# stochasticHydroTools/PSE

Hardware: AMD Instinct MI355X
Metric: BD particle-steps/s (full PSE Brownian step: M.F + k-space noise + Lanczos M^1/2.psi + Euler), N=1e6, phi=0.1 (higher is better)
Workload: dtype f64; 1 GPU; random-sphere suspension N=1000000, phi=0.1, cubic L=347.29, grid 256^3, xi=0.4405, rcut=5.966, P=6, error=0.001, kT=1.0, dt=0.001; parallelism=1 GPU

## Files before the change

include/pse_amd.h:

```cpp
#ifndef PSE_AMD_H
#define PSE_AMD_H

#ifdef __cplusplus
extern "C" {
#endif

typedef struct { double x, y, z, w; } pse_double4;
typedef struct { double x, y, z; } pse_double3;
typedef struct { int x, y, z; } pse_int3;

typedef struct pse_handle pse_handle;

enum pse_status {
    PSE_OK = 0,
    PSE_ERR_INVALID = -1,
    PSE_ERR_HIP = -2,
    PSE_ERR_FFT = -3,
    PSE_ERR_COMM = -4,
    PSE_ERR_NUMERIC = -5
};

typedef struct pse_params {
    unsigned int n_max;
    double Lx, Ly, Lz, xy;
    double xi;
    double error;
    double max_strain;
    unsigned int seed;
    int Nx, Ny, Nz;
    int P;
    double rcut;
    int device;
    int n_slabs;
    int slab_rank;
    int local_rows;
} pse_params;

typedef struct pse_info {
    int Nx, Ny, Nz, P;
    double rcut, xi, eta, gaussm, lambda, self_mobility, hx, hy, hz;
    int ncell_x, ncell_y, ncell_z;
    int lanczos_m;
    int lanczos_matvecs;
    double lanczos_stepnorm;
    double t_sort, t_spread, t_fft_fwd, t_scale, t_fft_inv, t_gather, t_real, t_lanczos, t_integrate, t_comm, t_total;
    unsigned long long device_bytes;
    double t_matvec;
    double t_records;
    int lanczos_exchanges;
    int lanczos_status;
    unsigned long long lanczos_open_calls;
} pse_info;

int pse_create(const pse_params *params, pse_handle **out);
int pse_destroy(pse_handle *h);
int pse_set_box(pse_handle *h, double Lx, double Ly, double Lz, double xy);
int pse_set_stream(pse_handle *h, void *hip_stream);
int pse_set_async(pse_handle *h, int enabled);
int pse_set_timestep_offset(pse_handle *h, const unsigned int *device_word);
int pse_debug_last_gate(pse_handle *h, int *gate);
int pse_set_neighbor_skin(pse_handle *h, double r_buff);
int pse_neighbor_stats(pse_handle *h, double *r_buff, unsigned long long *builds, unsigned long long *reuses);
int pse_set_timing(pse_handle *h, int enabled);
int pse_get_info(pse_handle *h, pse_info *info);
const char *pse_last_error(void);

int pse_mobility(pse_handle *h, const pse_double4 *pos, const pse_double4 *force, pse_double4 *vel,
                 const unsigned int *group_members, unsigned int N, int parts);

int pse_brownian_velocity(pse_handle *h, const pse_double4 *pos, const pse_double4 *force, pse_double4 *vel,
                          const unsigned int *group_members, unsigned int N,
                          double kT, double dt, unsigned int timestep, int *lanczos_m);

int pse_brownian_velocity_part(pse_handle *h, const pse_double4 *pos, const pse_double4 *force, pse_double4 *vel,
                               const unsigned int *group_members, unsigned int N, double kT, double dt, unsigned int timestep,
                               int parts, int *lanczos_m);
int pse_integrate(pse_handle *h, pse_double4 *pos, const pse_double4 *vel, pse_double3 *accel, pse_int3 *image,
                  const pse_double4 *net_force, const unsigned int *group_members, unsigned int N, double dt, double shear_rate);

int pse_step(pse_handle *h, pse_double4 *pos, pse_double4 *vel, pse_double3 *accel, pse_int3 *image,
             const pse_double4 *net_force, const unsigned int *group_members, unsigned int N,
             double kT, double dt, unsigned int timestep, double shear_rate, int *lanczos_m);

int pse_sqrt_mreal(pse_handle *h, const pse_double4 *pos, const pse_double4 *psi, pse_double4 *out,
                   const unsigned int *group_members, unsigned int N, double tol, int *lanczos_m);

int pse_random_psi(pse_handle *h, pse_double4 *psi, const unsigned int *group_members, unsigned int N,
                   unsigned int timestep);

int pse_eval_realspace(pse_handle *h, const double *r_host, int n, double *f_host, double *g_host);
int pse_pair_repulsion(pse_handle *h, const pse_double4 *pos, pse_double4 *force, const unsigned *group, unsigned N,
                       double k, double sigma, int accumulate);
int pse_debug_copy_grid(pse_handle *h, int stage, double *host_out);
int pse_debug_spread(pse_handle *h, const pse_double4 *pos, const pse_double4 *force, const unsigned int *group_members,
                     unsigned int N);
int pse_debug_kvector(pse_handle *h, int n, const int *ijk_host, double *out_host);
int pse_debug_grid_placement(pse_handle *h, int *tried, float *ms_first, float *ms_kept);
int pse_debug_vq_roundtrip(int n, const double *rows_host, double *out_host);
int pse_debug_matvec_ms(pse_handle *h, int reps, float *ms_per_launch);

typedef struct pse_team pse_team;
int pse_team_unique_id(void *id128_host);
int pse_team_create(pse_handle **members, int n_members, const void *id128_host, pse_team **out);
typedef struct pse_host_xfer {
    const double *send; size_t send_count; int send_to;
    double *recv; size_t recv_count; int recv_from;
} pse_host_xfer;
typedef struct pse_transport {
    void *user;
    int (*exchange)(void *user, int n_xfers, const pse_host_xfer *xfers);
    int (*allreduce_sum)(void *user, double *host_buf, size_t count);
} pse_transport;
int pse_team_create_transport(pse_handle *member, const pse_transport *transport, pse_team **out);
int pse_team_destroy(pse_team *team);
int pse_team_mobility(pse_team *team, const pse_double4 *const *pos, const pse_double4 *const *force,
                      pse_double4 *const *vel, const unsigned int *group_members, unsigned int N, int parts);
int pse_team_brownian_velocity(pse_team *team, const pse_double4 *const *pos, const pse_double4 *const *force,
                               pse_double4 *const *vel, const unsigned int *group_members, unsigned int N,
                               double kT, double dt, unsigned int timestep, int *lanczos_m);
int pse_team_step(pse_team *team, pse_double4 *const *pos, pse_double4 *const *vel, pse_double3 *const *accel,
                  pse_int3 *const *image, const pse_double4 *const *net_force, const unsigned int *group_members,
                  unsigned int N, double kT, double dt, unsigned int timestep, double shear_rate, int *lanczos_m);

int pse_team_step_local(pse_team *team, pse_double4 *const *pos, pse_double4 *const *vel, pse_double3 *const *accel,
                        pse_int3 *const *image, const pse_double4 *const *net_force, unsigned int *const *tag,
                        unsigned int *const *n_local, double kT, double dt, unsigned int timestep, double shear_rate,
                        int integrate, int *lanczos_m);
int pse_team_redistribute_local(pse_team *team, pse_double4 *const *pos, pse_double4 *const *vel, pse_double3 *const *accel,
                                pse_int3 *const *image, pse_double4 *const *net_force, unsigned int *const *tag,
                                unsigned int *const *n_local);
int pse_team_set_lanczos_extra(pse_team *team, int extra);
int pse_set_lanczos_extra(pse_handle *h, int extra);
enum pse_lanczos_operator { PSE_LANCZOS_RECORDS16 = 0, PSE_LANCZOS_FP64 = 1 };
int pse_set_lanczos_operator(pse_handle *h, int op);
int pse_get_lanczos_operator(pse_handle *h, int *op);
int pse_local_layout(pse_handle *h, int *rows_own, int *rows_ghost, int *records, int *layers, int *layers_per_rank);
int pse_team_local_status(pse_team *team, int *flags);

#define PSE_DIAG_MAX 48
typedef struct pse_team_diag {
    int n_exchanges;
    int kind[PSE_DIAG_MAX];
    int lane[PSE_DIAG_MAX];
    double device_us[PSE_DIAG_MAX];
    double host_us[PSE_DIAG_MAX];
    unsigned long long bytes[PSE_DIAG_MAX];
    double main_lane_ms, side_lane_ms;
    double critical_path_ms;
} pse_team_diag;
int pse_team_set_diag(pse_team *team, int enabled);
int pse_team_get_diag(pse_team *team, pse_team_diag *out);

int pse_team_debug_solo(pse_team *team, int slab_rank);

int pse_host_lanczos_sqrt_e1(int m, const double *alpha, const double *beta, double *t);
int pse_host_select_params(const pse_params *params, pse_info *info);

#ifdef __cplusplus
}
#endif
#endif
```

pse_amd/_lib.py:

```python
import ctypes
import os

_HERE = os.path.dirname(os.path.abspath(__file__))


def asan_dir():
    d = os.environ.get("PSE_ASAN_DIR")
    if not d:
        return None
    if not os.path.exists(os.path.join(d, ".pse_asan_build")):
        import sys
        print(f"pse_amd: PSE_ASAN_DIR={d} ignored: no sanitizer build there (python -m pse_amd.build --asan writes one)", file=sys.stderr)
        return None
    if not getattr(asan_dir, "_said", False):
        import sys
        print(f"pse_amd: using the CPU SANITIZER build in {d} (PSE_ASAN_DIR): device entry points are stubs", file=sys.stderr)
        asan_dir._said = True
    return d


_ASAN_DIR = asan_dir()
LIB_PATH = os.path.join(_ASAN_DIR or _HERE, "libpse_amd.so")

PSE_OK = 0
# ... 13 lines not shown
        ("local_rows", ctypes.c_int),
    ]


class pse_info(ctypes.Structure):
    _fields_ = [
        ("Nx", ctypes.c_int), ("Ny", ctypes.c_int), ("Nz", ctypes.c_int), ("P", ctypes.c_int),
        ("rcut", ctypes.c_double), ("xi", ctypes.c_double), ("eta", ctypes.c_double), ("gaussm", ctypes.c_double),
        ("lam", ctypes.c_double), ("self_mobility", ctypes.c_double),
        ("hx", ctypes.c_double), ("hy", ctypes.c_double), ("hz", ctypes.c_double),
        ("ncell_x", ctypes.c_int), ("ncell_y", ctypes.c_int), ("ncell_z", ctypes.c_int),
        ("lanczos_m", ctypes.c_int), ("lanczos_matvecs", ctypes.c_int),
        ("lanczos_stepnorm", ctypes.c_double),
        ("t_sort", ctypes.c_double), ("t_spread", ctypes.c_double), ("t_fft_fwd", ctypes.c_double),
        ("t_scale", ctypes.c_double), ("t_fft_inv", ctypes.c_double), ("t_gather", ctypes.c_double),
        ("t_real", ctypes.c_double), ("t_lanczos", ctypes.c_double), ("t_integrate", ctypes.c_double),
        ("t_comm", ctypes.c_double), ("t_total", ctypes.c_double),
        ("device_bytes", ctypes.c_ulonglong),
        ("t_matvec", ctypes.c_double),
        ("t_records", ctypes.c_double),
        ("lanczos_exchanges", ctypes.c_int),
        ("lanczos_status", ctypes.c_int),
        ("lanczos_open_calls", ctypes.c_ulonglong),
    ]

    def as_dict(self):
        return {name: getattr(self, name) for name, _ in self._fields_}


class pse_host_xfer(ctypes.Structure):
    _fields_ = [("send", ctypes.POINTER(ctypes.c_double)), ("send_count", ctypes.c_size_t), ("send_to", ctypes.c_int),
                ("recv", ctypes.POINTER(ctypes.c_double)), ("recv_count", ctypes.c_size_t), ("recv_from", ctypes.c_int)]


PSE_DIAG_MAX = 48


class pse_team_diag(ctypes.Structure):
    _fields_ = [("n_exchanges", ctypes.c_int), ("kind", ctypes.c_int * PSE_DIAG_MAX), ("lane", ctypes.c_int * PSE_DIAG_MAX),
                ("device_us", ctypes.c_double * PSE_DIAG_MAX), ("host_us", ctypes.c_double * PSE_DIAG_MAX),
                ("bytes", ctypes.c_ulonglong * PSE_DIAG_MAX), ("main_lane_ms", ctypes.c_double), ("side_lane_ms", ctypes.c_double),
                ("critical_path_ms", ctypes.c_double)]


EXCHANGE_FN = ctypes.CFUNCTYPE(ctypes.c_int, ctypes.c_void_p, ctypes.c_int, ctypes.POINTER(pse_host_xfer))
ALLREDUCE_FN = ctypes.CFUNCTYPE(ctypes.c_int, ctypes.c_void_p, ctypes.POINTER(ctypes.c_double), ctypes.c_size_t)


class pse_transport(ctypes.Structure):
    _fields_ = [("user", ctypes.c_void_p), ("exchange", EXCHANGE_FN), ("allreduce_sum", ALLREDUCE_FN)]


_vp, _i, _u, _d = ctypes.c_void_p, ctypes.c_int, ctypes.c_uint, ctypes.c_double
_ip = ctypes.POINTER(ctypes.c_int)
_dp = ctypes.POINTER(ctypes.c_double)
SYMBOLS = {
    "pse_create": (_i, [ctypes.POINTER(pse_params), ctypes.POINTER(_vp)]),
    "pse_destroy": (_i, [_vp]),
    "pse_set_box": (_i, [_vp, _d, _d, _d, _d]),
    "pse_set_stream": (_i, [_vp, _vp]),
    "pse_set_timing": (_i, [_vp, _i]),
    "pse_set_async": (_i, [_vp, _i]),
    "pse_set_timestep_offset": (_i, [_vp, _vp]),
    "pse_debug_last_gate": (_i, [_vp, _ip]),
    "pse_set_neighbor_skin": (_i, [_vp, _d]),
    "pse_neighbor_stats": (_i, [_vp, ctypes.POINTER(ctypes.c_double), ctypes.POINTER(ctypes.c_ulonglong), ctypes.POINTER(ctypes.c_ulonglong)]),
    "pse_get_info": (_i, [_vp, ctypes.POINTER(pse_info)]),
    "pse_last_error": (ctypes.c_char_p, []),
    "pse_mobility": (_i, [_vp, _vp, _vp, _vp, _vp, _u, _i]),
    "pse_brownian_velocity": (_i, [_vp, _vp, _vp, _vp, _vp, _u, _d, _d, _u, _ip]),
    "pse_brownian_velocity_part": (_i, [_vp, _vp, _vp, _vp, _vp, _u, _d, _d, _u, _i, _ip]),
    "pse_integrate": (_i, [_vp, _vp, _vp, _vp, _vp, _vp, _vp, _u, _d, _d]),
    "pse_step": (_i, [_vp, _vp, _vp, _vp, _vp, _vp, _vp, _u, _d, _d, _u, _d, _ip]),
    "pse_sqrt_mreal": (_i, [_vp, _vp, _vp, _vp, _vp, _u, _d, _ip]),
    "pse_random_psi": (_i, [_vp, _vp, _vp, _u, _u]),
    "pse_pair_repulsion": (_i, [_vp, _vp, _vp, _vp, _u, _d, _d, _i]),
    "pse_eval_realspace": (_i, [_vp, _dp, _i, _dp, _dp]),
    "pse_debug_copy_grid": (_i, [_vp, _i, _dp]),
    "pse_debug_spread": (_i, [_vp, _vp, _vp, _vp, _u]),
    "pse_debug_kvector": (_i, [_vp, _i, _ip, _dp]),
    "pse_debug_grid_placement": (_i, [_vp, _ip, ctypes.POINTER(ctypes.c_float), ctypes.POINTER(ctypes.c_float)]),
    "pse_debug_vq_roundtrip": (_i, [_i, _dp, _dp]),
    "pse_debug_matvec_ms": (_i, [_vp, _i, ctypes.POINTER(ctypes.c_float)]),
    "pse_team_unique_id": (_i, [_vp]),
    "pse_team_create": (_i, [ctypes.POINTER(_vp), _i, _vp, ctypes.POINTER(_vp)]),
    "pse_team_create_transport": (_i, [_vp, ctypes.POINTER(pse_transport), ctypes.POINTER(_vp)]),
    "pse_team_destroy": (_i, [_vp]),
    "pse_team_debug_solo": (_i, [_vp, _i]),
    "pse_team_mobility": (_i, [_vp, ctypes.POINTER(_vp), ctypes.POINTER(_vp), ctypes.POINTER(_vp), _vp, _u, _i]),
    "pse_team_brownian_velocity": (_i, [_vp, ctypes.POINTER(_vp), ctypes.POINTER(_vp), ctypes.POINTER(_vp), _vp, _u, _d, _d, _u, _ip]),
    "pse_team_step": (_i, [_vp, ctypes.POINTER(_vp), ctypes.POINTER(_vp), ctypes.POINTER(_vp), ctypes.POINTER(_vp),
                           ctypes.POINTER(_vp), _vp, _u, _d, _d, _u, _d, _ip]),
    "pse_team_step_local": (_i, [_vp, ctypes.POINTER(_vp), ctypes.POINTER(_vp), ctypes.POINTER(_vp), ctypes.POINTER(_vp),
                                 ctypes.POINTER(_vp), ctypes.POINTER(_vp), ctypes.POINTER(_vp), _d, _d, _u, _d, _i, _ip]),
    "pse_local_layout": (_i, [_vp, _ip, _ip, _ip, _ip, _ip]),
    "pse_team_local_status": (_i, [_vp, _ip]),
    "pse_team_set_lanczos_extra": (_i, [_vp, _i]),
    "pse_set_lanczos_extra": (_i, [_vp, _i]),
    "pse_set_lanczos_operator": (_i, [_vp, _i]),
    "pse_get_lanczos_operator": (_i, [_vp, _ip]),
    "pse_team_redistribute_local": (_i, [_vp] + [ctypes.POINTER(_vp)] * 7),
    "pse_team_set_diag": (_i, [_vp, _i]),
    "pse_team_get_diag": (_i, [_vp, ctypes.POINTER(pse_team_diag)]),
    "pse_host_lanczos_sqrt_e1": (_i, [_i, _dp, _dp, _dp]),
    "pse_host_select_params": (_i, [ctypes.POINTER(pse_params), ctypes.POINTER(pse_info)]),
}

_lib = None


class PSEError(RuntimeError):
    pass


def load():
    global _lib
    if _lib is not None:
        return _lib
    if not os.path.exists(LIB_PATH):
        raise PSEError(f"{LIB_PATH} not found: build it with `python -m pse_amd.build` "
                       "(there is no CPU fallback for the PSE hot path)")
    if not _ASAN_DIR:
        try:
            import torch
        except ImportError:
            pass
    lib = ctypes.CDLL(LIB_PATH, mode=ctypes.RTLD_GLOBAL)
    for name, (res, args) in SYMBOLS.items():
        fn = getattr(lib, name)
        fn.restype = res
        fn.argtypes = args
    _lib = lib
    return lib


def check(status):
    if status != PSE_OK:
        raise PSEError(f"pse_amd error {status}: {load().pse_last_error().decode()}")
```

pse_amd/csrc/asan_stub.cpp:

```cpp
#include <cmath>
#include <vector>

#include "pse_err.h"

using namespace pse;

struct pse_handle {
    pse_params par;
    Derived d;
    pse_info info;
    std::vector<double> coef;
    int n_intervals = 0;
    unsigned long long steps = 0;
    int lz_op = PSE_LANCZOS_RECORDS16;
};
struct pse_team { int unused; };

static int no_device(const char *what) { return fail(PSE_ERR_HIP, "%s: sanitizer build, there is no device behind this library", what); }

extern "C" {

int pse_create(const pse_params *p, pse_handle **out) {
    if (!p || !out) return fail(PSE_ERR_INVALID, "null argument");
    *out = nullptr;
    if (p->n_max == 0) return fail(PSE_ERR_INVALID, "n_max must be positive");
    if (!(std::fabs(p->xy) <= 0.5 * (1.0 + 1e-9))) return fail(PSE_ERR_INVALID, "tilt xy = %g outside [-0.5, 0.5]", p->xy);
    pse_handle *h = new pse_handle();
    h->par = *p;
    std::string e = select_params(Box{p->Lx, p->Ly, p->Lz, p->xy}, p->xi, p->error, p->max_strain, p->Nx, p->Ny, p->Nz, p->P, p->rcut, h->d);
    if (!e.empty()) { delete h; return fail(PSE_ERR_INVALID, "%s", e.c_str()); }
    if (int rc = gaussian_fits(h->d, h->d.hx, h->d.hy, h->d.hz)) { delete h; return rc; }
    build_realspace_table(h->d.xi, h->d.rcut, h->coef, h->n_intervals);
    fill_info(h->d, &h->info);
    *out = h;
    return 0;
}
int pse_destroy(pse_handle *h) { delete h; return 0; }
int pse_set_box(pse_handle *h, double Lx, double Ly, double Lz, double xy) {
    if (!h) return fail(PSE_ERR_INVALID, "null handle");
    if (!(Lx > 0 && Ly > 0 && Lz > 0)) return fail(PSE_ERR_INVALID, "box lengths must be positive");
    if (!(std::fabs(xy) <= 0.5 * (1.0 + 1e-9))) return fail(PSE_ERR_INVALID, "tilt xy = %g outside [-0.5, 0.5]", xy);
    if (int rc = gaussian_fits(h->d, Lx / h->d.Nx, Ly / h->d.Ny, Lz / h->d.Nz)) return rc;
    h->par.Lx = Lx; h->par.Ly = Ly; h->par.Lz = Lz; h->par.xy = xy;
    h->info.hx = Lx / h->d.Nx; h->info.hy = Ly / h->d.Ny; h->info.hz = Lz / h->d.Nz;
    return 0;
}
int pse_get_info(pse_handle *h, pse_info *info) {
    if (!h || !info) return fail(PSE_ERR_INVALID, "null argument");
    *info = h->info;
    return 0;
}
int pse_step(pse_handle *h, pse_double4 *, pse_double4 *, pse_double3 *, pse_int3 *, const pse_double4 *, const unsigned int *,
             unsigned int N, double kT, double dt, unsigned int, double, int *lanczos_m) {
    if (!h) return fail(PSE_ERR_INVALID, "null handle");
    if (N == 0 || N > h->par.n_max) return fail(PSE_ERR_INVALID, "N = %u outside (0, n_max = %u]", N, h->par.n_max);
    if (kT < 0 || !(dt > 0)) return fail(PSE_ERR_INVALID, "need kT >= 0 and dt > 0");
    ++h->steps;
    if (lanczos_m && *lanczos_m < 2) *lanczos_m = 2;
    return 0;
}
int pse_pair_repulsion(pse_handle *h, const pse_double4 *, pse_double4 *, const unsigned *, unsigned N, double, double sigma, int) {
    if (!h) return fail(PSE_ERR_INVALID, "null handle");
    if (N == 0 || N > h->par.n_max) return fail(PSE_ERR_INVALID, "N = %u outside (0, n_max = %u]", N, h->par.n_max);
    if (!(sigma > 0.0) || sigma > h->d.rcut) return fail(PSE_ERR_INVALID, "repulsion range %.4f outside (0, rcut = %.4f]", sigma, h->d.rcut);
    return 0;
}

int pse_set_stream(pse_handle *, void *) { return no_device("pse_set_stream"); }
int pse_set_timing(pse_handle *, int) { return no_device("pse_set_timing"); }
int pse_set_async(pse_handle *, int) { return no_device("pse_set_async"); }
int pse_set_timestep_offset(pse_handle *, const unsigned int *) { return no_device("pse_set_timestep_offset"); }
int pse_debug_last_gate(pse_handle *, int *) { return no_device("pse_debug_last_gate"); }
int pse_set_neighbor_skin(pse_handle *, double) { return no_device("pse_set_neighbor_skin"); }
int pse_neighbor_stats(pse_handle *, double *, unsigned long long *, unsigned long long *) { return no_device("pse_neighbor_stats"); }
int pse_mobility(pse_handle *, const pse_double4 *, const pse_double4 *, pse_double4 *, const unsigned int *, unsigned int, int) { return no_device("pse_mobility"); }
int pse_brownian_velocity(pse_handle *, const pse_double4 *, const pse_double4 *, pse_double4 *, const unsigned int *, unsigned int, double,
                          double, unsigned int, int *) { return no_device("pse_brownian_velocity"); }
int pse_sqrt_mreal(pse_handle *, const pse_double4 *, const pse_double4 *, pse_double4 *, const unsigned int *, unsigned int, double, int *) { return no_device("pse_sqrt_mreal"); }
int pse_random_psi(pse_handle *, pse_double4 *, const unsigned int *, unsigned int, unsigned int) { return no_device("pse_random_psi"); }
int pse_eval_realspace(pse_handle *, const double *, int, double *, double *) { return no_device("pse_eval_realspace"); }
int pse_debug_copy_grid(pse_handle *, int, double *) { return no_device("pse_debug_copy_grid"); }
int pse_debug_spread(pse_handle *, const pse_double4 *, const pse_double4 *, const unsigned int *, unsigned int) { return no_device("pse_debug_spread"); }
int pse_debug_kvector(pse_handle *, int, const int *, double *) { return no_device("pse_debug_kvector"); }
int pse_debug_grid_placement(pse_handle *, int *, float *, float *) { return no_device("pse_debug_grid_placement"); }
int pse_debug_vq_roundtrip(int, const double *, double *) { return no_device("pse_debug_vq_roundtrip"); }
int pse_debug_matvec_ms(pse_handle *, int, float *) { return no_device("pse_debug_matvec_ms"); }
int pse_set_lanczos_extra(pse_handle *, int) { return no_device("pse_set_lanczos_extra"); }
int pse_set_lanczos_operator(pse_handle *h, int op) {
    if (!h) return fail(PSE_ERR_INVALID, "pse_set_lanczos_operator: null handle");
    if (op != PSE_LANCZOS_RECORDS16 && op != PSE_LANCZOS_FP64) return fail(PSE_ERR_INVALID, "pse_set_lanczos_operator: %d is not an operator", op);
    h->lz_op = op;
    return 0;
}
int pse_get_lanczos_operator(pse_handle *h, int *op) {
    if (!h || !op) return fail(PSE_ERR_INVALID, "pse_get_lanczos_operator: null argument");
    *op = h->lz_op;
    return 0;
}
int pse_brownian_velocity_part(pse_handle *, const pse_double4 *, const pse_double4 *, pse_double4 *, const unsigned int *, unsigned int, double,
                               double, unsigned int, int, int *) { return no_device("pse_brownian_velocity_part"); }
int pse_integrate(pse_handle *, pse_double4 *, const pse_double4 *, pse_double3 *, pse_int3 *, const pse_double4 *, const unsigned int *, unsigned int,
                  double, double) { return no_device("pse_integrate"); }
int pse_team_redistribute_local(pse_team *, pse_double4 *const *, pse_double4 *const *, pse_double3 *const *, pse_int3 *const *, pse_double4 *const *,
                                unsigned int *const *, unsigned int *const *) { return no_device("pse_team_redistribute_local"); }
int pse_team_set_lanczos_extra(pse_team *, int) { return no_device("pse_team_set_lanczos_extra"); }
int pse_team_unique_id(void *) { return no_device("pse_team_unique_id"); }
int pse_team_create(pse_handle **, int, const void *, pse_team **) { return no_device("pse_team_create"); }
int pse_team_create_transport(pse_handle *, const pse_transport *, pse_team **) { return no_device("pse_team_create_transport"); }
int pse_team_destroy(pse_team *) { return 0; }
int pse_team_debug_solo(pse_team *, int) { return no_device("pse_team_debug_solo"); }
int pse_team_step_local(pse_team *, pse_double4 *const *, pse_double4 *const *, pse_double3 *const *, pse_int3 *const *, const pse_double4 *const *,
                        unsigned int *const *, unsigned int *const *, double, double, unsigned int, double, int, int *) { return no_device("pse_team_step_local"); }
int pse_local_layout(pse_handle *, int *, int *, int *, int *, int *) { return no_device("pse_local_layout"); }
int pse_team_local_status(pse_team *, int *) { return no_device("pse_team_local_status"); }
int pse_team_set_diag(pse_team *, int) { return no_device("pse_team_set_diag"); }
int pse_team_get_diag(pse_team *, pse_team_diag *) { return no_device("pse_team_get_diag"); }
int pse_team_mobility(pse_team *, const pse_double4 *const *, const pse_double4 *const *, pse_double4 *const *, const unsigned int *, unsigned int, int) { return no_device("pse_team_mobility"); }
int pse_team_brownian_velocity(pse_team *, const pse_double4 *const *, const pse_double4 *const *, pse_double4 *const *, const unsigned int *,
                               unsigned int, double, double, unsigned int, int *) { return no_device("pse_team_brownian_velocity"); }
int pse_team_step(pse_team *, pse_double4 *const *, pse_double4 *const *, pse_double3 *const *, pse_int3 *const *, const pse_double4 *const *,
                  const unsigned int *, unsigned int, double, double, unsigned int, double, int *) { return no_device("pse_team_step"); }

}
```

pse_amd/csrc/pse_capi.hip:

```cpp
#include <hip/hip_runtime.h>
#include <rccl/rccl.h>
#include <rocfft/rocfft.h>

#include <algorithm>
#include <chrono>
#include <cmath>
#include <cstdarg>
#include <cstdio>
#include <cstring>
#include <dlfcn.h>
#include <functional>
#include <future>
#include <memory>
#include <mutex>
#include <thread>
#include <string>
#include <vector>

#include "../../include/pse_amd.h"
#include "pse_err.h"
#include "pse_host.h"
#include "pse_kernels.h"
#include "pse_local.h"

using namespace pse;

#define HIPCHK(x)                                                                                      \
    do {                                                                                               \
        hipError_t e_ = (x);                                                                           \
        if (e_ != hipSuccess) return fail(PSE_ERR_HIP, "%s failed: %s (%s:%d)", #x, hipGetErrorString(e_), __FILE__, __LINE__); \
    } while (0)
#define FFTCHK(x)                                                                                      \
    do {                                                                                               \
        rocfft_status s_ = (x);                                                                        \
        if (s_ != rocfft_status_success) return fail(PSE_ERR_FFT, "%s failed: rocfft status %d (%s:%d)", #x, (int)s_, __FILE__, __LINE__); \
    } while (0)

#define TRY(x)              \
    do {                    \
        int r_ = (x);       \
        if (r_) return r_;  \
    } while (0)

constexpr int M_MAX = 100;
constexpr int PH_COUNT_ = 13;

struct Phase {
    hipEvent_t a = nullptr, b = nullptr;
};

struct pse_handle {
    pse_params par;
    Derived d;
    Box box;
    DBox dbox;
    DGrid G;
    DCells nc;
    double cell_gamma;
    int device = 0;
    hipStream_t stream = nullptr;
    hipStream_t wstream = nullptr;
    hipStream_t side = nullptr;
    hipStream_t side_owned = nullptr;
    int *bounds_host = nullptr;
    hipEvent_t ev_bounds = nullptr;
    bool bounds_pending = false;
    struct Tuning {
        int cell_bz = 6;
        double skin = 0.4;
        int overlap = 1;
        bool no_xfuse = false;
        int own_y_pow2 = 1;
        int own_y = 1;
        int own_z = 1;
        int yslab_regs = 1;
        int yfft_kb = 4;
        int wave_mode = 0;
        int spread_tz = 0, spread_nw = 0;
        int gather_bz = 0;
        int xmix_runtime = 0;
        int xfft_small_wide = 0;
        bool verbose = false;
        bool team_sstep = true;
        int team_sched[3] = {1, 2, 3};
        int vq = 1;
        int place_trials = 10;
        int lz_extra = 2;
        int lz_op = PSE_LANCZOS_RECORDS16;
    } tun;
    DCells bidx_nc = {0, 0, 0};
    hipEvent_t ev_fork = nullptr, ev_join = nullptr;
    bool overlap_all = false;
    bool side_on = false;
    hipEvent_t ev_scal = nullptr;
    int n_max = 0, n_pad = 0;
    unsigned *keys = nullptr, *keys_s = nullptr, *vals = nullptr, *perm = nullptr, *tag_s = nullptr;
    void *sort_tmp = nullptr;
    int *cell_cnt = nullptr;
    size_t sort_tmp_bytes = 0;
    int *cell_off = nullptr;
    int *cnt_block = nullptr;
    size_t cnt_bins = 0;
    SpreadWork sw = {};
    NbList nb = {};
    double4 *nb64 = nullptr;
    int lz_op = PSE_LANCZOS_RECORDS16;
    bool nb_valid = false;
    bool lz_last_queued = false;
    double skin = 0.0;
    double skin_max = 0.0;
    VerletList vl = {};
    double4 *pos_build = nullptr;
    int *flags_host = nullptr;
    bool vl_valid = false;
    bool vl_use = false;
    bool vl_pending = false;
    int vl_N = 0; const unsigned *vl_group = nullptr; Box vl_box = {};
    bool nc_wide = false;
    unsigned long long nlist_builds = 0, nlist_reuses = 0;
    int vl_reused_since_build = 0, vl_misses[2] = {0, 0}, vl_suspend_left[2] = {0, 0}, vl_suspend_len[2] = {32, 32};
    int vl_kind = 0;
    bool pv_is_f = false;
    bool w_is_mpsi = false;
    bool sums0_done = false;
    CombineSink sink = {};
    bool tail_done = false;
    bool async_mode = false;
    bool gated = false;
    int *gate_word = nullptr;
    size_t n_cells_alloc = 0;
    float4 *posf_s = nullptr;
    double2 *pv = nullptr;
    double4 *pos_s = nullptr, *f_s = nullptr, *uw_s = nullptr, *ur_s = nullptr, *ub_s = nullptr, *psi_s = nullptr, *w_s = nullptr;
    double *coef = nullptr;
    int n_intervals = 0;
    double *rgrid = nullptr;
    double2 *cgrid = nullptr;
    rocfft_plan plan_fwd = nullptr, plan_inv = nullptr;
    rocfft_plan plan_x_fwd = nullptr, plan_x_inv = nullptr;
    rocfft_execution_info info_fwd = nullptr, info_inv = nullptr;
    int n_slabs = 1, slab_rank = 0, nyl = 0, y0 = 0;
    double2 *sendbuf = nullptr, *recvbuf = nullptr;
    int *d_bidx = nullptr, *d_bounds = nullptr;
    std::vector<int> row_lo, first_end, last_begin;
    std::vector<int> first2_end, last2_begin;
    double4 *w2_s = nullptr, *u_s = nullptr;
    double *sums_all = nullptr;
    double4 *utot_s = nullptr;
    bool xfuse = false;
    bool own_y = false;
    bool own_y_slab = false;
    int lz_extra = -1;
    void *vq = nullptr;
    int place_tried = 0; float place_ms_first = 0, place_ms_kept = 0;
    bool own_z = false;
    double2 *twiddle_z = nullptr, *twiddle_z_owned = nullptr;
    double2 *twiddle_y = nullptr;
    double2 *twiddle_y_owned = nullptr;
    int grid_slabs = 1;
    double2 *twiddle = nullptr;
    void *fft_work = nullptr;
    size_t fft_work_bytes = 0;
    double4 *V = nullptr;
    double *scal = nullptr, *partials = nullptr;
    double *sc_host = nullptr;
    double *sc_host_dev = nullptr;
    int *bounds_host_dev = nullptr;
    int npart_cap = 0;
    struct LocalPlan {
        bool on = false;
        LocalGeom g{};
        int rows_cap = 0;
        double *send[2] = {nullptr, nullptr}, *recv[2] = {nullptr, nullptr};
        size_t msg = 0;
        double4 *stage_w1 = nullptr, *stage_w2 = nullptr;
        double4 *porig_s = nullptr; double *mass_s = nullptr; int3 *image_s = nullptr;
        LocalRows *rows = nullptr;
        int *counters = nullptr;
        int *layer_cnt = nullptr;
        size_t zero_ints = 0;
        bool zeroed = false;
        int *err = nullptr, *err_host = nullptr;
        double *rd_send = nullptr, *rd_recv = nullptr;
        int *rd_rows = nullptr, *rd_off = nullptr, *rd_host = nullptr;
    } loc;
// ... 94 lines not shown

static int cells_for(const Box &box, double rc, double gamma, int n_slabs, int bz_want, DCells &out, int xpad = 0) {
    const double wx = box.Lx / std::sqrt(1.0 + gamma * gamma), wy = box.Ly, wz = box.Lz;
    if (rc > 0.5 * wx * (1 + 1e-12) || rc > 0.5 * wy * (1 + 1e-12) || rc > 0.5 * wz * (1 + 1e-12))
        return fail(PSE_ERR_INVALID, "real-space cutoff %.4f exceeds half the box width (%.4f, %.4f, %.4f at tilt %.3f): "
                    "the minimum-image near field needs rcut <= L/2; increase xi", rc, wx, wy, wz, gamma);
    auto n = [&](double w) { int c = (int)std::floor(w / rc); if (c < 3) c = 1; if (c > 1024) c = 1024; return c; };
    out = DCells{n(wx), n(wy), n(wz), 0, 1, xpad};
    out.bz = (bz_want > 0 && out.nz >= 2 * bz_want) ? bz_want : out.nz;
    out.nzb = (out.nz + out.bz - 1) / out.bz;
    if (n_slabs > 1) {
        const int c = (int)std::floor(wx / rc) / n_slabs * n_slabs;
        if (c < 3 || c < n_slabs)
            return fail(PSE_ERR_INVALID, "box too small to split the near field over %d ranks: only %d cells of width >= rcut "
                        "fit along x", n_slabs, (int)std::floor(wx / rc));
        out.nx = std::min(c, 1024 / n_slabs * n_slabs);
    }
    return 0;
}
static double near_radius(const pse_handle *h) { return h->d.rcut + h->skin_max; }
static int set_cells(pse_handle *h, double gamma) {
    DCells nc;
    TRY(cells_for(h->box, near_radius(h), gamma, h->n_slabs, h->tun.cell_bz, nc, h->loc.on ? 1 : 0));
    h->nc = nc;
    h->cell_gamma = gamma;
    h->nc_wide = h->skin_max > 0.0;
    return 0;
}

enum { PH_SORT, PH_SPREAD, PH_FFTF, PH_SCALE, PH_FFTI, PH_GATHER, PH_REAL, PH_LANCZOS, PH_INTEG, PH_COMM, PH_TOTAL, PH_MATVEC, PH_RECORDS, PH_COUNT };
struct Roctx {
    int (*push)(const char *) = nullptr;
    int (*pop)() = nullptr;
    Roctx() {
        const char *e = getenv("PSE_ROCTX");
        if (!e || !atoi(e)) return;
        void *lib = dlopen("libroctx64.so.4", RTLD_NOW | RTLD_GLOBAL);
        if (!lib) lib = dlopen("libroctx64.so", RTLD_NOW | RTLD_GLOBAL);
        if (!lib) return;
        push = (int (*)(const char *))dlsym(lib, "roctxRangePushA");
        pop = (int (*)())dlsym(lib, "roctxRangePop");
        if (!push || !pop) push = nullptr, pop = nullptr;
    }
};
static const Roctx &roctx() { static Roctx r; return r; }
static_assert(PH_COUNT == PH_COUNT_, "phase table");
static const char *const PH_NAME[PH_COUNT] = {"pse:sort", "pse:spread", "pse:fft_forward", "pse:kspace_scale", "pse:fft_inverse", "pse:gather",
                                              "pse:near_field", "pse:lanczos", "pse:integrate", "pse:exchange", "pse:total", "pse:matvec",
                                              "pse:far_records"};
static void range_push(int p) { if (roctx().push) roctx().push(PH_NAME[p]); }
static void range_pop() { if (roctx().pop) roctx().pop(); }
static int ts(pse_handle *h, int p) { range_push(p); if (h->timing) HIPCHK(hipEventRecord(h->ph[p].a, h->stream)); return 0; }
static int te(pse_handle *h, int p) { if (h->timing) HIPCHK(hipEventRecord(h->ph[p].b, h->stream)); range_pop(); return 0; }
static int tsw(pse_handle *h, int p) { range_push(p); if (h->timing) HIPCHK(hipEventRecord(h->ph[p].a, h->wstream)); return 0; }
static int tew(pse_handle *h, int p) { if (h->timing) HIPCHK(hipEventRecord(h->ph[p].b, h->wstream)); range_pop(); return 0; }

static int collect_times(pse_handle *h, unsigned mask) {
    if (!h->timing) return 0;
    HIPCHK(hipStreamSynchronize(h->stream));
    if (h->side) HIPCHK(hipStreamSynchronize(h->side));
    double *dst[PH_COUNT] = {&h->info.t_sort, &h->info.t_spread, &h->info.t_fft_fwd, &h->info.t_scale, &h->info.t_fft_inv,
                             &h->info.t_gather, &h->info.t_real, &h->info.t_lanczos, &h->info.t_integrate, &h->info.t_comm,
                             &h->info.t_total, &h->info.t_matvec, &h->info.t_records};
    for (int p = 0; p < PH_COUNT; ++p) {
        *dst[p] = 0.0;
        if (mask & (1u << p)) {
            float ms = 0;
            if (hipEventElapsedTime(&ms, h->ph[p].a, h->ph[p].b) == hipSuccess) *dst[p] = ms;
        }
    }
    return 0;
}

extern "C" int pse_destroy(pse_handle *h) {
    if (!h) return 0;
    (void)hipSetDevice(h->device);
    (void)hipDeviceSynchronize();
    if (h->plan_fwd) rocfft_plan_destroy(h->plan_fwd);
    if (h->plan_inv) rocfft_plan_destroy(h->plan_inv);
    if (h->plan_x_fwd) rocfft_plan_destroy(h->plan_x_fwd);
    if (h->plan_x_inv) rocfft_plan_destroy(h->plan_x_inv);
    if (h->info_fwd) rocfft_execution_info_destroy(h->info_fwd);
    if (h->info_inv) rocfft_execution_info_destroy(h->info_inv);
    void *ptrs[] = {h->keys, h->keys_s, h->vals, h->perm, h->tag_s, h->sort_tmp, h->cell_off, h->cnt_block, h->sw.rec_t, h->sw.fb.off, h->sw.fb.rank_s, h->sw.fb.tmp, h->nb.data, h->nb.cnt, h->vl.idx, h->vl.cnt, h->pos_build, h->pos_s, h->posf_s, h->pv,
                    h->f_s, h->uw_s, h->ur_s, h->ub_s, h->psi_s, h->w_s, h->coef, h->rgrid, h->cgrid, h->sendbuf, h->recvbuf, h->d_bidx, h->d_bounds, h->utot_s, h->w2_s, h->u_s, h->sums_all, h->twiddle, h->twiddle_y_owned, h->twiddle_z_owned, h->fft_work, h->V,
                    h->scal, h->partials, h->lz_state, h->vq, h->nb64};
    for (void *p : ptrs) if (p) (void)hipFree(p);
    for (auto &p : h->ph) { if (p.a) (void)hipEventDestroy(p.a); if (p.b) (void)hipEventDestroy(p.b); }
    if (h->ev_fork) (void)hipEventDestroy(h->ev_fork);
    if (h->ev_scal) (void)hipEventDestroy(h->ev_scal);
    if (h->ev_join) (void)hipEventDestroy(h->ev_join);
    if (h->side_owned) (void)hipStreamDestroy(h->side_owned);
    if (h->bounds_host) (void)hipHostFree(h->bounds_host);
    if (h->ev_bounds) (void)hipEventDestroy(h->ev_bounds);
    if (h->sc_host) (void)hipHostFree(h->sc_host);
    if (h->flags_host) (void)hipHostFree(h->flags_host);
    {
        void *lp[] = {h->loc.send[0], h->loc.send[1], h->loc.recv[0], h->loc.recv[1], h->loc.stage_w1, h->loc.stage_w2, h->loc.porig_s, h->loc.mass_s,
                      h->loc.image_s, h->loc.rows, h->loc.err, h->loc.rd_send, h->loc.rd_recv, h->loc.rd_rows, h->loc.rd_off};
        for (void *q : lp) if (q) (void)hipFree(q);
        if (h->loc.err_host) (void)hipHostFree(h->loc.err_host);
        if (h->loc.rd_host) (void)hipHostFree(h->loc.rd_host);
    }
    delete h;
    return 0;
}

static int make_plans(pse_handle *h) {
    std::call_once(g_fft_once, [] { rocfft_setup(); });
    const DGrid &G = h->G;
    size_t work = 0, w = 0;
    h->xfuse = xfuse_supported(G.Nx) && !h->tun.no_xfuse;
    if (h->xfuse) {
        std::vector<double2> tw(G.Nx);
        for (int m = 0; m < G.Nx; ++m) {
            const long double ang = -2.0L * 3.14159265358979323846264338327950288L * m / G.Nx;
            tw[m] = make_double2((double)cosl(ang), (double)sinl(ang));
        }
        TRY(dmalloc(h, &h->twiddle, (size_t)G.Nx));
        HIPCHK(hipMemcpy(h->twiddle, tw.data(), G.Nx * sizeof(double2), hipMemcpyHostToDevice));
    }
    const bool z_ok = h->tun.own_z > 0 && zfft_supported(G.Nz);
    h->own_y = h->xfuse && h->grid_slabs == 1 && h->tun.own_y > 0 &&
               (yfft_supported(G.Ny) || (h->tun.own_y_pow2 && yfft_regs_supported(G.Ny, G.Nz, z_ok)));
    h->own_y_slab = h->xfuse && h->grid_slabs > 1 && h->tun.own_y > 0 && yfft_possible(G.Ny);
    h->own_z = z_ok && (h->own_y || h->own_y_slab);
    if (h->own_z) {
        if (G.Nz == G.Nx) h->twiddle_z = h->twiddle;
        else {
            std::vector<double2> tw(G.Nz);
            for (int m = 0; m < G.Nz; ++m) {
                const long double ang = -2.0L * 3.14159265358979323846264338327950288L * m / G.Nz;
                tw[m] = make_double2((double)cosl(ang), (double)sinl(ang));
            }
            TRY(dmalloc(h, &h->twiddle_z_owned, (size_t)G.Nz));
            HIPCHK(hipMemcpy(h->twiddle_z_owned, tw.data(), G.Nz * sizeof(double2), hipMemcpyHostToDevice));
            h->twiddle_z = h->twiddle_z_owned;
        }
    }
    if (h->own_y || h->own_y_slab) {
        if (G.Ny == G.Nx) h->twiddle_y = h->twiddle;
        else {
            std::vector<double2> tw(G.Ny);
            for (int m = 0; m < G.Ny; ++m) {
                const long double ang = -2.0L * 3.14159265358979323846264338327950288L * m / G.Ny;
                tw[m] = make_double2((double)cosl(ang), (double)sinl(ang));
            }
            TRY(dmalloc(h, &h->twiddle_y_owned, (size_t)G.Ny));
            HIPCHK(hipMemcpy(h->twiddle_y_owned, tw.data(), G.Ny * sizeof(double2), hipMemcpyHostToDevice));
            h->twiddle_y = h->twiddle_y_owned;
        }
    }
    auto real_plans = [&](size_t dims, const size_t *len, size_t batch) -> int {
        size_t rs[3] = {1, (size_t)G.Nz, (size_t)G.Ny * G.Nz}, cs[3] = {1, (size_t)G.Nzp, (size_t)G.Ny * G.Nzp};
        const size_t rdist = dims == 1 ? (size_t)G.Nz : (dims == 2 ? (size_t)G.Ny * G.Nz : (size_t)G.Nx * G.Ny * G.Nz);
        const size_t cdist = dims == 1 ? (size_t)G.Nzp : (dims == 2 ? (size_t)G.Ny * G.Nzp : (size_t)G.Nx * G.Ny * G.Nzp);
        rocfft_plan_description df = nullptr, di = nullptr;
        FFTCHK(rocfft_plan_description_create(&df));
        FFTCHK(rocfft_plan_description_create(&di));
        FFTCHK(rocfft_plan_description_set_data_layout(df, rocfft_array_type_real, rocfft_array_type_hermitian_interleaved, nullptr, nullptr,
                                                       dims, rs, rdist, dims, cs, cdist));
        FFTCHK(rocfft_plan_description_set_data_layout(di, rocfft_array_type_hermitian_interleaved, rocfft_array_type_real, nullptr, nullptr,
                                                       dims, cs, cdist, dims, rs, rdist));
        FFTCHK(rocfft_plan_create(&h->plan_fwd, rocfft_placement_notinplace, rocfft_transform_type_real_forward,
                                  rocfft_precision_double, dims, len, batch, df));
        FFTCHK(rocfft_plan_create(&h->plan_inv, rocfft_placement_notinplace, rocfft_transform_type_real_inverse,
                                  rocfft_precision_double, dims, len, batch, di));
// ... 1 lines not shown
        rocfft_plan_description_destroy(di);
        return 0;
    };
    if (h->own_y) {
        const size_t len1[1] = {(size_t)G.Nz};
        TRY(real_plans(1, len1, (size_t)3 * G.Nx * G.Ny));
    } else if (h->xfuse && h->grid_slabs == 1) {
        const size_t len2[2] = {(size_t)G.Nz, (size_t)G.Ny};
        TRY(real_plans(2, len2, (size_t)3 * G.Nx));
    } else if (h->grid_slabs == 1) {
        const size_t len[3] = {(size_t)G.Nz, (size_t)G.Ny, (size_t)G.Nx};
        TRY(real_plans(3, len, 3));
    } else {
        const size_t len2[2] = {(size_t)G.Nz, (size_t)G.Ny};
        const size_t len1[1] = {(size_t)G.Nz};
        if (h->own_y_slab) TRY(real_plans(1, len1, (size_t)G.nxl * G.Ny));
        else TRY(real_plans(2, len2, (size_t)G.nxl));
        const size_t lenx[1] = {(size_t)G.Nx};
        size_t stride[1] = {(size_t)h->nyl * G.Nzp};
        rocfft_plan_description desc = nullptr;
        FFTCHK(rocfft_plan_description_create(&desc));
        FFTCHK(rocfft_plan_description_set_data_layout(desc, rocfft_array_type_complex_interleaved,
                                                       rocfft_array_type_complex_interleaved, nullptr, nullptr, 1, stride, 1,
                                                       1, stride, 1));
        FFTCHK(rocfft_plan_create(&h->plan_x_fwd, rocfft_placement_inplace, rocfft_transform_type_complex_forward,
                                  rocfft_precision_double, 1, lenx, stride[0], desc));
        FFTCHK(rocfft_plan_create(&h->plan_x_inv, rocfft_placement_inplace, rocfft_transform_type_complex_inverse,
                                  rocfft_precision_double, 1, lenx, stride[0], desc));
        rocfft_plan_description_destroy(desc);
        FFTCHK(rocfft_plan_get_work_buffer_size(h->plan_x_fwd, &w)); work = std::max(work, w);
        FFTCHK(rocfft_plan_get_work_buffer_size(h->plan_x_inv, &w)); work = std::max(work, w);
    }
    FFTCHK(rocfft_plan_get_work_buffer_size(h->plan_fwd, &w)); work = std::max(work, w);
    FFTCHK(rocfft_plan_get_work_buffer_size(h->plan_inv, &w)); work = std::max(work, w);
    h->fft_work_bytes = work;
    if (work) TRY(dmalloc(h, (char **)&h->fft_work, work));
    FFTCHK(rocfft_execution_info_create(&h->info_fwd));
    FFTCHK(rocfft_execution_info_create(&h->info_inv));
    if (work) {
        FFTCHK(rocfft_execution_info_set_work_buffer(h->info_fwd, h->fft_work, work));
        FFTCHK(rocfft_execution_info_set_work_buffer(h->info_inv, h->fft_work, work));
    }
    FFTCHK(rocfft_execution_info_set_stream(h->info_fwd, h->wstream));
    FFTCHK(rocfft_execution_info_set_stream(h->info_inv, h->wstream));
    return 0;
}

static bool team_sstep(const pse_handle *h);
static int create_impl(const pse_params *p, pse_handle *h) {
    h->par = *p;
    h->box = Box{p->Lx, p->Ly, p->Lz, p->xy};
    std::string e = select_params(h->box, p->xi, p->error, p->max_strain, p->Nx, p->Ny, p->Nz, p->P, p->rcut, h->d);
    if (!e.empty()) return fail(PSE_ERR_INVALID, "%s", e.c_str());
    if (p->n_max == 0) return fail(PSE_ERR_INVALID, "n_max must be positive");
    TRY(gaussian_fits(h->d, h->d.hx, h->d.hy, h->d.hz));
    if (!(std::fabs(p->xy) <= 0.5 * (1.0 + 1e-9)))
        return fail(PSE_ERR_INVALID, "tilt xy = %g outside [-0.5, 0.5]: HOOMD flips the box there, and the sequential minimum image "
                    "(PSEv1/Mobility.cu:648) is exact only up to that tilt", p->xy);
    const Derived &d = h->d;
    if (p->device >= 0) { HIPCHK(hipSetDevice(p->device)); h->device = p->device; }
    else HIPCHK(hipGetDevice(&h->device));
    h->n_max = (int)p->n_max;
    set_dbox(h);
    h->n_slabs = std::max(1, p->n_slabs);
    h->loc.on = p->local_rows != 0;
    if (h->loc.on && h->n_slabs < 2) return fail(PSE_ERR_INVALID, "local_rows needs n_slabs >= 2 (an owned-particle rank is a member of a team)");
    (void)roctx();
    {
        auto ienv = [](const char *name, int dflt) { const char *v = getenv(name); return v ? atoi(v) : dflt; };
        auto &t = h->tun;
        t.cell_bz = std::min(16, std::max(0, ienv("PSE_CELL_BZ", 6)));
        if (const char *v = getenv("PSE_SKIN")) t.skin = atof(v);
        t.overlap = ienv("PSE_OVERLAP", 1);
        t.no_xfuse = getenv("PSE_NO_XFUSE") != nullptr;
        t.own_y = ienv("PSE_OWN_Y", 1); t.own_y_pow2 = ienv("PSE_OWN_Y_POW2", 1); t.yfft_kb = ienv("PSE_YFFT_KB", 4); t.own_z = ienv("PSE_OWN_Z", 1); t.yslab_regs = ienv("PSE_YSLAB_REGS", 1);
        if (const char *v = getenv("PSE_WAVE_MODE")) t.wave_mode = !strcmp(v, "slab") ? 1 : (!strcmp(v, "replicated") ? 2 : 0);
        t.spread_tz = ienv("PSE_SPREAD_TZ", 0); t.spread_nw = ienv("PSE_SPREAD_NW", 0);
        t.gather_bz = ienv("PSE_GATHER_BZ", 0); t.xmix_runtime = ienv("PSE_XMIX", 0) == 1; t.xfft_small_wide = ienv("PSE_XFFT_SMALL_KB", 2) == 8;
        t.verbose = ienv("PSE_VERBOSE", 0) > 0;
        t.team_sstep = ienv("PSE_TEAM_SSTEP", 1) > 0;
        t.lz_extra = std::max(0, std::min(32, ienv("PSE_LANCZOS_EXTRA", 2)));
        t.place_trials = std::max(0, std::min(12, ienv("PSE_PLACE_TRIALS", 10)));
        t.vq = ienv("PSE_VQ", 1);
        if (const char *v = getenv("PSE_LANCZOS_OP")) t.lz_op = !strcmp(v, "fp64") ? PSE_LANCZOS_FP64 : PSE_LANCZOS_RECORDS16;
        if (const char *v = getenv("PSE_TEAM_SCHED")) {
            int a = 1, b = 2, c = 3;
            if (sscanf(v, "%d,%d,%d", &a, &b, &c) == 3) { t.team_sched[0] = a; t.team_sched[1] = b; t.team_sched[2] = c; }
        }
        h->sw.force_tz = t.spread_tz; h->sw.force_nw = t.spread_nw; h->sw.force_bz = t.gather_bz;
    }
    {
        double skin = h->tun.skin;
        const int nint = (int)std::ceil(d.rcut * RS_PER_UNIT) + 1;
        const double gam = std::max(std::fabs(p->xy), p->max_strain);
        const double wmin = std::min(std::min(h->box.Lx / std::sqrt(1.0 + gam * gam), h->box.Ly), h->box.Lz);
        if (!(skin > 0.0) || h->n_slabs > 1 || !mreal_table_in_lds(nint * 2 * RS_NCOEF) || d.rcut + skin > 0.5 * wmin)
            skin = 0.0;
        h->skin = h->skin_max = skin;
    }
    TRY(set_cells(h, std::max(std::fabs(p->xy), p->max_strain)));
    fill_info(d, &h->info);
    h->info.ncell_x = h->nc.nx; h->info.ncell_y = h->nc.ny; h->info.ncell_z = h->nc.nz;

    DGrid &G = h->G;
    G.Nx = d.Nx; G.Ny = d.Ny; G.Nz = d.Nz; G.Nzh = d.Nz / 2 + 1; G.P = d.P;
    G.Nzp = (G.Nzh + 7) & ~7;
    h->n_slabs = std::max(1, p->n_slabs);
    h->slab_rank = h->n_slabs > 1 ? p->slab_rank : 0;
    if (h->slab_rank < 0 || h->slab_rank >= h->n_slabs) return fail(PSE_ERR_INVALID, "slab_rank outside [0, n_slabs)");
    h->grid_slabs = h->n_slabs;
    if (h->n_slabs > 1) {
        const bool replicate = h->tun.wave_mode ? h->tun.wave_mode == 2 : h->n_slabs == 2;
        if (replicate && !h->loc.on) h->grid_slabs = 1;
    }
    if (h->grid_slabs > 1) {
        if (d.Nx % h->grid_slabs || d.Ny % h->grid_slabs)
            return fail(PSE_ERR_INVALID, "slab decomposition needs Nx and Ny divisible by the number of ranks (%d x %d over %d)",
                        d.Nx, d.Ny, h->grid_slabs);
        if (d.Nx / h->grid_slabs < d.P)
            return fail(PSE_ERR_INVALID, "slabs of %d planes are thinner than the support P = %d", d.Nx / h->grid_slabs, d.P);
    }
    const int grid_rank = h->grid_slabs > 1 ? h->slab_rank : 0;
    G.nxl = d.Nx / h->grid_slabs; G.x0 = grid_rank * G.nxl;
    G.hl = h->grid_slabs > 1 ? (d.P - 1) / 2 : 0;
    G.nhalo = h->grid_slabs > 1 ? (d.P + 1) / 2 : 0;
    h->nyl = d.Ny / h->grid_slabs; h->y0 = grid_rank * h->nyl;
    G.hx = d.hx; G.hy = d.hy; G.hz = d.hz;
    const double c = 2.0 * d.xi * d.xi / d.eta;
    G.expfac = c;
    G.prefac = (c / M_PI) * std::sqrt(c / M_PI);

    const size_t n = ((size_t)h->n_max + h->n_slabs - 1) / h->n_slabs * h->n_slabs;
    h->n_pad = (int)n;
    TRY(dmalloc(h, &h->keys, n)); TRY(dmalloc(h, &h->keys_s, n)); TRY(dmalloc(h, &h->vals, n));
    TRY(dmalloc(h, &h->perm, n)); TRY(dmalloc(h, &h->tag_s, n));

    {
        const double rc = d.rcut;
        auto cnt = [&](double w) { int c2 = (int)std::floor(w / rc); if (c2 < 3) c2 = 1; if (c2 > 1024) c2 = 1024; return (size_t)c2; };
        h->n_cells_alloc = cnt(h->box.Lx) * cnt(h->box.Ly) * (cnt(h->box.Lz) + 16) + cnt(h->box.Lx);
    }
    TRY(dmalloc(h, &h->cell_off, h->n_cells_alloc + 1));
    h->sort_tmp_bytes = cell_sort_temp_bytes(h->n_cells_alloc);
    TRY(dmalloc(h, (char **)&h->sort_tmp, h->sort_tmp_bytes));
    const size_t nbins = (size_t)((d.Nx + 7) / 8) * ((d.Ny + 7) / 8) * ((d.Nz + 7) / 8);
    const bool fast_far = d.P >= 4 && d.P <= FAR_PMAX;
    h->cnt_bins = ((fast_far ? nbins + 1 : 0) + 1 + 3) & ~(size_t)3;
    constexpr size_t LAYER_INTS = (size_t)LOCAL_MAX_LAYERS * LOCAL_LAYER_SLOTS;
    TRY(dmalloc(h, &h->cnt_block, h->cnt_bins + 4 + h->n_cells_alloc + 1 + 8 + LOCAL_NCOUNTER + 2 + LAYER_INTS + 4));
    h->loc.counters = h->cnt_block + ((h->cnt_bins + 4 + h->n_cells_alloc + 1 + 8 + 1) & ~(size_t)1);
    h->loc.layer_cnt = h->loc.counters + LOCAL_NCOUNTER;
    h->loc.zero_ints = ((size_t)(h->loc.layer_cnt - h->cnt_block) + LAYER_INTS + 3) & ~(size_t)3;
    if (h->nc.nx > LOCAL_MAX_LAYERS && p->local_rows) return fail(PSE_ERR_INVALID, "more than %d cell layers along x", LOCAL_MAX_LAYERS);
    h->vl.flags = h->cnt_block + h->cnt_bins - 1;
    h->gate_word = h->cnt_block + h->cnt_bins + 1;
    h->cell_cnt = h->cnt_block + h->cnt_bins + 4;
    if (fast_far) {
        h->sw.fb.cnt = h->cnt_block;
        TRY(dmalloc(h, (char **)&h->sw.rec_t, (n + 64) * 64));
        TRY(dmalloc(h, &h->sw.fb.rank_s, n));
        TRY(dmalloc(h, &h->sw.fb.off, nbins + 1));
        h->sw.fb.tmp_bytes = bin_scan_temp_bytes(nbins);
        TRY(dmalloc(h, (char **)&h->sw.fb.tmp, h->sw.fb.tmp_bytes));
    }
    std::vector<double> coef;
    build_realspace_table(d.xi, d.rcut, coef, h->n_intervals);
    TRY(dmalloc(h, &h->coef, coef.size()));
    HIPCHK(hipMemcpy(h->coef, coef.data(), coef.size() * sizeof(double), hipMemcpyHostToDevice));
    TRY(dmalloc(h, &h->nb.cnt, n));
    {
        const double vol = h->box.Lx * h->box.Ly * h->box.Lz;
        const double n_box = h->loc.on ? (double)n * h->n_slabs * (h->nc.nx / h->n_slabs) / (h->nc.nx / h->n_slabs + 4.0) : (double)n;
        const double nbar = n_box / vol * 4.18879020478639 * d.rcut * d.rcut * d.rcut;
        int cap = (int)std::ceil(1.5 * nbar + 16.0);
        cap = (std::max(16, std::min(cap, 256)) + 3) & ~3;
        const double bytes = (double)cap * (double)n * 20.0;
        if (bytes > 32e9 || n >= ((size_t)1 << 27)) cap = 0;
        h->nb.cap = cap;
        if (cap > 0) {
            TRY(dmalloc(h, &h->nb.data, nb_list_bytes(n + 1024, cap)));
        }
        if (cap == 0) h->skin = h->skin_max = 0.0;
        if (h->skin_max > 0.0) {
            const double rs = d.rcut + h->skin_max, nbar_v = n_box / vol * 4.18879020478639 * rs * rs * rs;
            h->vl.cap = (std::max(16, std::min((int)std::ceil(2.0 * nbar_v + 32.0), 512)) + 3) & ~3;
            h->vl.rskin = rs;
            TRY(dmalloc(h, (char **)&h->vl.idx, verlet_list_bytes(n + 1024, h->vl.cap)));
            TRY(dmalloc(h, &h->vl.cnt, n));
            TRY(dmalloc(h, &h->pos_build, n));
            HIPCHK(hipHostMalloc((void **)&h->flags_host, 2 * sizeof(int)));
        }
    }
    TRY(dmalloc(h, &h->pos_s, n)); TRY(dmalloc(h, &h->posf_s, n));
    TRY(dmalloc(h, &h->pv, 3 * n));
    TRY(dmalloc(h, &h->f_s, n)); TRY(dmalloc(h, &h->uw_s, n)); TRY(dmalloc(h, &h->ur_s, n));
    TRY(dmalloc(h, &h->ub_s, n)); TRY(dmalloc(h, &h->psi_s, n)); TRY(dmalloc(h, &h->w_s, n));

    const size_t nr = (size_t)(G.nxl + G.hl + G.nhalo) * G.Ny * G.Nz, ncx = (size_t)G.nxl * G.Ny * G.Nzp;
    TRY(dmalloc(h, &h->rgrid, 3 * nr));
    TRY(dmalloc(h, &h->cgrid, 3 * ncx));
    if (h->grid_slabs > 1) { TRY(dmalloc(h, &h->sendbuf, 3 * ncx)); TRY(dmalloc(h, &h->recvbuf, 3 * ncx)); }
    if (h->n_slabs > 1) {
        HIPCHK(hipHostMalloc((void **)&h->bounds_host, ((size_t)5 * h->n_slabs + 1) * sizeof(int), hipHostMallocMapped));
        HIPCHK(hipHostGetDevicePointer((void **)&h->bounds_host_dev, h->bounds_host, 0));
        HIPCHK(hipEventCreateWithFlags(&h->ev_bounds, hipEventDisableTiming));
        TRY(dmalloc(h, &h->d_bidx, (size_t)5 * h->n_slabs + 1)); TRY(dmalloc(h, &h->d_bounds, (size_t)5 * h->n_slabs + 1));
        TRY(dmalloc(h, &h->utot_s, n));
        TRY(dmalloc(h, &h->sums_all, (size_t)h->n_slabs * LZ_NGRAM));
        if (h->tun.team_sstep && h->nb.cap > 0) {
            TRY(dmalloc(h, &h->w2_s, n)); TRY(dmalloc(h, &h->u_s, n));
        }
    }
    if (h->loc.on) {
        auto &L = h->loc;
        const int G_ = h->n_slabs, per = h->nc.nx / G_, depth = 2;
        if (per < depth + 1 || (G_ - 1) * per < 2 * depth)
            return fail(PSE_ERR_INVALID, "an owned-particle rank needs >= %d cell layers of width rcut per rank along x (%d ranks: %d layers each)",
                        G_ == 2 ? 2 * depth : depth + 1, G_, per);
        if (!team_sstep(h))
            return fail(PSE_ERR_INVALID, "an owned-particle rank needs the per-step pair list and the real-space table in LDS (rcut = %.3f, n_max = %d)",
                        d.rcut, h->n_max);
        if ((d.P / 2 + 1.0) / d.Nx > (double)depth / h->nc.nx)
            return fail(PSE_ERR_INVALID, "the spreading support (P = %d on %d planes) reaches beyond the %d ghost cell layers of an owned-particle rank", d.P, d.Nx, depth);
        const int c_g = (int)((double)h->n_max * depth / (per + 2 * depth)) / 256 * 256, c_own = (h->n_max - 2 * c_g) / 256 * 256;
        if (c_g < 256 || c_own < c_g)
            return fail(PSE_ERR_INVALID, "n_max = %d is too small a row capacity for an owned-particle rank (%d layers + 2 x %d ghost layers)", h->n_max, per, depth);
        L.g = LocalGeom{h->slab_rank, G_, per, depth, h->nc.nx, c_own, c_g, c_g};
        L.rows_cap = c_own + 2 * c_g;
        L.msg = (size_t)LOCAL_HDR + (size_t)LOCAL_REC * c_g;
        for (int q = 0; q < 2; ++q) { TRY(dmalloc(h, &L.send[q], L.msg)); TRY(dmalloc(h, &L.recv[q], L.msg)); HIPCHK(hipMemset(L.recv[q], 0, L.msg * sizeof(double))); }
        TRY(dmalloc(h, &L.stage_w1, (size_t)c_g)); TRY(dmalloc(h, &L.stage_w2, (size_t)c_g));
        TRY(dmalloc(h, &L.porig_s, (size_t)c_own)); TRY(dmalloc(h, &L.mass_s, (size_t)c_own)); TRY(dmalloc(h, &L.image_s, (size_t)c_own));
        TRY(dmalloc(h, &L.rows, 1));
        TRY(dmalloc(h, &L.err, 4));
        HIPCHK(hipMemset(L.err, 0, 4 * sizeof(int)));
        HIPCHK(hipMemset(L.rows, 0, sizeof(LocalRows)));
        HIPCHK(hipHostMalloc((void **)&L.err_host, 4 * sizeof(int)));
        L.err_host[0] = 0;
    }
    h->wstream = h->stream;
    if (h->tun.overlap >= 0) {
        {
            int lo = 0, hi = 0;
            (void)hipDeviceGetStreamPriorityRange(&lo, &hi);
// ... 409 lines not shown
    CopyBatch cb(act(T)[0]->stream);
    for (pse_handle *src : T.m)
        for (pse_handle *dst : act(T))
            if (src != dst) {
                const int r = src->slab_rank;
                cb.add(buf(dst) + (size_t)lo[r] * 4, buf(src) + (size_t)lo[r] * 4, (size_t)(lo[r + 1] - lo[r]) * 4);
            }
    return 0;
}

static int check_n(pse_handle *h, unsigned N) {
    if (!h) return fail(PSE_ERR_INVALID, "null handle");
    if (N == 0 || (int)N > h->n_max) return fail(PSE_ERR_INVALID, "N = %u outside (0, n_max = %d]", N, h->n_max);
    HIPCHK(hipSetDevice(h->device));
    return 0;
}

static void row_range(const pse_handle *h, int N, int &lo, int &hi) {
    if (h->n_slabs == 1) { lo = 0; hi = N; return; }
    lo = h->row_lo[h->slab_rank]; hi = h->row_lo[h->slab_rank + 1];
}

static int slab_bounds_issue(pse_handle *h) {
    const int G = h->n_slabs;
    if (G == 1) return 0;
    const int layer = h->nc.nzb * h->nc.ny * h->nc.bz, per = h->nc.nx / G;
    std::vector<int> idx(5 * G + 1);
    for (int r = 0; r <= G; ++r) idx[r] = r * per * layer;
    for (int r = 0; r < G; ++r) {
        idx[G + 1 + r] = (r * per + 1) * layer;
        idx[2 * G + 1 + r] = ((r + 1) * per - 1) * layer;
        idx[3 * G + 1 + r] = (r * per + std::min(2, per)) * layer;
        idx[4 * G + 1 + r] = ((r + 1) * per - std::min(2, per)) * layer;
    }
    if (h->bidx_nc.nx != h->nc.nx || h->bidx_nc.ny != h->nc.ny || h->bidx_nc.nz != h->nc.nz) {
        HIPCHK(hipStreamSynchronize(h->stream));
        HIPCHK(hipMemcpy(h->d_bidx, idx.data(), idx.size() * sizeof(int), hipMemcpyHostToDevice));
        h->bidx_nc = h->nc;
    }
    launch_pick(h->cell_off, h->d_bidx, (int)idx.size(), h->bounds_host_dev, h->stream);
    HIPCHK(hipEventRecord(h->ev_bounds, h->stream));
    h->bounds_pending = true;
    return 0;
}
static int slab_bounds_wait(pse_handle *h, int N) {
    if (!h->bounds_pending) return 0;
    h->bounds_pending = false;
    const int G = h->n_slabs;
    HIPCHK(hipEventSynchronize(h->ev_bounds));
    const int *out = h->bounds_host;
    h->row_lo.assign(out, out + G + 1);
    h->first_end.assign(out + G + 1, out + 2 * G + 1);
    h->last_begin.assign(out + 2 * G + 1, out + 3 * G + 1);
    h->first2_end.assign(out + 3 * G + 1, out + 4 * G + 1);
    h->last2_begin.assign(out + 4 * G + 1, out + 5 * G + 1);
    if (h->row_lo[0] != 0 || h->row_lo[G] != N) return fail(PSE_ERR_NUMERIC, "inconsistent cell offsets after the sort");
    return 0;
}

static bool team_sstep(const pse_handle *h) {
    const int G = h->n_slabs, per = h->nc.nx / std::max(1, G);
    return G > 1 && h->tun.team_sstep && h->w2_s && h->nb.cap > 0 && mreal_table_in_lds(h->n_intervals * 2 * RS_NCOEF) && per >= 2 &&
           h->nc.nx >= per + 4;
}

static CellRanges slab_need(const pse_handle *h) {
    CellRanges r{};
    const int G = h->n_slabs, nx = h->nc.nx;
    if (G == 1 || h->grid_slabs == 1) return r;
    const int per = nx / G, layer = h->nc.nzb * h->nc.ny * h->nc.bz;
    const int depth = team_sstep(h) ? 2 : 1;
    if (per + 2 * depth >= nx) return r;
    if ((h->G.P / 2 + 1.0) / h->G.Nx > 1.0 / nx) return r;
    const int start = ((h->slab_rank * per - depth) % nx + nx) % nx, len = per + 2 * depth;
    if (start + len <= nx) { r.n = 1; r.c0[0] = start * layer; r.c1[0] = (start + len) * layer; }
    else { r.n = 2; r.c0[0] = start * layer; r.c1[0] = nx * layer; r.c0[1] = 0; r.c1[1] = (start + len - nx) * layer; }
    return r;
}

struct PrepExtra { bool psi; unsigned timestep; };
static int prepare(pse_handle *h, const double4 *pos, const double4 *vec, const unsigned *group, int N, bool defer_bounds = false,
                   bool need_cells = false, PrepExtra px = PrepExtra{false, 0}, bool with_real = true) {
    TRY(ts(h, PH_SORT));
    const FarBinArgs far = far_bin_args(h->G, h->sw);
    double4 *psi_out = px.psi ? h->psi_s : nullptr;
    h->nb_valid = false;
    h->w_is_mpsi = false; h->sums0_done = false;
    h->vl_use = false;
    h->vl_pending = false;
    h->pv_is_f = vec != nullptr && h->pv != nullptr;
    const bool same_box = h->vl_box.Lx == h->box.Lx && h->vl_box.Ly == h->box.Ly && h->vl_box.Lz == h->box.Lz && h->vl_box.xy == h->box.xy;
    h->gated = false;
    if (h->async_mode && with_real && !px.psi && h->skin > 0.0 && h->vl_valid && !need_cells && h->vl_N == N && h->vl_group == group && same_box &&
        h->sorted_N == N && h->nc_wide && h->n_slabs == 1) {
        const int ncell = cells_total(h->nc);
        HIPCHK(hipMemsetAsync(h->cnt_block, 0, h->cnt_bins * sizeof(int), h->stream));
        launch_permute(pos, vec, group, h->perm, N, h->dbox, h->pos_s, h->posf_s, h->pv, h->f_s, h->tag_s, h->stream,
                       h->pos_build, 0.25 * h->skin * h->skin, h->vl.flags, CellRanges{}, nullptr, &far, nullptr, 0, 0);
        launch_gate_decide(h->vl.flags, h->gate_word, h->stream);
        const Gate rb{h->gate_word, 1};
        launch_gate_zero(rb, h->cnt_block, h->cnt_bins - 1, h->cell_cnt, (size_t)ncell + 1, h->stream);
        HIPCHK(cell_sort(pos, group, N, h->dbox, h->nc, h->keys, h->vals, h->keys_s, h->cell_cnt, ncell, h->sort_tmp, h->sort_tmp_bytes,
                         h->cell_off, h->perm, h->stream, CellRanges{}, SlabBook{}, true, rb));
        launch_permute(pos, vec, group, h->perm, N, h->dbox, h->pos_s, h->posf_s, h->pv, h->f_s, h->tag_s, h->stream, nullptr, 0.0, nullptr,
                       CellRanges{}, h->cell_off, &far, nullptr, 0, 0, rb);
        h->gated = true;
        h->vl.rskin = h->d.rcut + h->skin;
        h->sw.need = CellRanges{}; h->sw.cell_off = h->cell_off;
        ++h->nlist_builds;
        TRY(te(h, PH_SORT));
        HIPCHK(hipGetLastError());
        return 0;
    }
    if (h->skin > 0.0 && !h->async_mode && h->vl_valid && !need_cells && h->vl_N == N && h->vl_group == group && same_box && h->sorted_N == N) {
        HIPCHK(hipMemsetAsync(h->cnt_block, 0, h->cnt_bins * sizeof(int), h->stream));
        launch_permute(pos, vec, group, h->perm, N, h->dbox, h->pos_s, h->posf_s, h->pv, h->f_s, h->tag_s, h->stream,
                       h->pos_build, 0.25 * h->skin * h->skin, h->vl.flags, CellRanges{}, nullptr, &far, psi_out, h->par.seed, px.timestep, Gate{}, h->ts_off);
        HIPCHK(hipMemcpyAsync(h->flags_host, h->vl.flags, 2 * sizeof(int), hipMemcpyDeviceToHost, h->stream));
        HIPCHK(hipStreamSynchronize(h->stream));
        if (h->flags_host[0] == 0 && h->flags_host[1] == 0) {
            h->vl_use = true;
            ++h->nlist_reuses;
            ++h->vl_reused_since_build;
            h->vl_misses[h->vl_kind] = 0; h->vl_suspend_len[h->vl_kind] = 32;
            TRY(te(h, PH_SORT));
            return 0;
        }
        const int q = h->vl_kind;
        if (h->vl_reused_since_build == 0 && ++h->vl_misses[q] >= 2) {
            h->vl_suspend_left[q] = h->vl_suspend_len[q];
            h->vl_suspend_len[q] = std::min(2 * h->vl_suspend_len[q], 4096);
            h->vl_misses[q] = 1;
        }
    }
    h->vl_valid = false;
    ++h->nlist_builds;
    const bool with_list = h->skin > 0.0 && (h->async_mode ? !px.psi : h->vl_suspend_left[h->vl_kind] == 0);
    if (h->skin > 0.0 && !h->async_mode && !with_list) --h->vl_suspend_left[h->vl_kind];
    if (h->skin_max > 0.0) {
        const bool wide = h->nc_wide;
        if (wide != with_list) {
            DCells nc;
            TRY(cells_for(h->box, h->d.rcut + (with_list ? h->skin_max : 0.0), h->cell_gamma, h->n_slabs, h->tun.cell_bz, nc));
            h->nc = nc; h->nc_wide = with_list;
            h->info.ncell_x = nc.nx; h->info.ncell_y = nc.ny; h->info.ncell_z = nc.nz;
        }
    }
    const int ncell = cells_total(h->nc);
    if ((size_t)ncell > h->n_cells_alloc)
        return fail(PSE_ERR_INVALID, "cell grid %d x %d x %d exceeds the capacity sized at creation", h->nc.nx, h->nc.ny, h->nc.nz);
    const CellRanges need = slab_need(h);
    h->sw.need = need; h->sw.cell_off = h->cell_off;
    SlabBook sb{};
    if (need.n > 0 && h->n_slabs <= 64) {
        auto kept = [&](int c) { for (int q = 0; q < need.n; ++q) if (c >= need.c0[q] && c < need.c1[q]) return true; return false; };
        const int layer = h->nc.nzb * h->nc.ny * h->nc.bz, per = h->nc.nx / h->n_slabs;
        sb.n = h->n_slabs; sb.cells_per_slab = per * layer; sb.spread = std::max(1, std::min(1024, layer));
        for (int q = 0; q < h->n_slabs; ++q) {
            sb.book[q] = q * per * layer;
            for (int l = 0; l < per; ++l)
                if (!kept((q * per + l) * layer)) { sb.book[q] = (q * per + l) * layer; break; }
        }
    }
    HIPCHK(hipMemsetAsync(h->cnt_block, 0, ((h->cnt_bins + 4 + (size_t)ncell + 1 + 3) & ~(size_t)3) * sizeof(int), h->stream));
    HIPCHK(cell_sort(pos, group, N, h->dbox, h->nc, h->keys, h->vals, h->keys_s, h->cell_cnt, ncell, h->sort_tmp, h->sort_tmp_bytes,
                     h->cell_off, h->perm, h->stream, need, sb, true));
    launch_permute(pos, vec, group, h->perm, N, h->dbox, h->pos_s, h->posf_s, h->pv, h->f_s, h->tag_s, h->stream, nullptr, 0.0, nullptr,
                   need, h->cell_off, &far, psi_out, h->par.seed, px.timestep, Gate{}, h->ts_off);
    h->sorted_N = N;
    if (with_list) {
        h->vl_pending = true; h->vl_N = N; h->vl_group = group;
        h->vl.rskin = h->d.rcut + h->skin;
        h->vl_reused_since_build = 0;
    }
    TRY(slab_bounds_issue(h));
    if (!defer_bounds) TRY(slab_bounds_wait(h, N));
    TRY(te(h, PH_SORT));
    HIPCHK(hipGetLastError());
    return 0;
}

static ScaleArgs scale_args(pse_handle *h, bool noise, double kT, double dt, unsigned timestep) {
    ScaleArgs a;
    const DGrid &G = h->G;
    a.xi = h->d.xi; a.eta = h->d.eta; a.noise = noise ? 1 : 0;
    a.noise_fac = noise ? std::sqrt(2.0 * kT / dt / (G.hx * G.hy * G.hz)) : 0.0;
    a.seed = h->par.seed; a.timestep = timestep; a.ts_off = h->ts_off;
    a.transposed = h->grid_slabs > 1 ? 1 : 0; a.y0 = h->y0; a.nyl = h->grid_slabs > 1 ? h->nyl : G.Ny;
    a.runtime_plan = h->tun.xmix_runtime; a.wide_small = h->tun.xfft_small_wide;
    return a;
}

struct WaveArgs { int N; bool noise; double kT, dt; unsigned timestep; };
static int wave_compute(pse_team &T, const WaveArgs &a, int part) {
    const int GS = T.m[0]->grid_slabs;
    for (pse_handle *h : act(T)) {
        const DGrid &G = h->G;
        const size_t nr = (size_t)(G.nxl + G.hl + G.nhalo) * G.Ny * G.Nz, ncx = (size_t)G.nxl * G.Ny * G.Nzp;
        if (part == 0) {
            double *gx = h->rgrid, *gy = h->rgrid + nr, *gz = h->rgrid + 2 * nr;
            TRY(tsw(h, PH_RECORDS));
            HIPCHK(launch_far_records(h->pos_s, h->f_s, a.N, G, h->dbox, h->sw, h->wstream));
            TRY(tew(h, PH_RECORDS));
            TRY(tsw(h, PH_SPREAD));
            if (spread_needs_zero(G)) HIPCHK(hipMemsetAsync(h->rgrid, 0, 3 * nr * sizeof(double), h->wstream));
            HIPCHK(launch_spread(h->pos_s, h->f_s, a.N, gx, gy, gz, G, h->dbox, h->sw, h->wstream));
            TRY(tew(h, PH_SPREAD));
            TRY(tsw(h, PH_FFTF));
            double *zr[3]; double2 *zs[3];
            for (int c = 0; c < 3; ++c) { zr[c] = h->rgrid + c * nr + (size_t)G.hl * G.Ny * G.Nz; zs[c] = h->cgrid + c * ncx; }
            if (GS == 1) {
                if (h->own_z) launch_zfft(zr, zs, G.Nx * G.Ny, G.Nz, G.Nzp, false, h->twiddle_z, h->wstream);
                else {
                    void *in[1] = {h->rgrid}, *out[1] = {h->cgrid};
                    FFTCHK(rocfft_execute(h->plan_fwd, in, out, h->info_fwd));
                }
                if (h->own_y) launch_yfft(h->cgrid, G, false, h->twiddle_y, h->wstream, h->tun.yfft_kb);
            } else {
                if (h->own_z) launch_zfft(zr, zs, G.nxl * G.Ny, G.Nz, G.Nzp, false, h->twiddle_z, h->wstream);
                else for (int c = 0; c < 3; ++c) {
                    void *in[1] = {h->rgrid + c * nr + (size_t)G.hl * G.Ny * G.Nz}, *out[1] = {h->cgrid + c * ncx};
                    FFTCHK(rocfft_execute(h->plan_fwd, in, out, h->info_fwd));
                }
                if (h->own_y_slab) launch_yfft_slab(h->cgrid, h->sendbuf, G, h->nyl, false, h->twiddle_y, h->wstream, h->tun.yslab_regs > 0);
                else launch_slab_pack(h->cgrid, h->sendbuf, G.nxl, G.Ny, G.Nzp, h->nyl, 0, h->wstream);
            }
            TRY(tew(h, PH_FFTF));
        } else if (part == 1) {
            double2 *sp = GS == 1 ? h->cgrid : h->recvbuf;
            TRY(tsw(h, PH_SCALE));
            const ScaleArgs sa = scale_args(h, a.noise, a.kT, a.dt, a.timestep);
            if (h->xfuse) {
                launch_xfft_scale(sp, sp + ncx, sp + 2 * ncx, G, h->dbox, sa, h->twiddle, h->wstream);
            } else {
                if (GS > 1)
                    for (int c = 0; c < 3; ++c) { void *io[1] = {sp + c * ncx}; FFTCHK(rocfft_execute(h->plan_x_fwd, io, nullptr, h->info_fwd)); }
                launch_scale(sp, sp + ncx, sp + 2 * ncx, G, h->dbox, sa, h->wstream);
                if (GS > 1)
                    for (int c = 0; c < 3; ++c) { void *io[1] = {sp + c * ncx}; FFTCHK(rocfft_execute(h->plan_x_inv, io, nullptr, h->info_inv)); }
            }
            TRY(tew(h, PH_SCALE));
        } else if (part == 2) {
            TRY(tsw(h, PH_FFTI));
            double *zr[3]; double2 *zs[3];
            for (int c = 0; c < 3; ++c) { zr[c] = h->rgrid + c * nr + (size_t)G.hl * G.Ny * G.Nz; zs[c] = h->cgrid + c * ncx; }
            if (GS == 1) {
                if (h->own_y) launch_yfft(h->cgrid, G, true, h->twiddle_y, h->wstream, h->tun.yfft_kb);
                if (h->own_z) launch_zfft(zr, zs, G.Nx * G.Ny, G.Nz, G.Nzp, true, h->twiddle_z, h->wstream);
                else {
                    void *in[1] = {h->cgrid}, *out[1] = {h->rgrid};
                    FFTCHK(rocfft_execute(h->plan_inv, in, out, h->info_inv));
                }
            } else {
                if (h->own_y_slab) launch_yfft_slab(h->cgrid, h->sendbuf, G, h->nyl, true, h->twiddle_y, h->wstream, h->tun.yslab_regs > 0);
                else launch_slab_pack(h->cgrid, h->sendbuf, G.nxl, G.Ny, G.Nzp, h->nyl, 1, h->wstream);
                if (h->own_z) launch_zfft(zr, zs, G.nxl * G.Ny, G.Nz, G.Nzp, true, h->twiddle_z, h->wstream);
                else for (int c = 0; c < 3; ++c) {
                    void *in[1] = {h->cgrid + c * ncx}, *out[1] = {h->rgrid + c * nr + (size_t)G.hl * G.Ny * G.Nz};
                    FFTCHK(rocfft_execute(h->plan_inv, in, out, h->info_inv));
                }
            }
            TRY(tew(h, PH_FFTI));
        } else {
            TRY(tsw(h, PH_GATHER));
            HIPCHK(launch_gather(h->pos_s, h->sw, a.N, h->rgrid, h->rgrid + nr, h->rgrid + 2 * nr, G, h->dbox, h->uw_s, h->wstream));
            TRY(tew(h, PH_GATHER));
        }
    }
    return 0;
}
static int wave_exchange(pse_team &T, int k) {
    pse_handle *h0 = T.m[0];
    if (h0->grid_slabs == 1) return 0;
    const size_t blk = (size_t)h0->G.nxl * h0->nyl * h0->G.Nzp * 2, comp = blk * h0->grid_slabs;
    if (k == 0) {
        for (pse_handle *h : act(T)) TRY(tsw(h, PH_COMM));
        TRY(team_all_to_all(T, [&](pse_handle *h) { return (double *)h->sendbuf; }, [&](pse_handle *h) { return (double *)h->recvbuf; }, blk, 3, comp));
        for (pse_handle *h : act(T)) TRY(tew(h, PH_COMM));
        return 0;
    }
    if (k == 1)
        return team_all_to_all(T, [&](pse_handle *h) { return (double *)h->recvbuf; }, [&](pse_handle *h) { return (double *)h->sendbuf; }, blk, 3, comp);
    return team_halo_exchange(T);
}
struct WavePump {
// ... 912 lines not shown
    HIPCHK(hipMalloc((void **)&buf, (size_t)3 * n * sizeof(double)));
    hipError_t e = hipMemcpy(buf, r_host, n * sizeof(double), hipMemcpyHostToDevice);
    if (e == hipSuccess) {
        launch_eval_fg(buf, n, h->coef, buf + n, buf + 2 * n, h->stream);
        e = hipStreamSynchronize(h->stream);
    }
    if (e == hipSuccess) e = hipMemcpy(f_host, buf + n, n * sizeof(double), hipMemcpyDeviceToHost);
    if (e == hipSuccess) e = hipMemcpy(g_host, buf + 2 * n, n * sizeof(double), hipMemcpyDeviceToHost);
    (void)hipFree(buf);
    if (e != hipSuccess) return fail(PSE_ERR_HIP, "pse_eval_realspace: %s", hipGetErrorString(e));
    return 0;
}

extern "C" int pse_debug_matvec_ms(pse_handle *h, int reps, float *ms_per_launch) {
    if (!h || !ms_per_launch || reps < 1) return fail(PSE_ERR_INVALID, "pse_debug_matvec_ms: bad argument");
    HIPCHK(hipSetDevice(h->device));
    if (h->n_slabs != 1 || !h->nb_valid || h->nb.cap <= 0 || h->sorted_N <= 0)
        return fail(PSE_ERR_INVALID, "pse_debug_matvec_ms: needs the pair list of a Brownian call on a single-GPU engine (call it right after one)");
    const size_t stride = h->n_pad;
    const int N = h->sorted_N;
    RowMap rm{};
    rm.n = 1; rm.lo[0] = 0; rm.hi[0] = N;
    hipEvent_t e0 = nullptr, e1 = nullptr;
    HIPCHK(hipEventCreate(&e0)); HIPCHK(hipEventCreate(&e1));
    auto run = [&](int n) {
        for (int r = 0; r < n; ++r)
            launch_mreal_lanczos(h->pos_s, h->V + stride, h->w_s, rm, h->cell_off, h->dbox, h->nc, h->d.rcut, h->d.self, h->coef, h->nb,
                                 LzFuse{h->psi_s, h->partials, h->npart_cap, nullptr, nullptr, nullptr}, h->scal, nullptr, nullptr, h->stream,
                                 VerletList{}, 1, nullptr, DevRowArgs{}, vq_of(h), true);
    };
    run(2);
    HIPCHK(hipEventRecord(e0, h->stream));
    run(reps);
    HIPCHK(hipEventRecord(e1, h->stream));
    HIPCHK(hipEventSynchronize(e1));
    float ms = 0;
    HIPCHK(hipEventElapsedTime(&ms, e0, e1));
    (void)hipEventDestroy(e0); (void)hipEventDestroy(e1);
    HIPCHK(hipGetLastError());
    *ms_per_launch = ms / (float)reps;
    return 0;
}
extern "C" int pse_debug_vq_roundtrip(int n, const double *rows_host, double *out_host) {
    if (n < 0 || (n > 0 && (!rows_host || !out_host))) return fail(PSE_ERR_INVALID, "pse_debug_vq_roundtrip: null argument");
    if (n == 0) return 0;
    double *d_in = nullptr, *d_out = nullptr;
    hipError_t e = hipMalloc((void **)&d_in, (size_t)3 * n * sizeof(double));
    if (e == hipSuccess) e = hipMalloc((void **)&d_out, (size_t)3 * n * sizeof(double));
    if (e == hipSuccess) e = hipMemcpy(d_in, rows_host, (size_t)3 * n * sizeof(double), hipMemcpyHostToDevice);
    if (e == hipSuccess) { launch_vq_roundtrip(d_in, d_out, n, nullptr); e = hipGetLastError(); }
    if (e == hipSuccess) e = hipMemcpy(out_host, d_out, (size_t)3 * n * sizeof(double), hipMemcpyDeviceToHost);
    (void)hipFree(d_in); (void)hipFree(d_out);
    if (e != hipSuccess) return fail(PSE_ERR_HIP, "pse_debug_vq_roundtrip: %s", hipGetErrorString(e));
    return 0;
}
extern "C" int pse_debug_grid_placement(pse_handle *h, int *tried, float *ms_first, float *ms_kept) {
    if (!h || !tried || !ms_first || !ms_kept) return fail(PSE_ERR_INVALID, "pse_debug_grid_placement: null argument");
    *tried = h->place_tried; *ms_first = h->place_ms_first; *ms_kept = h->place_ms_kept;
    return 0;
}
extern "C" int pse_debug_kvector(pse_handle *h, int n, const int *ijk_host, double *out_host) {
    if (!h || !ijk_host || !out_host || n <= 0) return fail(PSE_ERR_INVALID, "bad argument");
    HIPCHK(hipSetDevice(h->device));
    for (int t = 0; t < n; ++t)
        if (ijk_host[3 * t] < 0 || ijk_host[3 * t] >= h->G.Nx || ijk_host[3 * t + 1] < 0 || ijk_host[3 * t + 1] >= h->G.Ny ||
            ijk_host[3 * t + 2] < 0 || ijk_host[3 * t + 2] >= h->G.Nz)
            return fail(PSE_ERR_INVALID, "node %d outside the %d x %d x %d grid", t, h->G.Nx, h->G.Ny, h->G.Nz);
    int *d_ijk = nullptr;
    double *d_out = nullptr;
    HIPCHK(hipMalloc((void **)&d_ijk, (size_t)3 * n * sizeof(int)));
    hipError_t e = hipMalloc((void **)&d_out, (size_t)5 * n * sizeof(double));
    if (e == hipSuccess) e = hipMemcpy(d_ijk, ijk_host, (size_t)3 * n * sizeof(int), hipMemcpyHostToDevice);
    if (e == hipSuccess) {
        launch_debug_kop(d_ijk, n, h->G, h->dbox, h->d.xi, h->d.eta, d_out, h->stream);
        e = hipStreamSynchronize(h->stream);
    }
    if (e == hipSuccess) e = hipMemcpy(out_host, d_out, (size_t)5 * n * sizeof(double), hipMemcpyDeviceToHost);
    (void)hipFree(d_ijk);
    if (d_out) (void)hipFree(d_out);
    if (e != hipSuccess) return fail(PSE_ERR_HIP, "pse_debug_kvector: %s", hipGetErrorString(e));
    return 0;
}

extern "C" int pse_debug_spread(pse_handle *h, const pse_double4 *pos, const pse_double4 *force, const unsigned *group, unsigned N) {
    TRY(check_n(h, N));
    if (!pos || !force) return fail(PSE_ERR_INVALID, "null array");
    if (h->n_slabs > 1) return fail(PSE_ERR_INVALID, "this handle is a slab rank: drive it through a pse_team");
    TRY(prepare(h, (const double4 *)pos, (const double4 *)force, group, (int)N));
    const DGrid &G = h->G;
    const size_t nr = (size_t)(G.nxl + G.hl + G.nhalo) * G.Ny * G.Nz;
    if (spread_needs_zero(G)) HIPCHK(hipMemsetAsync(h->rgrid, 0, 3 * nr * sizeof(double), h->stream));
    HIPCHK(launch_far_records(h->pos_s, h->f_s, (int)N, G, h->dbox, h->sw, h->stream));
    HIPCHK(launch_spread(h->pos_s, h->f_s, (int)N, h->rgrid, h->rgrid + nr, h->rgrid + 2 * nr, G, h->dbox, h->sw, h->stream));
    HIPCHK(hipStreamSynchronize(h->stream));
    return 0;
}

extern "C" int pse_debug_copy_grid(pse_handle *h, int stage, double *host_out) {
    if (!h || !host_out) return fail(PSE_ERR_INVALID, "bad argument");
    (void)stage;
    HIPCHK(hipSetDevice(h->device));
    HIPCHK(hipStreamSynchronize(h->stream));
    if (h->side) HIPCHK(hipStreamSynchronize(h->side));
    const size_t plane = (size_t)h->G.Ny * h->G.Nz, full = plane * (h->G.nxl + h->G.hl + h->G.nhalo);
    for (int c = 0; c < 3; ++c)
        HIPCHK(hipMemcpy(host_out + (size_t)c * plane * h->G.nxl, h->rgrid + c * full + plane * h->G.hl, plane * h->G.nxl * sizeof(double),
                         hipMemcpyDeviceToHost));
    return 0;
}

extern "C" int pse_team_unique_id(void *id128_host) {
    if (!id128_host) return fail(PSE_ERR_INVALID, "null argument");
    static_assert(sizeof(ncclUniqueId) == 128, "RCCL unique id is 128 bytes");
    ncclUniqueId id;
    NCCLCHK(ncclGetUniqueId(&id));
    memcpy(id128_host, &id, sizeof id);
    return 0;
}

extern "C" int pse_team_destroy(pse_team *T);
static int team_ring_test(pse_team &T) {
    if (T.G < 2 || !remote(T)) return 0;
    pse_handle *h = T.m[0];
    HIPCHK(hipSetDevice(h->device));
    double *buf = nullptr;
    HIPCHK(hipMalloc((void **)&buf, 2 * sizeof(double)));
    const double mine = 1000.0 + h->slab_rank;
    double got = -1.0;
    int rc = 0;
    hipError_t e = hipMemcpy(buf, &mine, sizeof(double), hipMemcpyHostToDevice);
    if (e == hipSuccess) {
        const int L = (h->slab_rank + T.G - 1) % T.G, R = (h->slab_rank + 1) % T.G;
        rc = team_exchange(T, {Xfer{buf, 1, R, buf + 1, 1, L}}, false);
        if (!rc) e = hipStreamSynchronize(h->stream);
        if (!rc && e == hipSuccess && T.comm) e = hipStreamSynchronize(T.comm);
        if (!rc && e == hipSuccess) e = hipMemcpy(&got, buf + 1, sizeof(double), hipMemcpyDeviceToHost);
        if (!rc && e == hipSuccess && got != 1000.0 + L)
            rc = fail(PSE_ERR_COMM, "team ring test: rank %d expected %g from its left neighbour %d and received %g -- the transport does not "
                      "connect the ranks as a ring of %d", h->slab_rank, 1000.0 + L, L, got, T.G);
    }
    (void)hipFree(buf);
    if (e != hipSuccess && !rc) rc = fail(PSE_ERR_COMM, "team ring test failed: %s", hipGetErrorString(e));
    return rc;
}
static int team_connect(pse_team *T, const void *id128_host) {
    if (T->m.size() != 1 || !id128_host) return 0;
    ncclUniqueId id;
    memcpy(&id, id128_host, sizeof id);
    HIPCHK(hipSetDevice(T->m[0]->device));
    {
        const char *te_ = getenv("PSE_TEAM_CONNECT_TIMEOUT");
        const int limit = te_ ? std::max(1, atoi(te_)) : 300;
        struct Slot { std::promise<ncclResult_t> done; ncclComm_t comm = nullptr; std::atomic<bool> abandoned{false}; };
        auto slot = std::make_shared<Slot>();
        std::future<ncclResult_t> fut = slot->done.get_future();
        const int G_ = T->G, r_ = T->m[0]->slab_rank, dev_ = T->m[0]->device;
        std::thread([slot, G_, id, r_, dev_]() {
            (void)hipSetDevice(dev_);
            const ncclResult_t r = ncclCommInitRank(&slot->comm, G_, id, r_);
            if (slot->abandoned.load() && r == ncclSuccess && slot->comm) { (void)ncclCommAbort(slot->comm); slot->comm = nullptr; }
            slot->done.set_value(r);
        }).detach();
        if (fut.wait_for(std::chrono::seconds(limit)) != std::future_status::ready) {
            slot->abandoned.store(true);
            return fail(PSE_ERR_COMM, "RCCL communicator of %d ranks did not form within %d s: a peer is missing (rank %d waited; "
                        "PSE_TEAM_CONNECT_TIMEOUT sets the limit)", G_, limit, r_);
        }
        const ncclResult_t r0 = fut.get();
        if (r0 != ncclSuccess) return fail(PSE_ERR_COMM, "ncclCommInitRank failed: %s", ncclGetErrorString(r0));
        T->nccl = slot->comm;
    }
    {
        const char *e = getenv("PSE_TEAM_LANES");
        T->lanes = e && atoi(e) > 0;
    }
// ... 313 lines not shown
```

pse_amd/csrc/pse_farbin.h:

```cpp
#pragma once
#include "pse_kernels.h"

namespace pse {

constexpr int BIN = 8;
__host__ __device__ inline int bins_of(int n) { return (n + BIN - 1) / BIN; }
__device__ __forceinline__ int bin_index(int ox, int oy, int oz, const FarBins &fb) {
    return ((ox / BIN) * fb.nby + (oy / BIN)) * fb.nbz + (oz / BIN);
}

__device__ __forceinline__ void support_start(double f, int n, int P, int &start, double &delta0) {
    const double s = f * n;
    const int i0 = (int)s;
    start = i0 - P / 2 + 1 - ((P & 1) && (s - i0 < 0.5) ? 1 : 0);
    delta0 = start - s;
}

__device__ __forceinline__ void far_support(double fx, double fy, double fz, const DGrid &G, int4 &o, double4 &d) {
    support_start(fx, G.Nx, G.P, o.x, d.x);
    support_start(fy, G.Ny, G.P, o.y, d.y);
    support_start(fz, G.Nz, G.P, o.z, d.z);
    o.x = wrapi(o.x, G.Nx); o.y = wrapi(o.y, G.Ny); o.z = wrapi(o.z, G.Nz);
    o.w = min((int)(fx * G.Nx), G.Nx - 1);
    d.w = 0.0;
}

__device__ __forceinline__ int far_bin_rank(bool need, int bin, int *__restrict__ cnt) {
    const int lane = threadIdx.x & 63;
    const unsigned long long below = (1ull << lane) - 1ull;
    unsigned long long todo = __ballot(need);
    if (!need) bin = -1;
    int prefix = 0, count = 0, leader = lane;
    while (todo) {
        const int src = __ffsll((long long)todo) - 1;
        const int b0 = __shfl(bin, src, 64);
        const unsigned long long m = __ballot(bin == b0) & todo;
        if (bin == b0) { prefix = __popcll(m & below); count = __popcll(m); leader = src; }
        todo &= ~m;
    }
    int base = 0;
    if (need && leader == lane) base = atomicAdd(&cnt[bin], count);
    base = __shfl(base, leader, 64);
    return need ? base + prefix : -1;
}

}
```

pse_amd/csrc/pse_farfield.hip:

```cpp
#include "pse_kernels.h"
#include "pse_farbin.h"

#include <hipcub/hipcub.hpp>
#include <type_traits>

namespace pse {

static inline int nblocks(long n, int tpb) { return (int)((n + tpb - 1) / tpb); }


struct FarRec {
    int ox, oy, oz;
    unsigned idx;
    double d0x, d0y, d0z;
    double fx, fy, fz;
};
static_assert(sizeof(FarRec) == 64, "record is four 16-byte loads");

template <int P>
__device__ __forceinline__ void gauss_axis(double e0, double lq, const double *__restrict__ r, double (&a)[P]) {
    double e = exp_lean(e0);
    const double q = exp_lean(lq);
#pragma unroll
    for (int t = 0; t < P; ++t) { a[t] = e; if (t + 1 < P) e *= q * r[t]; }
}

template <int P>
__device__ __forceinline__ void gauss_tables(double d0x, double d0y, double d0z, const DGrid &G, double s, const GaussConsts &gc,
                                             double (&ax)[P], double (&ay)[P], double (&az)[P]) {
    const double c = G.expfac;
    const double Y0 = G.hy * d0y, Z0 = G.hz * d0z, u = G.hx * d0x + s * Y0;
    double e = exp_lean(-c * u * u), q = exp_lean(-2.0 * c * G.hx * u);
#pragma unroll
    for (int t = 0; t < P; ++t) { ax[t] = e; if (t + 1 < P) e *= q * gc.rx[t]; }
    e = exp_lean(-c * Y0 * Y0); q = exp_lean(-2.0 * c * G.hy * (Y0 + s * u));
#pragma unroll
    for (int t = 0; t < P; ++t) { ay[t] = e; if (t + 1 < P) e *= q * gc.ry[t]; }
    e = exp_lean(-c * Z0 * Z0); q = exp_lean(-2.0 * c * G.hz * Z0);
#pragma unroll
    for (int t = 0; t < P; ++t) { az[t] = e; if (t + 1 < P) e *= q * gc.rz[t]; }
}

GaussConsts gauss_consts(const DGrid &G, double xy) {
    GaussConsts gc;
    const double c = G.expfac;
    for (int t = 0; t < FAR_PMAX - 1; ++t) {
        gc.rx[t] = std::exp(-c * G.hx * G.hx * (2 * t + 1));
        gc.ry[t] = std::exp(-c * G.hy * G.hy * (1.0 + xy * xy) * (2 * t + 1));
        gc.rz[t] = std::exp(-c * G.hz * G.hz * (2 * t + 1));
    }
    gc.lnk = -2.0 * c * xy * G.hx * G.hy;
    gc.s = xy;
    return gc;
}

struct FastDiv { unsigned m, d; };
static FastDiv fast_div(int d) { return FastDiv{(unsigned)((0x100000000ull + (unsigned)d - 1) / (unsigned)d), (unsigned)d}; }
__device__ __forceinline__ int fdiv(int n, FastDiv q, int &rem) {
    const int k = (int)__umulhi((unsigned)n, q.m);
    rem = n - k * (int)q.d;
    return k;
}

size_t bin_scan_temp_bytes(size_t nbins) {
    size_t bytes = 0;
    (void)hipcub::DeviceScan::ExclusiveSum(nullptr, bytes, (const int *)nullptr, (int *)nullptr, (int)(nbins + 1));
    return bytes;
}

bool farfield_fast_path(const DGrid &G);
__global__ void __launch_bounds__(256)
k_far_records(const double4 *__restrict__ pos_s, const double4 *__restrict__ f_s, int N, DGrid G, DBox box,
              FarBins fb, FarRec *__restrict__ rec) {
    const int p = blockIdx.x * blockDim.x + threadIdx.x;
    if (p >= N) return;
    const int rank = fb.rank_s[p];
    if (rank < 0) return;
    const double4 q = pos_s[p];
    double fx, fy, fz;
    frac_coords(box, q.x, q.y, q.z, fx, fy, fz);
    int4 sp;
    double4 d0;
    far_support(fx, fy, fz, G, sp, d0);
    const double4 F = f_s[p];
    const int slot = fb.off[bin_index(sp.x, sp.y, sp.z, fb)] + rank;
    const bool owned = G.nxl == G.Nx || wrapi(sp.w - G.x0, G.Nx) < G.nxl;
    int4 h = make_int4(sp.x, sp.y, sp.z, (int)((unsigned)p | (owned ? 0u : 0x80000000u)));
    double2 *o = reinterpret_cast<double2 *>(rec + slot);
    o[0] = *reinterpret_cast<double2 *>(&h);
    o[1] = make_double2(d0.x, d0.y);
    o[2] = make_double2(d0.z, G.prefac * F.x);
    o[3] = make_double2(G.prefac * F.y, G.prefac * F.z);
}

hipError_t launch_far_records(const double4 *pos_s, const double4 *f_s, int N, DGrid G, DBox box, SpreadWork w, hipStream_t s) {
    if (!farfield_fast_path(G) || !w.rec_t) return hipSuccess;
    FarBins fb = w.fb;
    fb.nbx = bins_of(G.Nx); fb.nby = bins_of(G.Ny); fb.nbz = bins_of(G.Nz);
    const int nbins = fb.nbx * fb.nby * fb.nbz;
    size_t tb = fb.tmp_bytes;
    hipError_t e = hipcub::DeviceScan::ExclusiveSum(fb.tmp, tb, fb.cnt, fb.off, nbins + 1, s);
    if (e != hipSuccess) return e;
    hipLaunchKernelGGL(k_far_records, dim3(nblocks(N, 256)), dim3(256), 0, s, pos_s, f_s, N, G, box, fb, w.rec_t);
    return hipGetLastError();
}
FarBinArgs far_bin_args(const DGrid &G, const SpreadWork &w) {
    FarBinArgs a{};
    a.on = farfield_fast_path(G) && w.rec_t != nullptr;
    a.G = G;
    a.fb = w.fb;
    a.fb.nbx = bins_of(G.Nx); a.fb.nby = bins_of(G.Ny); a.fb.nbz = bins_of(G.Nz);
    return a;
}
size_t far_bin_count(const DGrid &G) { return (size_t)bins_of(G.Nx) * bins_of(G.Ny) * bins_of(G.Nz) + 1; }

template <class F, int... I>
__device__ __forceinline__ void static_for_impl(F &&f, std::integer_sequence<int, I...>) { (f(std::integral_constant<int, I>{}), ...); }
template <int N, class F>
__device__ __forceinline__ void static_for(F &&f) { static_for_impl(f, std::make_integer_sequence<int, N>{}); }

template <int LO, int HI, class F>
__device__ __forceinline__ void uniform_dispatch(int k, F &&f) {
    if constexpr (HI - LO == 1) {
        f(std::integral_constant<int, LO>{});
    } else {
        constexpr int MID = (LO + HI) / 2;
        if (k < MID) uniform_dispatch<LO, MID>(k, f);
        else uniform_dispatch<MID, HI>(k, f);
    }
}

template <int P, int TZ, bool SHEAR, int NW>
__global__ void __launch_bounds__(64 * NW)
k_spread_tiles(const FarRec *__restrict__ rec, FarBins fb, double *__restrict__ gx, double *__restrict__ gy,
               double *__restrict__ gz, DGrid G, GaussConsts gc, FastDiv dz, FastDiv dy) {
    constexpr int TX = 8, TY = 8, PT = P + 1, LS = 65, RMAX = P <= 8 ? 20 : 32;
    constexpr int UB = (P + 4) & ~1;
    constexpr int WB = 2 * PT * LS + UB * 64 + ((2 * PT * LS) & 1);
    constexpr int RED = (NW - 1) * TZ * 3 * 64;
    __shared__ __attribute__((aligned(16))) double s_tab[NW * WB > RED ? NW * WB : RED];
    constexpr int KS = PT <= 8 ? 8 : 16;
    __shared__ double s_k[SHEAR ? PT * KS : 1];
    __shared__ int s_rb[RMAX], s_ro[RMAX + 1];
    const int lane = threadIdx.x & 63, wv = threadIdx.x >> 6, lx = lane & 7, ly = lane >> 3;
    double *const s_ax = s_tab + wv * WB, *const s_ay = s_ax + PT * LS, *const s_u = s_tab + wv * WB + (WB - UB * 64);
    auto wave_sync = [] () __attribute__((always_inline)) {
        if (NW == 1) __syncthreads(); else __builtin_amdgcn_wave_barrier();
    };
    int tz_, ty_;
    const int tx_ = fdiv(fdiv(xcd_block(blockIdx.x, gridDim.x), dz, tz_), dy, ty_);
    const int t0[3] = {G.x0 + tx_ * TX, ty_ * TY, tz_ * TZ};
    const int ext[3] = {min(TX, G.x0 + G.nxl - t0[0]), min(TY, G.Ny - t0[1]), min(TZ, G.Nz - t0[2])};
    const int Nn[3] = {G.Nx, G.Ny, G.Nz};
    const int nb[3] = {fb.nbx, fb.nby, fb.nbz};

    if (SHEAR)
        for (int e = threadIdx.x; e < PT * KS; e += 64 * NW) s_k[e] = exp_lean(gc.lnk * (double)((e / KS) * (e % KS)));
    int blo[3], bcnt[3];
#pragma unroll
    for (int a = 0; a < 3; ++a) {
        blo[a] = wrapi(t0[a] - (P - 1), Nn[a]) / BIN;
        bcnt[a] = min(nb[a], wrapi((t0[a] + ext[a] - 1) / BIN - blo[a], nb[a]) + 1);
    }
    const int zparts = blo[2] + bcnt[2] > nb[2] ? 2 : 1;
    const int nr = bcnt[0] * bcnt[1] * zparts;
    if ((int)threadIdx.x < nr) {
        const int zp = lane % zparts, r = lane / zparts, iy = r % bcnt[1], ix = r / bcnt[1];
        const int row = (((blo[0] + ix) % nb[0]) * nb[1] + (blo[1] + iy) % nb[1]) * nb[2];
        int z0 = blo[2], z1 = blo[2] + bcnt[2];
        if (zparts == 2) { if (zp == 0) z1 = nb[2]; else { z0 = 0; z1 = blo[2] + bcnt[2] - nb[2]; } }
        const int o = fb.off[row + z0];
        s_rb[lane] = o;
        s_ro[lane + 1] = fb.off[row + z1] - o;
    }
    __syncthreads();
    if (threadIdx.x == 0) {
        int run = 0;
        s_ro[0] = 0;
        for (int r = 0; r < nr; ++r) { run += s_ro[r + 1]; s_ro[r + 1] = run; }
    }
    __syncthreads();
    const int total = s_ro[nr];

    double acc[TZ][3];
    static_for<TZ>([&](auto zc) __attribute__((always_inline)) { constexpr int z = decltype(zc)::value; acc[z][0] = acc[z][1] = acc[z][2] = 0.0; });

    const unsigned lxb = (unsigned)(lx * LS * 8), lyb = (unsigned)(ly * LS * 8);
    double2 n0, n1, n2, n3;
    auto fetch = [&](int c0) __attribute__((always_inline)) {
        const int k = c0 + lane;
        int r = 0;
        for (int q = 1; q < nr; ++q) r = s_ro[q] <= k ? q : r;
        const size_t slot = k < total ? (size_t)(s_rb[r] + (k - s_ro[r])) : (size_t)s_rb[0];
        const double2 *rp = reinterpret_cast<const double2 *>(rec + slot);
        n0 = rp[0]; n1 = rp[1]; n2 = rp[2]; n3 = rp[3];
    };
    if (64 * wv < total) fetch(64 * wv);
    for (int c0 = 64 * wv; c0 < total; c0 += 64 * NW) {
        const bool valid = c0 + lane < total;
        const double2 q0 = n0, q1 = n1, q2 = n2, q3 = n3;
        if (c0 + 64 * NW < total) fetch(c0 + 64 * NW);
        const int4 hd = *reinterpret_cast<const int4 *>(&q0);
        const int o[3] = {hd.x, hd.y, hd.z};
        int rel[3];
        bool hit = valid;
#pragma unroll
        for (int a = 0; a < 3; ++a) {
            int d = o[a] - t0[a];
            if (d < -Nn[a] / 2) d += Nn[a]; else if (d >= Nn[a] - Nn[a] / 2) d -= Nn[a];
            rel[a] = d;
            hit = hit && d + P > 0 && d < ext[a];
        }
        unsigned long long mask = __ballot(hit);
        if (mask == 0ull) continue;
        wave_sync();
        {
            const double c = G.expfac;
            const double Y0 = G.hy * q1.y, Z0 = G.hz * q2.x, u = G.hx * q1.x + gc.s * Y0;
            double a[P];
            gauss_axis<P>(-c * u * u, -2.0 * c * G.hx * u, gc.rx, a);
            if (hit) {
                s_ax[P * LS + lane] = 0.0;
#pragma unroll
                for (int t = 0; t < P; ++t) s_ax[t * LS + lane] = a[t];
            }
            gauss_axis<P>(-c * Y0 * Y0, -2.0 * c * G.hy * (Y0 + gc.s * u), gc.ry, a);
            if (hit) {
                s_ay[P * LS + lane] = 0.0;
#pragma unroll
                for (int t = 0; t < P; ++t) s_ay[t * LS + lane] = a[t];
            }
            gauss_axis<P>(-c * Z0 * Z0, -2.0 * c * G.hz * Z0, gc.rz, a);
            if (hit) {
                double ub[UB];
#pragma unroll
                for (int t = 0; t < UB; ++t) ub[t] = t < P ? a[t] : 0.0;
                ub[P] = q2.y; ub[P + 1] = q3.x; ub[P + 2] = q3.y;
                double2 *up = reinterpret_cast<double2 *>(s_u + lane * UB);
#pragma unroll
                for (int t = 0; t < UB / 2; ++t) up[t] = make_double2(ub[2 * t], ub[2 * t + 1]);
            }
        }
        const int metax = rel[0] * (LS * 8) - lane * 8, metay = rel[1] * (LS * 8) - lane * 8;
        const int kzl = hit ? rel[2] + P - 1 : -1;
        wave_sync();
        static_for<TZ + P - 1>([&](auto kc) __attribute__((always_inline)) {
            constexpr int KZ = decltype(kc)::value, OZ = KZ - (P - 1);
            unsigned long long m = __ballot(kzl == KZ);
            while (m) {
                const int p = __ffsll((long long)m) - 1;
                m &= m - 1ull;
                const unsigned mx = (unsigned)__builtin_amdgcn_readlane(metax, p), my = (unsigned)__builtin_amdgcn_readlane(metay, p);
                const unsigned cap = (unsigned)(P * LS * 8 + p * 8);
                const unsigned bxo = min(lxb - mx, cap), byo = min(lyb - my, cap);
                double w = *reinterpret_cast<const double *>(reinterpret_cast<const char *>(s_ax) + bxo) *
// ... 95 lines not shown
    if (force == 8 || force == 16) return G.Nz >= 2 * force ? force : 8;
    const long blocks16 = (long)((G.nxl + 7) / 8) * ((G.Ny + 7) / 8) * ((G.Nz + 15) / 16);
    return G.Nz >= 64 && blocks16 >= 2048 ? 16 : 8;
}

bool farfield_fast_path(const DGrid &G) {
    const int need = 2 * std::max(8, G.P);
    return G.P >= 4 && G.P <= FAR_PMAX && G.Nx >= need && G.Ny >= need && G.Nz >= need;
}
bool spread_needs_zero(const DGrid &G) { return !farfield_fast_path(G); }
size_t farfield_bins(const DGrid &G) { return (size_t)bins_of(G.Nx) * bins_of(G.Ny) * bins_of(G.Nz); }

template <int P, int TZ, int NW>
static void launch_spread_pt(const FarRec *rec, FarBins fb, double *gx, double *gy, double *gz, const DGrid &G, const GaussConsts &gc,
                             hipStream_t s) {
    const int ntx = (G.nxl + 7) / 8, nty = (G.Ny + 7) / 8, ntz = (G.Nz + TZ - 1) / TZ;
    const dim3 g(ntx * nty * ntz), b(64 * NW);
    const FastDiv dz = fast_div(ntz), dy = fast_div(nty);
    if (gc.s != 0.0) hipLaunchKernelGGL((k_spread_tiles<P, TZ, true, NW>), g, b, 0, s, rec, fb, gx, gy, gz, G, gc, dz, dy);
    else hipLaunchKernelGGL((k_spread_tiles<P, TZ, false, NW>), g, b, 0, s, rec, fb, gx, gy, gz, G, gc, dz, dy);
}
constexpr int SPREAD_NW = 4;
template <int P>
static void launch_spread_p(const FarRec *rec, FarBins fb, double *gx, double *gy, double *gz, const DGrid &G, const GaussConsts &gc,
                            int force_tz, int nw_env, hipStream_t s) {
    const long blocks8 = (long)((G.nxl + 7) / 8) * ((G.Ny + 7) / 8) * ((G.Nz + 7) / 8);
    if (spread_tz(G, force_tz) == 16) launch_spread_pt<P, 16, 1>(rec, fb, gx, gy, gz, G, gc, s);
    else if (P <= 8 && (nw_env ? nw_env > 1 : blocks8 < 1024)) launch_spread_pt<P, 8, SPREAD_NW>(rec, fb, gx, gy, gz, G, gc, s);
    else launch_spread_pt<P, 8, 1>(rec, fb, gx, gy, gz, G, gc, s);
}

hipError_t launch_spread(const double4 *pos_s, const double4 *f_s, int N, double *gx, double *gy, double *gz, DGrid G,
                         DBox box, SpreadWork w, hipStream_t s) {
    if (!farfield_fast_path(G) || !w.rec_t) {
        hipLaunchKernelGGL(k_spread_atomic, dim3(nblocks(N, 4)), dim3(256), 0, s, pos_s, f_s, N, gx, gy, gz, G, box, w.need, w.cell_off);
        return hipGetLastError();
    }
    FarBins fb = w.fb;
    fb.nbx = bins_of(G.Nx); fb.nby = bins_of(G.Ny); fb.nbz = bins_of(G.Nz);
    const GaussConsts gc = gauss_consts(G, box.xy);
    switch (G.P) {
#define PSE_SPREAD_CASE(PV) case PV: launch_spread_p<PV>(w.rec_t, fb, gx, gy, gz, G, gc, w.force_tz, w.force_nw, s); break;
        PSE_SPREAD_CASE(4) PSE_SPREAD_CASE(5) PSE_SPREAD_CASE(6) PSE_SPREAD_CASE(7) PSE_SPREAD_CASE(8) PSE_SPREAD_CASE(9)
        PSE_SPREAD_CASE(10) PSE_SPREAD_CASE(11) PSE_SPREAD_CASE(12) PSE_SPREAD_CASE(13)
        default: launch_spread_p<14>(w.rec_t, fb, gx, gy, gz, G, gc, w.force_tz, w.force_nw, s); break;
#undef PSE_SPREAD_CASE
    }
    return hipGetLastError();
}

template <int CTRL>
__device__ __forceinline__ double dpp_quad(double v) {
    const int lo = __builtin_amdgcn_mov_dpp(__double2loint(v), CTRL, 0xF, 0xF, true);
    const int hi = __builtin_amdgcn_mov_dpp(__double2hiint(v), CTRL, 0xF, 0xF, true);
    return __hiloint2double(hi, lo);
}

typedef __attribute__((address_space(3))) void lds_void_t;
typedef __attribute__((address_space(1))) const void glb_void_t;

template <int P, bool SHEAR, int BZ = 1>
__global__ void __launch_bounds__(256)
k_gather_bins(const FarRec *__restrict__ rec, FarBins fb, FastDiv dz, FastDiv dy, int bx0, const double *__restrict__ gx,
              const double *__restrict__ gy, const double *__restrict__ gz, DGrid G, GaussConsts gc, double4 *__restrict__ u_s) {
    constexpr int NT = 256, E = BIN + P - 1, BINZ = BIN * BZ;
    constexpr int ZPL = 2, LPP = P <= 7 ? 4 : 8, ZW = ZPL * LPP;
    constexpr int EZ = (BINZ + P - 1 > BINZ - 2 + ZW ? BINZ + P : BINZ - 2 + ZW) & ~1, HZ = EZ / 2, ROW = E * EZ, E3 = E * ROW, NW = 2 * P + ZW;
    constexpr int PPP = (NT / LPP) < 40 ? (NT / LPP) : 40;
    constexpr int NPC = E * E * HZ, ITER = (NPC + NT - 1) / NT;
    static_assert(EZ >= BINZ + P - 1 && BINZ - 2 + ZW <= EZ, "z window inside the padded row");
    __shared__ __attribute__((aligned(16))) double reg[E3];
    __shared__ double s_w[NW * PPP];
    __shared__ int s_o[PPP];
    __shared__ unsigned s_id[PPP];
    constexpr int KS = P <= 8 ? 8 : 16;
    __shared__ double s_k[SHEAR ? P * KS : 1];
    const int tid = threadIdx.x, wave = tid >> 6, lane = tid & 63;
    int b = xcd_block(blockIdx.x, gridDim.x), bz, by;
    const int cmp = b % 3; b /= 3;
    b = fdiv(b, dz, bz);
    b = fdiv(b, dy, by);
    int bx = bx0 + b; if (bx >= fb.nbx) bx -= fb.nbx;
    const int bin = (bx * fb.nby + by) * fb.nbz + bz * BZ;
    const int base = fb.off[bin], n = fb.off[bin + min(BZ, fb.nbz - bz * BZ)] - base;
    if (n == 0) return;
    const double *g = cmp == 0 ? gx : (cmp == 1 ? gy : gz);
    const int t0[3] = {bx * BIN, by * BIN, bz * BINZ};
    static_assert(P <= 16 && P * KS <= NT, "one table entry per thread");
    if (SHEAR && tid < P * KS) s_k[tid] = exp_lean(gc.lnk * (double)((tid / KS) * (tid % KS)));
    const bool windowed = G.nxl < G.Nx;
    const int px0 = windowed ? wrapi(t0[0] - (G.x0 - G.hl), G.Nx) : t0[0];
    if (px0 + E <= (windowed ? G.nxl + G.hl + G.nhalo : G.Nx) && t0[1] + E <= G.Ny && t0[2] + EZ <= G.Nz) {
        const char *src = reinterpret_cast<const char *>(g + ((size_t)px0 * G.Ny + t0[1]) * G.Nz + t0[2]);
#pragma unroll
        for (int it = 0; it < ITER; ++it) {
            const int e0 = it * NT + wave * 64, e = e0 + lane, hz = e % HZ, r = e / HZ, qy = r % E, qx = r / E;
            const unsigned rel = (unsigned)((((size_t)qx * G.Ny + qy) * G.Nz + 2 * hz) * sizeof(double));
            if (e < NPC) __builtin_amdgcn_global_load_lds((glb_void_t *)(src + rel), (lds_void_t *)(reg + 2 * e0), 16, 0, 0);
        }
    } else {
        const int xs = G.x0 - G.hl, nstored = G.nxl + G.hl + G.nhalo;
        const size_t plane = (size_t)G.Ny * G.Nz;
        double2 v[ITER];
#pragma unroll
        for (int it = 0; it < ITER; ++it) {
            const int e = tid + it * NT, hz = e % HZ, r = e / HZ, qy = r % E, qx = r / E;
            int ix = t0[0] + qx; if (ix >= G.Nx) ix -= G.Nx;
            int iy = t0[1] + qy; if (iy >= G.Ny) iy -= G.Ny;
            int iz = t0[2] + 2 * hz; if (iz >= G.Nz) iz -= G.Nz;
            bool ok = e < NPC;
            if (windowed) { ix = wrapi(ix - xs, G.Nx); ok = ok && ix < nstored; }
            v[it] = make_double2(0.0, 0.0);
            if (ok) v[it] = *reinterpret_cast<const double2 *>(g + (size_t)ix * plane + (size_t)iy * G.Nz + iz);
        }
#pragma unroll
        for (int it = 0; it < ITER; ++it) {
            const int e = tid + it * NT;
            if (e < NPC) *reinterpret_cast<double2 *>(reg + 2 * e) = v[it];
        }
    }
    const int grp = tid / LPP, tl = tid % LPP;
    const double cw = G.prefac * G.hx * G.hy * G.hz;
    for (int h0 = 0; h0 < n; h0 += PPP) {
        const int np = min(PPP, n - h0);
        if (h0) __syncthreads();
        if (wave < 3 && lane < np) {
            const double2 *rp = reinterpret_cast<const double2 *>(rec + base + h0 + lane);
            const double2 q0 = rp[0], q1 = rp[1], q2 = rp[2];
            const int4 hd = *reinterpret_cast<const int4 *>(&q0);
            const double c = G.expfac;
            const double Y0 = G.hy * q1.y, Z0 = G.hz * q2.x, u = G.hx * q1.x + gc.s * Y0;
            double a[P];
            if (wave == 0) {
                gauss_axis<P>(-c * u * u, -2.0 * c * G.hx * u, gc.rx, a);
#pragma unroll
                for (int t = 0; t < P; ++t) s_w[t * PPP + lane] = a[t];
            } else if (wave == 1) {
                gauss_axis<P>(-c * Y0 * Y0, -2.0 * c * G.hy * (Y0 + gc.s * u), gc.ry, a);
#pragma unroll
                for (int t = 0; t < P; ++t) s_w[(P + t) * PPP + lane] = a[t];
            } else {
                gauss_axis<P>(-c * Z0 * Z0, -2.0 * c * G.hz * Z0, gc.rz, a);
                const int oz = hd.z - t0[2], odd = ZPL == 2 ? (oz & 1) : 0;
#pragma unroll
                for (int jw = 0; jw < ZW; ++jw) {
                    double wj = 0.0;
#pragma unroll
                    for (int t = 0; t < P; ++t) wj = (jw - odd == t) ? a[t] : wj;
                    s_w[(2 * P + jw) * PPP + lane] = wj;
                }
                s_o[lane] = (hd.x - t0[0]) * ROW + (hd.y - t0[1]) * EZ + (oz - odd);
                s_id[lane] = (unsigned)hd.w;
            }
        }
        __syncthreads();
        double u0 = 0.0;
        if (grp < np) {
            const double *r0 = reg + s_o[grp] + ZPL * tl;
            double ax[P], ay[P];
#pragma unroll
            for (int t = 0; t < P; ++t) { ax[t] = s_w[t * PPP + grp]; ay[t] = s_w[(P + t) * PPP + grp]; }
            double x0 = 0.0, x1 = 0.0;
#pragma unroll
            for (int tx = 0; tx < P; ++tx) {
                double y0 = 0.0, y1 = 0.0;
#pragma unroll
                for (int ty = 0; ty < P; ++ty) {
// ... 124 lines not shown
```

pse_amd/csrc/pse_kernels.h:

```cpp
#pragma once
#include <hip/hip_runtime.h>
#include <stdint.h>

#include "pse_device.h"

namespace pse {

size_t cell_sort_temp_bytes(size_t ncell);
struct CellRanges {
    int n, c0[3], c1[3];
    __device__ __forceinline__ bool cell(int c) const {
        if (n == 0) return true;
        for (int q = 0; q < n; ++q) if (c >= c0[q] && c < c1[q]) return true;
        return false;
    }
    __device__ __forceinline__ bool row(int s, const int *__restrict__ cell_off) const {
        if (n == 0) return true;
        for (int q = 0; q < n; ++q) if (s >= cell_off[c0[q]] && s < cell_off[c1[q]]) return true;
        return false;
    }
};
struct RowMap {
    int n, lo[3], hi[3], base[3];
    __host__ __device__ int list_rows() const { return n ? base[n - 1] + ((hi[n - 1] - lo[n - 1] + 255) & ~255) : 0; }
    __device__ __forceinline__ int first_row() const { return hi[0] > lo[0] ? lo[0] : (n > 1 && hi[1] > lo[1] ? lo[1] : lo[2]); }
    __device__ __forceinline__ int row(int lr) const {
        int l = lo[0], h = hi[0], b = base[0];
        if (n > 1 && lr >= base[1]) { l = lo[1]; h = hi[1]; b = base[1]; }
        if (n > 2 && lr >= base[2]) { l = lo[2]; h = hi[2]; b = base[2]; }
        const int i = l + (lr - b);
        return i < h ? i : -1;
    }
};
struct RowRanges { int n, lo[3], hi[3]; };
struct LocalRows {
    int n_own, n_gl, n_gr;
    int first_end;
    int last_begin;
    int ok;
    RowMap own, own1;
    RowRanges all;
};
struct DevRowArgs {
    const RowMap *rm;
    const LocalRows *lr;
    double4 *stage_hi;
    int rows_cap;
    int stage_cap;
};
struct RowMapRegs {
    int n, l0, l1, l2, h0, h1, h2, b1, b2;
    __device__ __forceinline__ RowMapRegs(const RowMap &m, const RowMap *dev) {
        n = m.n; l0 = m.lo[0]; l1 = m.lo[1]; l2 = m.lo[2]; h0 = m.hi[0]; h1 = m.hi[1]; h2 = m.hi[2]; b1 = m.base[1]; b2 = m.base[2];
        if (dev) { n = dev->n; l0 = dev->lo[0]; l1 = dev->lo[1]; l2 = dev->lo[2]; h0 = dev->hi[0]; h1 = dev->hi[1]; h2 = dev->hi[2]; b1 = dev->base[1]; b2 = dev->base[2]; }
    }
    __device__ __forceinline__ int list_rows() const { return n == 0 ? 0 : (n == 1 ? ((h0 - l0 + 255) & ~255) : (n == 2 ? b1 + ((h1 - l1 + 255) & ~255) : b2 + ((h2 - l2 + 255) & ~255))); }
    __device__ __forceinline__ int first_row() const { return h0 > l0 ? l0 : (n > 1 && h1 > l1 ? l1 : l2); }
    __device__ __forceinline__ int row(int lr) const {
        int l = l0, h = h0, b = 0;
        if (n > 1 && lr >= b1) { l = l1; h = h1; b = b1; }
        if (n > 2 && lr >= b2) { l = l2; h = h2; b = b2; }
        const int i = l + (lr - b);
        return i < h ? i : -1;
    }
};
inline RowMap row_map(int lo, int hi) { return RowMap{1, {lo, 0, 0}, {hi, 0, 0}, {0, 0, 0}}; }
inline RowMap row_map(const int (*rg)[2], int n) {
    RowMap m{};
    m.n = n;
    int base = 0;
    for (int k = 0; k < n; ++k) { m.lo[k] = rg[k][0]; m.hi[k] = rg[k][1]; m.base[k] = base; base += (rg[k][1] - rg[k][0] + 255) & ~255; }
    return m;
}

struct Gate {
    const int *word;
    int want;
    __device__ __forceinline__ bool closed() const { return word != nullptr && ((*word != 0) != (want != 0)); }
};
void launch_gate_decide(int *flags, int *word, hipStream_t s);
void launch_gate_zero(Gate g, int *a, size_t na, int *b, size_t nb, hipStream_t s);
void launch_gate_copy(Gate g, double4 *dst, const double4 *src, size_t n, hipStream_t s);
struct SlabBook { int n, cells_per_slab, spread, book[64]; };
hipError_t cell_sort(const double4 *pos, const unsigned *group, int N, DBox box, DCells nc, unsigned *keys, unsigned *rank,
                     unsigned *slots, int *cnt, int ncell, void *tmp, size_t tmp_bytes, int *cell_off, unsigned *perm, hipStream_t s,
                     CellRanges need = CellRanges{}, SlabBook sb = SlabBook{}, bool cnt_is_zero = false,
                     Gate gate = Gate{});
hipError_t launch_cell_scan(const int *cnt, int *out, int n, void *tmp, size_t tmp_bytes, hipStream_t s);
void launch_permute(const double4 *pos, const double4 *vec, const unsigned *group, const unsigned *perm, int N, DBox box,
                    double4 *pos_s, float4 *posf_s, double2 *pv, double4 *vec_s, unsigned *tag_s, hipStream_t s,
                    const double4 *pos_build = nullptr, double half_skin2 = 0.0, int *flags = nullptr,
                    CellRanges need = CellRanges{}, const int *cell_off = nullptr,
                    const struct FarBinArgs *far = nullptr,
                    double4 *psi_s = nullptr, uint32_t seed = 0, uint32_t timestep = 0,
                    Gate gate = Gate{}, const uint32_t *ts_off = nullptr);
void launch_permute_vec(const double4 *vec, const unsigned *tag_s, int N, double4 *vec_s, hipStream_t s);

struct NbList {
    char *data;
    int *cnt;
    int cap;
    double4 *c64;
};
__host__ __device__ inline size_t nb_list64_bytes(size_t rows, int cap) { return ((rows + 63) / 64) * (size_t)cap * 64 * 32; }
struct VerletList {
    unsigned *idx;
    int *cnt;
    int cap;
    int *flags;
    double rskin;
};
__host__ __device__ inline size_t verlet_list_bytes(size_t rows, int cap) { return ((rows + 63) / 64) * (size_t)(cap / 4) * 1024; }
enum { VL_NONE = 0, VL_WRITE = 1, VL_USE = 2 };
constexpr size_t NB_REC = 64 * 16;
__host__ __device__ inline size_t nb_list_bytes(size_t rows, int cap) { return ((rows + 63) / 64) * (size_t)cap * NB_REC; }
enum { MREAL_CELLS = 0, MREAL_BUILD_LIST = 1, MREAL_USE_LIST = 2 };
struct LzFuse {
    const double4 *vprev;
    double *partials;
    int npart_cap;
    const double4 *q, *p, *u;
};
enum { LZG_QW1 = 0, LZG_W1W1, LZG_W1W2, LZG_W2W2, LZG_PW1, LZG_PW2, LZG_UW2, LZG_QQ, LZ_NGRAM };
void launch_mreal(const double4 *pos_s, const float4 *posf_s, const double4 *vec_s, double4 *out_s, RowMap rows,
                  const int *cell_off, DBox box, DCells nc, double rcut, double self, const double *coef, int ncoef, NbList nb,
                  int mode, hipStream_t s, const double4 *vec2_s = nullptr, double4 *out2_s = nullptr,
                  VerletList vl = VerletList{}, int vl_mode = VL_NONE,
                  const double2 *pv = nullptr,
                  double *sums0 = nullptr, int sums0_cap = 0, double *scal = nullptr,
                  Gate gate = Gate{},
                  DevRowArgs dr = DevRowArgs{});
bool mreal_table_in_lds(int ncoef);
void launch_mreal_lanczos(const double4 *pos_s, const double4 *vec_s, double4 *w, RowMap rows, const int *cell_off,
                          DBox box, DCells nc, double rcut, double self, const double *coef, NbList nb, LzFuse lz,
                          double *scal, hipEvent_t ev_begin, hipEvent_t ev_end, hipStream_t s,
                          VerletList vl = VerletList{},
                          int sums = 1,
                          const int *stop = nullptr,
                          DevRowArgs dr = DevRowArgs{},
                          const void *vec_q = nullptr,
                          bool no_reduce = false);
int mreal_partials_needed(int rows);
void launch_lz_reduce3(const double *partials, int npart, int cap, double *scal, hipStream_t s);

struct FarBins {
    int nbx, nby, nbz;
    int *cnt, *off;
    int *rank_s;
    void *tmp; size_t tmp_bytes;
};
size_t bin_scan_temp_bytes(size_t nbins);
struct FarRec;
struct SpreadWork {
    FarBins fb;
    FarRec *rec_t;
    int force_tz, force_nw;
    int force_bz;
    CellRanges need;
    const int *cell_off;
    int rows_local;
};
constexpr int FAR_PMAX = 14;
struct GaussConsts { double rx[FAR_PMAX - 1], ry[FAR_PMAX - 1], rz[FAR_PMAX - 1], lnk, s; };
size_t farfield_bins(const DGrid &G);
bool spread_needs_zero(const DGrid &G);
struct FarBinArgs { bool on; DGrid G; FarBins fb; };
FarBinArgs far_bin_args(const DGrid &G, const SpreadWork &w);
size_t far_bin_count(const DGrid &G);
hipError_t launch_far_records(const double4 *pos_s, const double4 *f_s, int N, DGrid G, DBox box, SpreadWork w, hipStream_t s);
hipError_t launch_spread(const double4 *pos_s, const double4 *f_s, int N, double *gx, double *gy, double *gz, DGrid G,
                   DBox box, SpreadWork w, hipStream_t s);
struct ScaleArgs {
    double xi, eta;
    int noise;
    double noise_fac;
    uint32_t seed, timestep;
    const uint32_t *ts_off;
    int transposed;
    int y0, nyl;
    int runtime_plan;
    int wide_small;
};
void launch_scale(double2 *X, double2 *Y, double2 *Z, DGrid G, DBox box, ScaleArgs a, hipStream_t s);
void launch_debug_kop(const int *ijk, int n, DGrid G, DBox box, double xi, double eta, double *out, hipStream_t s);
bool xfuse_supported(int Nx);
bool yfft_supported(int Ny);
bool yfft_regs_supported(int Ny, int Nz, bool own_z = false);
bool yfft_possible(int Ny);
void launch_yfft_slab(double2 *cgrid, double2 *blocks, DGrid G, int nyl, bool inverse, const double2 *tw, hipStream_t s,
                      bool regs = true);
void launch_yfft(double2 *spectra, DGrid G, bool inverse, const double2 *tw, hipStream_t s, int kb = 4);
bool zfft_supported(int Nz);
void launch_zfft(double *const real[3], double2 *const spec[3], int rows, int Nz, int Nzp, bool inverse, const double2 *tw, hipStream_t s);
void launch_xfft_scale(double2 *X, double2 *Y, double2 *Z, DGrid G, DBox box, ScaleArgs a, const double2 *tw, hipStream_t s);
hipError_t launch_gather(const double4 *pos_s, SpreadWork w, int N, const double *gx, const double *gy, const double *gz, DGrid G,
                   DBox box, double4 *u_s, hipStream_t s);

void launch_slab_pack(double2 *cgrid, double2 *buf, int nxl, int Ny, int Nzh, int nyl, int unpack, hipStream_t s);
void launch_add_inplace(double *a, const double *b, size_t n, hipStream_t s);
struct CopyList { int n; const double *src[40]; double *dst[40]; unsigned cnt[40]; };
void launch_copy_list(const CopyList &l, hipStream_t s);

void launch_psi(double4 *psi_s, const unsigned *tag_s, int N, uint32_t seed, uint32_t timestep, hipStream_t s,
                CellRanges need = CellRanges{}, const int *cell_off = nullptr);
constexpr int LZ_ALPHA = 0, LZ_BETA = 128, LZ_NORM = 256, LZ_TMP = 257, LZ_UU = 272, LZ_NSCAL = 400;
constexpr int LZ_NPART = 1024;
struct BasisCoef { double t[104]; };
struct CombineSink { bool on; const double4 *add_a, *add_b; const unsigned *tag_s; double4 *vel; double4 *rows; };
void launch_basis_combine(const double4 *x0, const double4 *V, size_t stride, const BasisCoef &t, int m, const double *scal,
                          double scale, int use_norm, double4 *out_s, int lo, int hi, hipStream_t s, CombineSink sink = CombineSink{},
                          const struct LzState *st = nullptr);
void launch_lz_dots(const double4 *x, const double4 *y, const double4 *vprev, int lo, int hi, double *partials, int cap,
                    double *scal, hipStream_t s);
struct LzBlockArgs {
    const double4 *q, *p, *w1, *w2;
    double4 *u;
    double4 *v1, *v2;
    int j;
};
void launch_lz_block(const LzBlockArgs &a, bool full, double *scal, const int (*row_ranges)[2], int n_ranges, hipStream_t s,
                     const double *sums_all = nullptr, int nranks = 0, double *sch = nullptr,
                     const RowRanges *rg_dev = nullptr, int rows_cap = 0,
                     bool vectors_off = false, const int *stop = nullptr);
void launch_vq_roundtrip(const double *in, double *out, int n, hipStream_t s);
void launch_lz_update(const double4 *xin, const double4 *y, const double4 *xprev, double4 *xnext, int j,
                      double *scal, const int (*row_ranges)[2], int n_ranges, hipStream_t s,
                      const double *sums_all = nullptr, int nranks = 0, double *sch = nullptr, const int *stop = nullptr,
                      void *xq = nullptr);
struct LzState {
    int done;
    int m_final;
    int checked;
    int status;
    double stepnorm;
    double t_prev[104];
    double coef[104];
};
struct LzDecide {
    int m_lo, m_hi;
    int done_iters;
    int have_last_beta;
    int pending_beta;
    int first;
    int last;
    int normalised;
    int m_max;
    double tol;
};
constexpr int LZ_HOST_M = 380, LZ_HOST_STEPNORM = 381, LZ_HOST_STATUS = 382, LZ_HOST_SEQ = 383, LZ_HOST_OPEN = 384;
// ... 15 lines not shown
```

pse_amd/csrc/pse_kernels.hip:

```cpp
#include "pse_kernels.h"
#include "pse_dft.h"
#include "pse_farbin.h"

#include <hipcub/hipcub.hpp>
#include <atomic>

namespace pse {

constexpr int TPB = 256;
constexpr double TWO_PI = 6.283185307179586476925286766559;

static inline int nblocks(long n, int tpb) { return (int)((n + tpb - 1) / tpb); }

struct LdsAttr {
    std::atomic<size_t> have[32];
    bool need(size_t lds) {
        int dev = 0;
        (void)hipGetDevice(&dev);
        if (dev < 0 || dev >= 32) return true;
        if (have[dev].load(std::memory_order_relaxed) >= lds) return false;
        have[dev].store(lds, std::memory_order_relaxed);
        return true;
    }
};

__device__ __forceinline__ double wave_sum(double v) {
#pragma unroll
    for (int o = 32; o > 0; o >>= 1) v += __shfl_xor(v, o, 64);
    return v;
}
__device__ __forceinline__ double block_sum(double v, double *sh ) {
    v = wave_sum(v);
    const int w = threadIdx.x >> 6;
    __syncthreads();
    if ((threadIdx.x & 63) == 0) sh[w] = v;
    __syncthreads();
    return sh[0] + sh[1] + sh[2] + sh[3];
}
__device__ __forceinline__ double reduce_partials(const double *partials, int n, double *sh) {
    double v = 0.0;
    for (int i = threadIdx.x; i < n; i += TPB) v += partials[i];
    return block_sum(v, sh);
}

constexpr unsigned KEY_FOREIGN = 0xFFFFFFFFu;
__global__ void k_cell_keys(const double4 *__restrict__ pos, const unsigned *__restrict__ group, int N, DBox box,
                            DCells nc, unsigned *__restrict__ keys, unsigned *__restrict__ rank, int *__restrict__ cnt, CellRanges need,
                            SlabBook sb, Gate gate) {
    if (gate.closed()) return;
    const int g = blockIdx.x * blockDim.x + threadIdx.x;
    const bool live = g < N;
    unsigned key = 0;
    bool mine = false;
    if (live) {
        const unsigned idx = group ? group[g] : (unsigned)g;
        const double4 p = pos[idx];
        double fx, fy, fz;
        frac_coords(box, p.x, p.y, p.z, fx, fy, fz);
        const int cx = cell_coord(fx, nc.nx), cy = cell_coord(fy, nc.ny), cz = cell_coord(fz, nc.nz);
        const int zb = cz / nc.bz;
        key = (unsigned)cell_slot(nc, cx, cy, zb, cz - zb * nc.bz);
        mine = need.cell((int)key);
        if (mine) {
            keys[g] = key;
            rank[g] = (unsigned)atomicAdd(&cnt[key], 1);
        } else {
            keys[g] = KEY_FOREIGN;
            if (sb.n == 0) atomicAdd(&cnt[key], 1);
        }
    }
    if (sb.n > 0) {
        const int slab = live && !mine ? (int)(key / (unsigned)sb.cells_per_slab) : -1;
        unsigned long long todo = __ballot(slab >= 0);
        const int lane = threadIdx.x & 63;
        while (todo) {
            const int src = __ffsll((long long)todo) - 1;
            const int s0 = __shfl(slab, src, 64);
            const unsigned long long m = __ballot(slab == s0) & todo;
            if (lane == src) atomicAdd(&cnt[sb.book[s0] + (int)((blockIdx.x * 4u + (threadIdx.x >> 6)) % (unsigned)sb.spread)], __popcll(m));
            todo &= ~m;
        }
    }
}
__global__ void k_cell_scatter(const unsigned *__restrict__ keys, const unsigned *__restrict__ rank,
                               const int *__restrict__ cell_off, int N, unsigned *__restrict__ slots, Gate gate) {
    if (gate.closed()) return;
    const int g = blockIdx.x * blockDim.x + threadIdx.x;
    if (g < N && keys[g] != KEY_FOREIGN) slots[cell_off[keys[g]] + rank[g]] = (unsigned)g;
}
__global__ void __launch_bounds__(TPB)
k_cell_order(const int *__restrict__ cell_off, const unsigned *__restrict__ keys, int N, const unsigned *__restrict__ slots,
             unsigned *__restrict__ perm, CellRanges need, Gate gate) {
    if (gate.closed()) return;
    const int s = blockIdx.x * TPB + threadIdx.x;
    if (s >= N || !need.row(s, cell_off)) return;
    const unsigned v = slots[s];
    const int c = (int)keys[v], a = cell_off[c], n = cell_off[c + 1] - a;
    int smaller = 0;
    for (int t = 0; t < n; ++t) smaller += slots[a + t] < v ? 1 : 0;
    perm[a + smaller] = v;
}
size_t cell_sort_temp_bytes(size_t ncell) {
    size_t bytes = 0;
    (void)hipcub::DeviceScan::ExclusiveSum(nullptr, bytes, (const int *)nullptr, (int *)nullptr, (int)(ncell + 1));
    return bytes;
}
hipError_t launch_cell_scan(const int *cnt, int *out, int n, void *tmp, size_t tmp_bytes, hipStream_t s) {
    return hipcub::DeviceScan::ExclusiveSum(tmp, tmp_bytes, cnt, out, n, s);
}
hipError_t cell_sort(const double4 *pos, const unsigned *group, int N, DBox box, DCells nc, unsigned *keys, unsigned *rank,
                     unsigned *slots, int *cnt, int ncell, void *tmp, size_t tmp_bytes, int *cell_off, unsigned *perm, hipStream_t s,
                     CellRanges need, SlabBook sb, bool cnt_is_zero, Gate gate) {
    hipError_t e = cnt_is_zero ? hipSuccess : hipMemsetAsync(cnt, 0, (size_t)(ncell + 1) * sizeof(int), s);
    if (e != hipSuccess) return e;
    hipLaunchKernelGGL(k_cell_keys, dim3(nblocks(N, TPB)), dim3(TPB), 0, s, pos, group, N, box, nc, keys, rank, cnt, need, sb, gate);
    e = hipcub::DeviceScan::ExclusiveSum(tmp, tmp_bytes, cnt, cell_off, ncell + 1, s);
    if (e != hipSuccess) return e;
    hipLaunchKernelGGL(k_cell_scatter, dim3(nblocks(N, TPB)), dim3(TPB), 0, s, keys, rank, cell_off, N, slots, gate);
    hipLaunchKernelGGL(k_cell_order, dim3(nblocks(N, TPB)), dim3(TPB), 0, s, cell_off, keys, N, slots, perm, need, gate);
    return hipGetLastError();
}

__global__ void __launch_bounds__(TPB)
k_permute(const double4 *__restrict__ pos, const double4 *__restrict__ vec,
                          const unsigned *__restrict__ group, const unsigned *__restrict__ perm, int N, DBox box,
                          double4 *__restrict__ pos_s, float4 *__restrict__ posf_s, double2 *__restrict__ pv,
                          double4 *__restrict__ vec_s, unsigned *__restrict__ tag_s, const double4 *__restrict__ pos_build,
                          double half_skin2, int *__restrict__ flags, CellRanges need, const int *__restrict__ cell_off,
                          FarBinArgs far, double4 *__restrict__ psi_s, uint32_t seed, uint32_t timestep, Gate gate,
                          const uint32_t *__restrict__ ts_off) {
    if (gate.closed()) return;
    if (ts_off) timestep += *ts_off;
    const int s = blockIdx.x * blockDim.x + threadIdx.x;
    if (s - (int)(threadIdx.x & 63) >= N) return;
    const bool live = s < N && need.row(s, cell_off);
    bool bin_need = false;
    int bin = -1;
    if (live) {
        const unsigned g = perm[s];
        const unsigned idx = group ? group[g] : g;
        const double4 p = pos[idx];
        double fx, fy, fz;
        frac_coords(box, p.x, p.y, p.z, fx, fy, fz);
        const double y = (fy - 0.5) * box.Ly;
        double4 q;
        q.x = (fx - 0.5) * box.Lx + box.xy * y;
        q.y = y;
        q.z = (fz - 0.5) * box.Lz;
        q.w = 0.0;
        pos_s[s] = q;
        posf_s[s] = make_float4((float)q.x, (float)q.y, (float)q.z, 0.0f);
        if (pv) {
            pv[3 * (size_t)s] = make_double2(q.x, q.y);
            ((double *)&pv[3 * (size_t)s + 1])[0] = q.z;
        }
        tag_s[s] = idx;
        if (vec) {
            double4 v = vec[idx];
            v.w = 0.0;
            vec_s[s] = v;
            if (pv) {
                ((double *)&pv[3 * (size_t)s + 1])[1] = v.x;
                pv[3 * (size_t)s + 2] = make_double2(v.y, v.z);
            }
        }
        if (pos_build) {
            const double4 b = pos_build[s];
            double dx = q.x - b.x, dy = q.y - b.y, dz = q.z - b.z;
            min_image(box, dx, dy, dz);
            if (dx * dx + dy * dy + dz * dz > half_skin2) flags[0] = 1;
        }
        if (psi_s) {
            uint32_t r[4];
            philox4x32(idx, 0u, timestep, DOMAIN_PARTICLE, seed, PHILOX_KEY1, r);
            const double c = 1.7320508075688772;
            psi_s[s] = make_double4(uniform_pm(r[0], c), uniform_pm(r[1], c), uniform_pm(r[2], c), 0.0);
        }
        if (far.on) {
            double gx, gy, gz;
            frac_coords(box, q.x, q.y, q.z, gx, gy, gz);
            int4 o;
            double4 d;
            far_support(gx, gy, gz, far.G, o, d);
            bin_need = true;
            if (far.G.nxl < far.G.Nx) bin_need = wrapi(o.w - (far.G.x0 - far.G.P), far.G.Nx) < far.G.nxl + 2 * far.G.P;
            bin = bin_index(o.x, o.y, o.z, far.fb);
        }
    }
    if (far.on) {
        const int rk = far_bin_rank(bin_need, bin, far.fb.cnt);
        if (s < N) far.fb.rank_s[s] = rk;
    }
}

__global__ void k_permute_vec(const double4 *__restrict__ vec, const unsigned *__restrict__ tag_s, int N,
                              double4 *__restrict__ vec_s) {
    const int s = blockIdx.x * blockDim.x + threadIdx.x;
    if (s >= N) return;
    double4 v = vec[tag_s[s]];
    v.w = 0.0;
    vec_s[s] = v;
}

void launch_permute(const double4 *pos, const double4 *vec, const unsigned *group, const unsigned *perm, int N, DBox box,
                    double4 *pos_s, float4 *posf_s, double2 *pv, double4 *vec_s, unsigned *tag_s, hipStream_t s,
                    const double4 *pos_build, double half_skin2, int *flags, CellRanges need, const int *cell_off,
                    const FarBinArgs *far, double4 *psi_s, uint32_t seed, uint32_t timestep, Gate gate, const uint32_t *ts_off) {
    hipLaunchKernelGGL(k_permute, dim3(nblocks(N, TPB)), dim3(TPB), 0, s, pos, vec, group, perm, N, box, pos_s, posf_s, pv, vec_s, tag_s,
                       pos_build, half_skin2, flags, need, cell_off, far ? *far : FarBinArgs{}, psi_s, seed, timestep, gate, ts_off);
}
__global__ void k_gate_decide(int *__restrict__ flags, int *__restrict__ word) {
    const int f = flags[0] | flags[1];
    *word = f;
    if (f) flags[1] = 0;
}
void launch_gate_decide(int *flags, int *word, hipStream_t s) { hipLaunchKernelGGL(k_gate_decide, dim3(1), dim3(1), 0, s, flags, word); }
__global__ void k_gate_zero(Gate g, int *__restrict__ a, size_t na, int *__restrict__ b, size_t nb) {
    if (g.closed()) return;
    for (size_t i = (size_t)blockIdx.x * blockDim.x + threadIdx.x; i < na + nb; i += (size_t)gridDim.x * blockDim.x) {
        if (i < na) a[i] = 0; else b[i - na] = 0;
    }
}
void launch_gate_zero(Gate g, int *a, size_t na, int *b, size_t nb, hipStream_t s) {
    hipLaunchKernelGGL(k_gate_zero, dim3(std::max(1, std::min(1024, nblocks((long)(na + nb), TPB)))), dim3(TPB), 0, s, g, a, na, b, nb);
}
__global__ void k_gate_copy(Gate g, double4 *__restrict__ dst, const double4 *__restrict__ src, size_t n) {
    if (g.closed()) return;
    for (size_t i = (size_t)blockIdx.x * blockDim.x + threadIdx.x; i < n; i += (size_t)gridDim.x * blockDim.x) dst[i] = src[i];
}
void launch_gate_copy(Gate g, double4 *dst, const double4 *src, size_t n, hipStream_t s) {
    hipLaunchKernelGGL(k_gate_copy, dim3(std::max(1, std::min(4096, nblocks((long)n, TPB)))), dim3(TPB), 0, s, g, dst, src, n);
}
void launch_permute_vec(const double4 *vec, const unsigned *tag_s, int N, double4 *vec_s, hipStream_t s) {
    hipLaunchKernelGGL(k_permute_vec, dim3(nblocks(N, TPB)), dim3(TPB), 0, s, vec, tag_s, N, vec_s);
}

constexpr int QCAP = 44;
constexpr unsigned JMASK = (1u << 27) - 1;

struct PairCoef { int f, mx, my, mz, es; unsigned neg; };
__device__ __forceinline__ PairCoef pair_coef(double f, double h, double dx, double dy, double dz) {
    const double hs = (double)sqrtf((float)fabs(h));
    const double sx = dx * hs, sy = dy * hs, sz = dz * hs;
    const double m = fmax(fabs(sx), fmax(fabs(sy), fabs(sz)));
    int e = 0;
    (void)frexp(m, &e);
    e = e < -100 ? -100 : (e > 100 ? 100 : e);
    const double sc = __hiloint2double((21 - e + 1023) << 20, 0);
    const double lim = 2097151.0;
    PairCoef p;
    p.mx = (int)fmax(-lim, fmin(lim, rint(sx * sc))); p.my = (int)fmax(-lim, fmin(lim, rint(sy * sc))); p.mz = (int)fmax(-lim, fmin(lim, rint(sz * sc)));
    p.es = e;
    p.f = (int)fmax(-33554431.0, fmin(33554431.0, rint(f * 16777216.0)));
    p.neg = h < 0.0 ? 1u : 0u;
    return p;
}
__device__ __forceinline__ void pair_apply(const PairCoef &p, double vx, double vy, double vz, double &ux, double &uy, double &uz) {
    const double sc = __hiloint2double((p.es - 21 + 1023) << 20, 0);
    const double fr = (double)p.f * 5.9604644775390625e-08, sx = (double)p.mx * sc, sy = (double)p.my * sc, sz = (double)p.mz * sc;
    double sd = sx * vx + sy * vy + sz * vz;
    if (p.neg) sd = -sd;
    ux += fr * vx + sd * sx; uy += fr * vy + sd * sy; uz += fr * vz + sd * sz;
}
typedef unsigned nb4 __attribute__((ext_vector_type(4)));
__device__ __forceinline__ nb4 nb_pack(unsigned j, const PairCoef &p) {
    const unsigned f = (unsigned)p.f & 0x3FFFFFFu, mx = (unsigned)p.mx & 0x3FFFFFu, my = (unsigned)p.my & 0x3FFFFFu, mz = (unsigned)p.mz & 0x3FFFFFu;
    nb4 w;
    w.x = j | (p.neg ? (1u << 27) : 0u) | (f << 28);
    w.y = (f >> 4) | (mx << 22);
    w.z = (mx >> 10) | (my << 12);
    w.w = (my >> 20) | (mz << 2) | ((unsigned)(p.es + 128) << 24);
    return w;
}
__device__ __forceinline__ PairCoef nb_unpack(nb4 w, bool ok) {
    PairCoef p;
    p.neg = w.x & (1u << 27);
    p.f = ok ? (int)((((w.y & 0x3FFFFFu) << 4) | (w.x >> 28)) << 6) >> 6 : 0;
    p.mx = ok ? (int)((((w.z & 0xFFFu) << 10) | (w.y >> 22)) << 10) >> 10 : 0;
    p.my = ok ? (int)((((w.w & 0x3u) << 20) | (w.z >> 12)) << 10) >> 10 : 0;
    p.mz = ok ? (int)(((w.w >> 2) & 0x3FFFFFu) << 10) >> 10 : 0;
    p.es = ok ? (int)(w.w >> 24) - 128 : 0;
    return p;
}
template <bool STREAM = false>
__device__ __forceinline__ void nb_store(char *rec, int slot, int lane, unsigned j, const PairCoef &p) {
    char *r = rec + (size_t)(slot >> 2) * (4 * NB_REC);
    const nb4 w = nb_pack(j, p);
    if (STREAM) __builtin_nontemporal_store(w, (nb4 *)r + (slot & 3) * 64 + lane);
    else ((nb4 *)r)[(slot & 3) * 64 + lane] = w;
}
constexpr unsigned NB_NEG = 1u << 27;

// ... 2158 lines not shown
```

pse_amd/engine.py:

```python
import ctypes

from . import _lib
from ._lib import pse_info, pse_params


def _ptr(t):
    return ctypes.c_void_p(t.data_ptr()) if t is not None else None


def _chk4(t, name, n=None):
    import torch
    if not (isinstance(t, torch.Tensor) and t.is_cuda and t.dtype == torch.float64 and t.dim() == 2
            and t.shape[1] == 4 and t.is_contiguous()):
        raise ValueError(f"{name} must be a contiguous (N,4) float64 CUDA tensor")
    if n is not None and t.shape[0] < n:
        raise ValueError(f"{name} has fewer than {n} rows")


def _chk_group(g, name="group"):
    import torch
    if g is None:
        return
    if not (isinstance(g, torch.Tensor) and g.is_cuda and g.dtype in (torch.int32, torch.uint32) and g.dim() == 1
            and g.is_contiguous()):
# ... 138 lines not shown
        _chk4(pos, "pos"); _chk4(force, "force"); _chk_group(group)
        if vel is None:
            vel = torch.zeros_like(pos)
        _chk4(vel, "vel")
        m = ctypes.c_int(int(lanczos_m))
        _lib.check(self._lib.pse_brownian_velocity_part(self._h, _ptr(pos), _ptr(force), _ptr(vel), _ptr(group), n, float(kT), float(dt),
                                                        int(timestep), int(parts), ctypes.byref(m)))
        return vel, m.value

    def integrate(self, pos, vel, accel, image, force, dt, shear_rate=0.0, group=None):
        import torch
        n = pos.shape[0] if group is None else group.shape[0]
        _chk4(pos, "pos"); _chk4(vel, "vel"); _chk4(force, "force"); _chk_group(group)
        _chk_arr(accel, "accel", 3, torch.float64, pos.shape[0]); _chk_arr(image, "image", 3, torch.int32, pos.shape[0])
        _lib.check(self._lib.pse_integrate(self._h, _ptr(pos), _ptr(vel), _ptr(accel), _ptr(image), _ptr(force), _ptr(group), n, float(dt),
                                           float(shear_rate)))

    def step(self, pos, vel, accel, image, force, kT, dt, timestep, shear_rate=0.0, group=None, lanczos_m=2):
        n = pos.shape[0] if group is None else group.shape[0]
        import torch
        _chk4(pos, "pos"); _chk4(vel, "vel"); _chk4(force, "force"); _chk_group(group)
        _chk_arr(accel, "accel", 3, torch.float64, pos.shape[0]); _chk_arr(image, "image", 3, torch.int32, pos.shape[0])
        m = ctypes.c_int(int(lanczos_m))
        _lib.check(self._lib.pse_step(self._h, _ptr(pos), _ptr(vel), _ptr(accel), _ptr(image), _ptr(force),
                                      _ptr(group), n, float(kT), float(dt), int(timestep), float(shear_rate),
                                      ctypes.byref(m)))
        return m.value

    def sqrt_mreal(self, pos, psi, tol=1e-3, group=None, lanczos_m=2):
        import torch
        n = pos.shape[0] if group is None else group.shape[0]
        _chk4(pos, "pos"); _chk4(psi, "psi"); _chk_group(group)
        out = torch.zeros_like(psi)
        m = ctypes.c_int(int(lanczos_m))
        _lib.check(self._lib.pse_sqrt_mreal(self._h, _ptr(pos), _ptr(psi), _ptr(out), _ptr(group), n, float(tol),
                                            ctypes.byref(m)))
        return out, m.value

    def pair_repulsion(self, pos, force, k, sigma=2.0, group=None, accumulate=True):
        n = pos.shape[0] if group is None else group.shape[0]
        _chk4(pos, "pos"); _chk4(force, "force"); _chk_group(group)
        _lib.check(self._lib.pse_pair_repulsion(self._h, _ptr(pos), _ptr(force), _ptr(group), n, float(k), float(sigma),
                                                1 if accumulate else 0))
        return force

    def random_psi(self, n, timestep, group=None):
        import torch
        rows = n if group is None else int(group.max().item()) + 1
        psi = torch.zeros((rows, 4), dtype=torch.float64, device="cuda")
        _lib.check(self._lib.pse_random_psi(self._h, _ptr(psi), _ptr(group), n, int(timestep)))
        return psi

    def eval_realspace(self, r):
        import numpy as np
        r = np.ascontiguousarray(r, dtype=np.float64)
        f = np.zeros_like(r); g = np.zeros_like(r)
        dp = ctypes.POINTER(ctypes.c_double)
        _lib.check(self._lib.pse_eval_realspace(self._h, r.ctypes.data_as(dp), len(r), f.ctypes.data_as(dp),
                                                g.ctypes.data_as(dp)))
        return f, g

    def debug_spread(self, pos, force, group=None):
        n = pos.shape[0] if group is None else group.shape[0]
        _chk4(pos, "pos"); _chk4(force, "force"); _chk_group(group)
        _lib.check(self._lib.pse_debug_spread(self._h, _ptr(pos), _ptr(force), _ptr(group), n))
        return self.debug_grid()

    def debug_kvector(self, ijk):
        import numpy as np
        ijk = np.ascontiguousarray(ijk, dtype=np.int32)
        out = np.zeros((len(ijk), 5))
        _lib.check(self._lib.pse_debug_kvector(self._h, len(ijk), ijk.ctypes.data_as(ctypes.POINTER(ctypes.c_int)),
                                               out.ctypes.data_as(ctypes.POINTER(ctypes.c_double))))
        return out

    def set_lanczos_extra(self, extra):
        _lib.check(self._lib.pse_set_lanczos_extra(self._h, int(extra)))

    def matvec_ms(self, reps=20):
        ms = ctypes.c_float(0)
        _lib.check(self._lib.pse_debug_matvec_ms(self._h, int(reps), ctypes.byref(ms)))
        return ms.value

    def grid_placement(self):
        n, a, b = ctypes.c_int(0), ctypes.c_float(0), ctypes.c_float(0)
        _lib.check(self._lib.pse_debug_grid_placement(self._h, ctypes.byref(n), ctypes.byref(a), ctypes.byref(b)))
        return {"tried": n.value, "ms_first": a.value, "ms_kept": b.value}

    def debug_grid(self):
        import numpy as np
        i = self.info()
        out = np.zeros((3, i["Nx"] // max(1, self.params.n_slabs), i["Ny"], i["Nz"]))
        _lib.check(self._lib.pse_debug_copy_grid(self._h, 0, out.ctypes.data_as(ctypes.POINTER(ctypes.c_double))))
        return out


class Team:

    def __init__(self, engines, unique_id=None, transport=None):
        self._lib = _lib.load()
        self.engines = list(engines)
        self._t = ctypes.c_void_p()
        if transport is not None:
            self._transport = transport
            self._cb = _lib.pse_transport(None, _lib.EXCHANGE_FN(self._exchange), _lib.ALLREDUCE_FN(self._allreduce))
            _lib.check(self._lib.pse_team_create_transport(self.engines[0]._h, ctypes.byref(self._cb), ctypes.byref(self._t)))
            return
        arr = (ctypes.c_void_p * len(self.engines))(*[e._h for e in self.engines])
        idbuf = ctypes.create_string_buffer(bytes(unique_id), 128) if unique_id is not None else None
        _lib.check(self._lib.pse_team_create(arr, len(self.engines), idbuf, ctypes.byref(self._t)))

    def _exchange(self, _user, n, xfers):
        import numpy as np
        try:
            ops = []
            for q in range(n):
                x = xfers[q]
                send = np.ctypeslib.as_array(x.send, shape=(x.send_count,)) if x.send_count else None
                recv = np.ctypeslib.as_array(x.recv, shape=(x.recv_count,)) if x.recv_count else None
                ops.append((send, x.send_to, recv, x.recv_from))
            self._transport.exchange(ops)
            return 0
        except Exception as e:
            print("pse_amd transport: exchange failed:", repr(e))
            return 1

    def _allreduce(self, _user, buf, n):
        import numpy as np
        try:
            self._transport.allreduce_sum(np.ctypeslib.as_array(buf, shape=(n,)))
            return 0
        except Exception as e:
            print("pse_amd transport: all-reduce failed:", repr(e))
            return 1

    @staticmethod
    def unique_id():
        buf = ctypes.create_string_buffer(128)
        _lib.check(_lib.load().pse_team_unique_id(buf))
        return buf.raw

    def debug_solo(self, slab_rank):
        _lib.check(self._lib.pse_team_debug_solo(self._t, int(slab_rank)))

    def close(self):
        if getattr(self, "_t", None) is not None and self._t.value:
            self._lib.pse_team_destroy(self._t)
            self._t = ctypes.c_void_p()

    __del__ = close

    @staticmethod
    def _ptrs(tensors):
        return (ctypes.c_void_p * len(tensors))(*[t.data_ptr() for t in tensors])

    @staticmethod
    def _chk(group, *lists):
        _chk_group(group)
        for name, ts in lists:
            for t in ts:
                _chk4(t, name)

    def mobility(self, pos, force, vel, group=None, parts=3):
        n = pos[0].shape[0] if group is None else group.shape[0]
        self._chk(group, ("pos", pos), ("force", force), ("vel", vel))
        _lib.check(self._lib.pse_team_mobility(self._t, self._ptrs(pos), self._ptrs(force), self._ptrs(vel), _ptr(group),
# ... 91 lines not shown
```

Baseline: 327.1 million particle-steps/s.

## Fuse far-field bin counting and record writing into cell sort and permute

Far-field bin counts are now taken inside the cell-key kernel, and one exclusive scan covers both cell and bin offsets. The permute kernel writes the spreading records directly with a take-style atomic rank, so the separate record kernel no longer runs. The cell-order kernel is folded into permute, which derives each slot by counting smaller original indices within the cell. This removes several launches and passes over the data, but adds a per-thread loop over cell occupancy and makes record order within a bin nondeterministic.

```diff
diff --git a/include/pse_amd.h b/include/pse_amd.h
--- a/include/pse_amd.h
+++ b/include/pse_amd.h
@@ -98,6 +98,7 @@
 int pse_debug_grid_placement(pse_handle *h, int *tried, float *ms_first, float *ms_kept);
 int pse_debug_vq_roundtrip(int n, const double *rows_host, double *out_host);
 int pse_debug_matvec_ms(pse_handle *h, int reps, float *ms_per_launch);
+int pse_debug_prologue(pse_handle *h, unsigned int n, unsigned int *tag_host, int *rec_host, int *bin_host, unsigned int *n_rec);
 
 typedef struct pse_team pse_team;
 int pse_team_unique_id(void *id128_host);
diff --git a/pse_amd/_lib.py b/pse_amd/_lib.py
--- a/pse_amd/_lib.py
+++ b/pse_amd/_lib.py
@@ -119,6 +119,7 @@
     "pse_debug_grid_placement": (_i, [_vp, _ip, ctypes.POINTER(ctypes.c_float), ctypes.POINTER(ctypes.c_float)]),
     "pse_debug_vq_roundtrip": (_i, [_i, _dp, _dp]),
     "pse_debug_matvec_ms": (_i, [_vp, _i, ctypes.POINTER(ctypes.c_float)]),
+    "pse_debug_prologue": (_i, [_vp, _u, ctypes.POINTER(ctypes.c_uint), _ip, _ip, ctypes.POINTER(ctypes.c_uint)]),
     "pse_team_unique_id": (_i, [_vp]),
     "pse_team_create": (_i, [ctypes.POINTER(_vp), _i, _vp, ctypes.POINTER(_vp)]),
     "pse_team_create_transport": (_i, [_vp, ctypes.POINTER(pse_transport), ctypes.POINTER(_vp)]),
diff --git a/pse_amd/csrc/asan_stub.cpp b/pse_amd/csrc/asan_stub.cpp
--- a/pse_amd/csrc/asan_stub.cpp
+++ b/pse_amd/csrc/asan_stub.cpp
@@ -85,6 +85,7 @@
 int pse_debug_grid_placement(pse_handle *, int *, float *, float *) { return no_device("pse_debug_grid_placement"); }
 int pse_debug_vq_roundtrip(int, const double *, double *) { return no_device("pse_debug_vq_roundtrip"); }
 int pse_debug_matvec_ms(pse_handle *, int, float *) { return no_device("pse_debug_matvec_ms"); }
+int pse_debug_prologue(pse_handle *, unsigned int, unsigned int *, int *, int *, unsigned int *) { return no_device("pse_debug_prologue"); }
 int pse_set_lanczos_extra(pse_handle *, int) { return no_device("pse_set_lanczos_extra"); }
 int pse_set_lanczos_operator(pse_handle *h, int op) {
     if (!h) return fail(PSE_ERR_INVALID, "pse_set_lanczos_operator: null handle");
diff --git a/pse_amd/csrc/pse_capi.hip b/pse_amd/csrc/pse_capi.hip
--- a/pse_amd/csrc/pse_capi.hip
+++ b/pse_amd/csrc/pse_capi.hip
@@ -86,6 +86,7 @@
         int vq = 1;
         int place_trials = 10;
         int lz_extra = 2;
+        int prologue = 3;
         int lz_op = PSE_LANCZOS_RECORDS16;
     } tun;
     DCells bidx_nc = {0, 0, 0};
@@ -101,6 +102,8 @@
     int *cell_off = nullptr;
     int *cnt_block = nullptr;
     size_t cnt_bins = 0;
+    int *bin_off = nullptr;
+    bool rec_inline = false;
     SpreadWork sw = {};
     NbList nb = {};
     double4 *nb64 = nullptr;
@@ -361,7 +364,7 @@
     if (h->plan_x_inv) rocfft_plan_destroy(h->plan_x_inv);
     if (h->info_fwd) rocfft_execution_info_destroy(h->info_fwd);
     if (h->info_inv) rocfft_execution_info_destroy(h->info_inv);
-    void *ptrs[] = {h->keys, h->keys_s, h->vals, h->perm, h->tag_s, h->sort_tmp, h->cell_off, h->cnt_block, h->sw.rec_t, h->sw.fb.off, h->sw.fb.rank_s, h->sw.fb.tmp, h->nb.data, h->nb.cnt, h->vl.idx, h->vl.cnt, h->pos_build, h->pos_s, h->posf_s, h->pv,
+    void *ptrs[] = {h->keys, h->keys_s, h->vals, h->perm, h->tag_s, h->sort_tmp, h->cell_off, h->cnt_block, h->sw.rec_t, h->bin_off, h->sw.fb.rank_s, h->sw.fb.tmp, h->nb.data, h->nb.cnt, h->vl.idx, h->vl.cnt, h->pos_build, h->pos_s, h->posf_s, h->pv,
                     h->f_s, h->uw_s, h->ur_s, h->ub_s, h->psi_s, h->w_s, h->coef, h->rgrid, h->cgrid, h->sendbuf, h->recvbuf, h->d_bidx, h->d_bounds, h->utot_s, h->w2_s, h->u_s, h->sums_all, h->twiddle, h->twiddle_y_owned, h->twiddle_z_owned, h->fft_work, h->V,
                     h->scal, h->partials, h->lz_state, h->vq, h->nb64};
     for (void *p : ptrs) if (p) (void)hipFree(p);
@@ -529,6 +532,7 @@
         t.lz_extra = std::max(0, std::min(32, ienv("PSE_LANCZOS_EXTRA", 2)));
         t.place_trials = std::max(0, std::min(12, ienv("PSE_PLACE_TRIALS", 10)));
         t.vq = ienv("PSE_VQ", 1);
+        t.prologue = ienv("PSE_PROLOGUE", 3);
         if (const char *v = getenv("PSE_LANCZOS_OP")) t.lz_op = !strcmp(v, "fp64") ? PSE_LANCZOS_FP64 : PSE_LANCZOS_RECORDS16;
         if (const char *v = getenv("PSE_TEAM_SCHED")) {
             int a = 1, b = 2, c = 3;
@@ -587,15 +591,16 @@
         auto cnt = [&](double w) { int c2 = (int)std::floor(w / rc); if (c2 < 3) c2 = 1; if (c2 > 1024) c2 = 1024; return (size_t)c2; };
         h->n_cells_alloc = cnt(h->box.Lx) * cnt(h->box.Ly) * (cnt(h->box.Lz) + 16) + cnt(h->box.Lx);
     }
-    TRY(dmalloc(h, &h->cell_off, h->n_cells_alloc + 1));
-    h->sort_tmp_bytes = cell_sort_temp_bytes(h->n_cells_alloc);
-    TRY(dmalloc(h, (char **)&h->sort_tmp, h->sort_tmp_bytes));
     const size_t nbins = (size_t)((d.Nx + 7) / 8) * ((d.Ny + 7) / 8) * ((d.Nz + 7) / 8);
     const bool fast_far = d.P >= 4 && d.P <= FAR_PMAX;
+    const size_t bins2 = fast_far ? ((nbins + 1 + 3) & ~(size_t)3) : 0;
+    TRY(dmalloc(h, &h->cell_off, h->n_cells_alloc + 1 + bins2));
+    h->sort_tmp_bytes = cell_sort_temp_bytes(h->n_cells_alloc + bins2);
+    TRY(dmalloc(h, (char **)&h->sort_tmp, h->sort_tmp_bytes));
     h->cnt_bins = ((fast_far ? nbins + 1 : 0) + 1 + 3) & ~(size_t)3;
     constexpr size_t LAYER_INTS = (size_t)LOCAL_MAX_LAYERS * LOCAL_LAYER_SLOTS;
-    TRY(dmalloc(h, &h->cnt_block, h->cnt_bins + 4 + h->n_cells_alloc + 1 + 8 + LOCAL_NCOUNTER + 2 + LAYER_INTS + 4));
-    h->loc.counters = h->cnt_block + ((h->cnt_bins + 4 + h->n_cells_alloc + 1 + 8 + 1) & ~(size_t)1);
+    TRY(dmalloc(h, &h->cnt_block, h->cnt_bins + 4 + h->n_cells_alloc + bins2 + 1 + 8 + LOCAL_NCOUNTER + 2 + LAYER_INTS + 4));
+    h->loc.counters = h->cnt_block + ((h->cnt_bins + 4 + h->n_cells_alloc + bins2 + 1 + 8 + 1) & ~(size_t)1);
     h->loc.layer_cnt = h->loc.counters + LOCAL_NCOUNTER;
     h->loc.zero_ints = ((size_t)(h->loc.layer_cnt - h->cnt_block) + LAYER_INTS + 3) & ~(size_t)3;
     if (h->nc.nx > LOCAL_MAX_LAYERS && p->local_rows) return fail(PSE_ERR_INVALID, "more than %d cell layers along x", LOCAL_MAX_LAYERS);
@@ -606,7 +611,8 @@
         h->sw.fb.cnt = h->cnt_block;
         TRY(dmalloc(h, (char **)&h->sw.rec_t, (n + 64) * 64));
         TRY(dmalloc(h, &h->sw.fb.rank_s, n));
-        TRY(dmalloc(h, &h->sw.fb.off, nbins + 1));
+        TRY(dmalloc(h, &h->bin_off, nbins + 1));
+        h->sw.fb.off = h->bin_off;
         h->sw.fb.tmp_bytes = bin_scan_temp_bytes(nbins);
         TRY(dmalloc(h, (char **)&h->sw.fb.tmp, h->sw.fb.tmp_bytes));
     }
@@ -1182,6 +1188,8 @@
 static int prepare(pse_handle *h, const double4 *pos, const double4 *vec, const unsigned *group, int N, bool defer_bounds = false,
                    bool need_cells = false, PrepExtra px = PrepExtra{false, 0}, bool with_real = true) {
     TRY(ts(h, PH_SORT));
+    h->rec_inline = false;
+    if (h->sw.rec_t) { h->sw.fb.cnt = h->cnt_block; h->sw.fb.off = h->bin_off; }
     const FarBinArgs far = far_bin_args(h->G, h->sw);
     double4 *psi_out = px.psi ? h->psi_s : nullptr;
     h->nb_valid = false;
@@ -1262,11 +1270,23 @@
                 if (!kept((q * per + l) * layer)) { sb.book[q] = (q * per + l) * layer; break; }
         }
     }
-    HIPCHK(hipMemsetAsync(h->cnt_block, 0, ((h->cnt_bins + 4 + (size_t)ncell + 1 + 3) & ~(size_t)3) * sizeof(int), h->stream));
+    const bool fold = (h->tun.prologue & 1) != 0;
+    const bool fused = far.on && (h->tun.prologue & 2) != 0;
+    FarBinArgs far_here = far;
+    if (fused) {
+        h->sw.fb.cnt = h->cell_cnt + ncell + 1; h->sw.fb.off = h->cell_off + ncell + 1;
+        far_here = far_bin_args(h->G, h->sw);
+        far_here.rec = h->sw.rec_t;
+        h->rec_inline = true;
+        HIPCHK(hipMemsetAsync(h->cnt_block + h->cnt_bins - 4, 0, ((4 + 4 + (size_t)ncell + 1 + far_bin_count(h->G) + 3) & ~(size_t)3) * sizeof(int), h->stream));
+    } else {
+        HIPCHK(hipMemsetAsync(h->cnt_block, 0, ((h->cnt_bins + 4 + (size_t)ncell + 1 + 3) & ~(size_t)3) * sizeof(int), h->stream));
+    }
     HIPCHK(cell_sort(pos, group, N, h->dbox, h->nc, h->keys, h->vals, h->keys_s, h->cell_cnt, ncell, h->sort_tmp, h->sort_tmp_bytes,
-                     h->cell_off, h->perm, h->stream, need, sb, true));
-    launch_permute(pos, vec, group, h->perm, N, h->dbox, h->pos_s, h->posf_s, h->pv, h->f_s, h->tag_s, h->stream, nullptr, 0.0, nullptr,
-                   need, h->cell_off, &far, psi_out, h->par.seed, px.timestep, Gate{}, h->ts_off);
+                     h->cell_off, h->perm, h->stream, need, sb, true, Gate{}, fused ? &far_here : nullptr, !fold));
+    launch_permute(pos, vec, group, fold ? h->keys_s : h->perm, N, h->dbox, h->pos_s, h->posf_s, h->pv, h->f_s, h->tag_s, h->stream, nullptr, 0.0, nullptr,
+                   need, h->cell_off, &far_here, psi_out, h->par.seed, px.timestep, Gate{}, h->ts_off, fold ? h->keys : nullptr,
+                   fold && h->skin_max > 0.0 ? h->perm : nullptr);
     h->sorted_N = N;
     if (with_list) {
         h->vl_pending = true; h->vl_N = N; h->vl_group = group;
@@ -1300,7 +1320,7 @@
         if (part == 0) {
             double *gx = h->rgrid, *gy = h->rgrid + nr, *gz = h->rgrid + 2 * nr;
             TRY(tsw(h, PH_RECORDS));
-            HIPCHK(launch_far_records(h->pos_s, h->f_s, a.N, G, h->dbox, h->sw, h->wstream));
+            if (!h->rec_inline) HIPCHK(launch_far_records(h->pos_s, h->f_s, a.N, G, h->dbox, h->sw, h->wstream));
             TRY(tew(h, PH_RECORDS));
             TRY(tsw(h, PH_SPREAD));
             if (spread_needs_zero(G)) HIPCHK(hipMemsetAsync(h->rgrid, 0, 3 * nr * sizeof(double), h->wstream));
@@ -2379,6 +2399,31 @@
     return 0;
 }
 
+extern "C" int pse_debug_prologue(pse_handle *h, unsigned n, unsigned *tag_host, int *rec_host, int *bin_host, unsigned *n_rec) {
+    if (!h || !tag_host || !rec_host || !bin_host || !n_rec) return fail(PSE_ERR_INVALID, "pse_debug_prologue: null argument");
+    HIPCHK(hipSetDevice(h->device));
+    if (h->n_slabs != 1 || !h->sw.rec_t || h->sorted_N <= 0 || (int)n != h->sorted_N)
+        return fail(PSE_ERR_INVALID, "pse_debug_prologue: needs a single-GPU engine on the fast far-field path, after a call with n particles");
+    HIPCHK(hipStreamSynchronize(h->stream));
+    if (h->side) HIPCHK(hipStreamSynchronize(h->side));
+    const size_t nb1 = far_bin_count(h->G);
+    std::vector<int> off(nb1), rec((size_t)n * 16);
+    HIPCHK(hipMemcpy(tag_host, h->tag_s, (size_t)n * sizeof(unsigned), hipMemcpyDeviceToHost));
+    HIPCHK(hipMemcpy(off.data(), h->sw.fb.off, nb1 * sizeof(int), hipMemcpyDeviceToHost));
+    const long total = (long)off[nb1 - 1] - off[0];
+    if (total < 0 || total > (long)n) return fail(PSE_ERR_NUMERIC, "pse_debug_prologue: %ld records for %u particles", total, n);
+    HIPCHK(hipMemcpy(rec.data(), h->sw.rec_t, (size_t)total * 64, hipMemcpyDeviceToHost));
+    size_t b = 0;
+    for (long k = 0; k < total; ++k) {
+        while (b + 1 < nb1 - 1 && off[b + 1] - off[0] <= k) ++b;
+        const int *r = &rec[(size_t)k * 16];
+        rec_host[4 * k] = (int)((unsigned)r[3] & 0x7FFFFFFFu); rec_host[4 * k + 1] = r[0]; rec_host[4 * k + 2] = r[1]; rec_host[4 * k + 3] = r[2];
+        bin_host[k] = (int)b;
+    }
+    *n_rec = (unsigned)total;
+    return 0;
+}
+
 extern "C" int pse_debug_spread(pse_handle *h, const pse_double4 *pos, const pse_double4 *force, const unsigned *group, unsigned N) {
     TRY(check_n(h, N));
     if (!pos || !force) return fail(PSE_ERR_INVALID, "null array");
@@ -2387,7 +2432,7 @@
     const DGrid &G = h->G;
     const size_t nr = (size_t)(G.nxl + G.hl + G.nhalo) * G.Ny * G.Nz;
     if (spread_needs_zero(G)) HIPCHK(hipMemsetAsync(h->rgrid, 0, 3 * nr * sizeof(double), h->stream));
-    HIPCHK(launch_far_records(h->pos_s, h->f_s, (int)N, G, h->dbox, h->sw, h->stream));
+    if (!h->rec_inline) HIPCHK(launch_far_records(h->pos_s, h->f_s, (int)N, G, h->dbox, h->sw, h->stream));
     HIPCHK(launch_spread(h->pos_s, h->f_s, (int)N, h->rgrid, h->rgrid + nr, h->rgrid + 2 * nr, G, h->dbox, h->sw, h->stream));
     HIPCHK(hipStreamSynchronize(h->stream));
     return 0;
diff --git a/pse_amd/csrc/pse_farbin.h b/pse_amd/csrc/pse_farbin.h
--- a/pse_amd/csrc/pse_farbin.h
+++ b/pse_amd/csrc/pse_farbin.h
@@ -8,6 +8,14 @@
 __device__ __forceinline__ int bin_index(int ox, int oy, int oz, const FarBins &fb) {
     return ((ox / BIN) * fb.nby + (oy / BIN)) * fb.nbz + (oz / BIN);
 }
+
+struct FarRec {
+    int ox, oy, oz;
+    unsigned idx;
+    double d0x, d0y, d0z;
+    double fx, fy, fz;
+};
+static_assert(sizeof(FarRec) == 64, "record is four 16-byte loads");
 
 __device__ __forceinline__ void support_start(double f, int n, int P, int &start, double &delta0) {
     const double s = f * n;
@@ -25,6 +33,56 @@
     d.w = 0.0;
 }
 
+__device__ __forceinline__ double4 wrapped_position(const DBox &box, double fx, double fy, double fz) {
+    const double y = (fy - 0.5) * box.Ly;
+    double4 q;
+    q.x = (fx - 0.5) * box.Lx + box.xy * y;
+    q.y = y;
+    q.z = (fz - 0.5) * box.Lz;
+    q.w = 0.0;
+    return q;
+}
+
+struct FarSite { int4 o; double4 d; int bin; bool need; };
+__device__ __forceinline__ FarSite far_site(const DBox &box, const DGrid &G, const FarBins &fb, const double4 &q) {
+    FarSite t;
+    double gx, gy, gz;
+    frac_coords(box, q.x, q.y, q.z, gx, gy, gz);
+    far_support(gx, gy, gz, G, t.o, t.d);
+    t.need = true;
+    if (G.nxl < G.Nx) t.need = wrapi(t.o.w - (G.x0 - G.P), G.Nx) < G.nxl + 2 * G.P;
+    t.bin = bin_index(t.o.x, t.o.y, t.o.z, fb);
+    return t;
+}
+__device__ __forceinline__ void far_record_store(FarRec *__restrict__ rec, const FarSite &t, int p, const DGrid &G, double Fx, double Fy, double Fz) {
+    const bool owned = G.nxl == G.Nx || wrapi(t.o.w - G.x0, G.Nx) < G.nxl;
+    int4 h = make_int4(t.o.x, t.o.y, t.o.z, (int)((unsigned)p | (owned ? 0u : 0x80000000u)));
+    double2 *o = reinterpret_cast<double2 *>(rec);
+    o[0] = *reinterpret_cast<double2 *>(&h);
+    o[1] = make_double2(t.d.x, t.d.y);
+    o[2] = make_double2(t.d.z, G.prefac * Fx);
+    o[3] = make_double2(G.prefac * Fy, G.prefac * Fz);
+}
+
+__device__ __forceinline__ void far_bin_add(bool need, int bin, int *__restrict__ cnt) {
+    const int lane = threadIdx.x & 63;
+    if (!need) bin = -1;
+    const int prev = __shfl_up(bin, 1, 64);
+    if (__ballot(need && lane > 0 && bin == prev) == 0) {
+        if (need) atomicAdd(&cnt[bin], 1);
+        return;
+    }
+    unsigned long long todo = __ballot(need);
+    while (todo) {
+        const int src = __ffsll((long long)todo) - 1;
+        const int b0 = __shfl(bin, src, 64);
+        const unsigned long long m = __ballot(bin == b0) & todo;
+        if (lane == src) atomicAdd(&cnt[b0], __popcll(m));
+        todo &= ~m;
+    }
+}
+
+template <bool TAKE = false>
 __device__ __forceinline__ int far_bin_rank(bool need, int bin, int *__restrict__ cnt) {
     const int lane = threadIdx.x & 63;
     const unsigned long long below = (1ull << lane) - 1ull;
@@ -39,7 +97,7 @@
         todo &= ~m;
     }
     int base = 0;
-    if (need && leader == lane) base = atomicAdd(&cnt[bin], count);
+    if (need && leader == lane) base = TAKE ? atomicSub(&cnt[bin], count) - count : atomicAdd(&cnt[bin], count);
     base = __shfl(base, leader, 64);
     return need ? base + prefix : -1;
 }
diff --git a/pse_amd/csrc/pse_farfield.hip b/pse_amd/csrc/pse_farfield.hip
--- a/pse_amd/csrc/pse_farfield.hip
+++ b/pse_amd/csrc/pse_farfield.hip
@@ -8,14 +8,6 @@
 
 static inline int nblocks(long n, int tpb) { return (int)((n + tpb - 1) / tpb); }
 
-
-struct FarRec {
-    int ox, oy, oz;
-    unsigned idx;
-    double d0x, d0y, d0z;
-    double fx, fy, fz;
-};
-static_assert(sizeof(FarRec) == 64, "record is four 16-byte loads");
 
 template <int P>
 __device__ __forceinline__ void gauss_axis(double e0, double lq, const double *__restrict__ r, double (&a)[P]) {
@@ -76,21 +68,9 @@
     if (p >= N) return;
     const int rank = fb.rank_s[p];
     if (rank < 0) return;
-    const double4 q = pos_s[p];
-    double fx, fy, fz;
-    frac_coords(box, q.x, q.y, q.z, fx, fy, fz);
-    int4 sp;
-    double4 d0;
-    far_support(fx, fy, fz, G, sp, d0);
+    const FarSite t = far_site(box, G, fb, pos_s[p]);
     const double4 F = f_s[p];
-    const int slot = fb.off[bin_index(sp.x, sp.y, sp.z, fb)] + rank;
-    const bool owned = G.nxl == G.Nx || wrapi(sp.w - G.x0, G.Nx) < G.nxl;
-    int4 h = make_int4(sp.x, sp.y, sp.z, (int)((unsigned)p | (owned ? 0u : 0x80000000u)));
-    double2 *o = reinterpret_cast<double2 *>(rec + slot);
-    o[0] = *reinterpret_cast<double2 *>(&h);
-    o[1] = make_double2(d0.x, d0.y);
-    o[2] = make_double2(d0.z, G.prefac * F.x);
-    o[3] = make_double2(G.prefac * F.y, G.prefac * F.z);
+    far_record_store(rec + (fb.off[t.bin] - fb.off[0] + rank), t, p, G, F.x, F.y, F.z);
 }
 
 hipError_t launch_far_records(const double4 *pos_s, const double4 *f_s, int N, DGrid G, DBox box, SpreadWork w, hipStream_t s) {
@@ -170,7 +150,7 @@
         int z0 = blo[2], z1 = blo[2] + bcnt[2];
         if (zparts == 2) { if (zp == 0) z1 = nb[2]; else { z0 = 0; z1 = blo[2] + bcnt[2] - nb[2]; } }
         const int o = fb.off[row + z0];
-        s_rb[lane] = o;
+        s_rb[lane] = o - fb.off[0];
         s_ro[lane + 1] = fb.off[row + z1] - o;
     }
     __syncthreads();
@@ -432,7 +412,7 @@
     b = fdiv(b, dy, by);
     int bx = bx0 + b; if (bx >= fb.nbx) bx -= fb.nbx;
     const int bin = (bx * fb.nby + by) * fb.nbz + bz * BZ;
-    const int base = fb.off[bin], n = fb.off[bin + min(BZ, fb.nbz - bz * BZ)] - base;
+    const int base = fb.off[bin] - fb.off[0], n = fb.off[bin + min(BZ, fb.nbz - bz * BZ)] - fb.off[bin];
     if (n == 0) return;
     const double *g = cmp == 0 ? gx : (cmp == 1 ? gy : gz);
     const int t0[3] = {bx * BIN, by * BIN, bz * BINZ};
diff --git a/pse_amd/csrc/pse_kernels.h b/pse_amd/csrc/pse_kernels.h
--- a/pse_amd/csrc/pse_kernels.h
+++ b/pse_amd/csrc/pse_kernels.h
@@ -82,10 +82,13 @@
 void launch_gate_zero(Gate g, int *a, size_t na, int *b, size_t nb, hipStream_t s);
 void launch_gate_copy(Gate g, double4 *dst, const double4 *src, size_t n, hipStream_t s);
 struct SlabBook { int n, cells_per_slab, spread, book[64]; };
+struct FarBinArgs;
 hipError_t cell_sort(const double4 *pos, const unsigned *group, int N, DBox box, DCells nc, unsigned *keys, unsigned *rank,
                      unsigned *slots, int *cnt, int ncell, void *tmp, size_t tmp_bytes, int *cell_off, unsigned *perm, hipStream_t s,
                      CellRanges need = CellRanges{}, SlabBook sb = SlabBook{}, bool cnt_is_zero = false,
-                     Gate gate = Gate{});
+                     Gate gate = Gate{},
+                     const FarBinArgs *far = nullptr,
+                     bool order = true);
 hipError_t launch_cell_scan(const int *cnt, int *out, int n, void *tmp, size_t tmp_bytes, hipStream_t s);
 void launch_permute(const double4 *pos, const double4 *vec, const unsigned *group, const unsigned *perm, int N, DBox box,
                     double4 *pos_s, float4 *posf_s, double2 *pv, double4 *vec_s, unsigned *tag_s, hipStream_t s,
@@ -93,7 +96,8 @@
                     CellRanges need = CellRanges{}, const int *cell_off = nullptr,
                     const struct FarBinArgs *far = nullptr,
                     double4 *psi_s = nullptr, uint32_t seed = 0, uint32_t timestep = 0,
-                    Gate gate = Gate{}, const uint32_t *ts_off = nullptr);
+                    Gate gate = Gate{}, const uint32_t *ts_off = nullptr,
+                    const unsigned *cell_keys = nullptr, unsigned *perm_out = nullptr);
 void launch_permute_vec(const double4 *vec, const unsigned *tag_s, int N, double4 *vec_s, hipStream_t s);
 
 struct NbList {
@@ -164,7 +168,7 @@
 struct GaussConsts { double rx[FAR_PMAX - 1], ry[FAR_PMAX - 1], rz[FAR_PMAX - 1], lnk, s; };
 size_t farfield_bins(const DGrid &G);
 bool spread_needs_zero(const DGrid &G);
-struct FarBinArgs { bool on; DGrid G; FarBins fb; };
+struct FarBinArgs { bool on; DGrid G; FarBins fb; FarRec *rec; };
 FarBinArgs far_bin_args(const DGrid &G, const SpreadWork &w);
 size_t far_bin_count(const DGrid &G);
 hipError_t launch_far_records(const double4 *pos_s, const double4 *f_s, int N, DGrid G, DBox box, SpreadWork w, hipStream_t s);
diff --git a/pse_amd/csrc/pse_kernels.hip b/pse_amd/csrc/pse_kernels.hip
--- a/pse_amd/csrc/pse_kernels.hip
+++ b/pse_amd/csrc/pse_kernels.hip
@@ -46,12 +46,13 @@
 constexpr unsigned KEY_FOREIGN = 0xFFFFFFFFu;
 __global__ void k_cell_keys(const double4 *__restrict__ pos, const unsigned *__restrict__ group, int N, DBox box,
                             DCells nc, unsigned *__restrict__ keys, unsigned *__restrict__ rank, int *__restrict__ cnt, CellRanges need,
-                            SlabBook sb, Gate gate) {
+                            SlabBook sb, Gate gate, FarBinArgs far) {
     if (gate.closed()) return;
     const int g = blockIdx.x * blockDim.x + threadIdx.x;
     const bool live = g < N;
     unsigned key = 0;
-    bool mine = false;
+    bool mine = false, bin_need = false;
+    int bin = -1;
     if (live) {
         const unsigned idx = group ? group[g] : (unsigned)g;
         const double4 p = pos[idx];
@@ -64,11 +65,17 @@
         if (mine) {
             keys[g] = key;
             rank[g] = (unsigned)atomicAdd(&cnt[key], 1);
+            if (far.on) {
+                const FarSite t = far_site(box, far.G, far.fb, wrapped_position(box, fx, fy, fz));
+                bin_need = t.need;
+                bin = t.bin;
+            }
         } else {
             keys[g] = KEY_FOREIGN;
             if (sb.n == 0) atomicAdd(&cnt[key], 1);
         }
     }
+    if (far.on) far_bin_add(bin_need, bin, far.fb.cnt);
     if (sb.n > 0) {
         const int slab = live && !mine ? (int)(key / (unsigned)sb.cells_per_slab) : -1;
         unsigned long long todo = __ballot(slab >= 0);
@@ -110,14 +117,18 @@
 }
 hipError_t cell_sort(const double4 *pos, const unsigned *group, int N, DBox box, DCells nc, unsigned *keys, unsigned *rank,
                      unsigned *slots, int *cnt, int ncell, void *tmp, size_t tmp_bytes, int *cell_off, unsigned *perm, hipStream_t s,
-                     CellRanges need, SlabBook sb, bool cnt_is_zero, Gate gate) {
-    hipError_t e = cnt_is_zero ? hipSuccess : hipMemsetAsync(cnt, 0, (size_t)(ncell + 1) * sizeof(int), s);
+                     CellRanges need, SlabBook sb, bool cnt_is_zero, Gate gate, const FarBinArgs *far, bool order) {
+    const bool bins = far && far->on;
+    const int nbin1 = bins ? far->fb.nbx * far->fb.nby * far->fb.nbz + 1 : 0;
+    if (bins && (far->fb.cnt != cnt + ncell + 1 || far->fb.off != cell_off + ncell + 1)) return hipErrorInvalidValue;
+    hipError_t e = cnt_is_zero ? hipSuccess : hipMemsetAsync(cnt, 0, (size_t)(ncell + 1 + nbin1) * sizeof(int), s);
     if (e != hipSuccess) return e;
-    hipLaunchKernelGGL(k_cell_keys, dim3(nblocks(N, TPB)), dim3(TPB), 0, s, pos, group, N, box, nc, keys, rank, cnt, need, sb, gate);
-    e = hipcub::DeviceScan::ExclusiveSum(tmp, tmp_bytes, cnt, cell_off, ncell + 1, s);
+    hipLaunchKernelGGL(k_cell_keys, dim3(nblocks(N, TPB)), dim3(TPB), 0, s, pos, group, N, box, nc, keys, rank, cnt, need, sb, gate,
+                       bins ? *far : FarBinArgs{});
+    e = hipcub::DeviceScan::ExclusiveSum(tmp, tmp_bytes, cnt, cell_off, ncell + 1 + nbin1, s);
     if (e != hipSuccess) return e;
     hipLaunchKernelGGL(k_cell_scatter, dim3(nblocks(N, TPB)), dim3(TPB), 0, s, keys, rank, cell_off, N, slots, gate);
-    hipLaunchKernelGGL(k_cell_order, dim3(nblocks(N, TPB)), dim3(TPB), 0, s, cell_off, keys, N, slots, perm, need, gate);
+    if (order) hipLaunchKernelGGL(k_cell_order, dim3(nblocks(N, TPB)), dim3(TPB), 0, s, cell_off, keys, N, slots, perm, need, gate);
     return hipGetLastError();
 }
 
@@ -128,26 +139,30 @@
                           double4 *__restrict__ vec_s, unsigned *__restrict__ tag_s, const double4 *__restrict__ pos_build,
                           double half_skin2, int *__restrict__ flags, CellRanges need, const int *__restrict__ cell_off,
                           FarBinArgs far, double4 *__restrict__ psi_s, uint32_t seed, uint32_t timestep, Gate gate,
-                          const uint32_t *__restrict__ ts_off) {
+                          const uint32_t *__restrict__ ts_off, const unsigned *__restrict__ cell_keys, unsigned *__restrict__ perm_out) {
     if (gate.closed()) return;
     if (ts_off) timestep += *ts_off;
-    const int s = blockIdx.x * blockDim.x + threadIdx.x;
-    if (s - (int)(threadIdx.x & 63) >= N) return;
-    const bool live = s < N && need.row(s, cell_off);
-    bool bin_need = false;
-    int bin = -1;
+    const int slot = blockIdx.x * blockDim.x + threadIdx.x;
+    if (slot - (int)(threadIdx.x & 63) >= N) return;
+    const bool live = slot < N && need.row(slot, cell_off);
+    int s = slot;
+    FarSite site;
+    site.need = false; site.bin = -1;
+    double4 v = make_double4(0.0, 0.0, 0.0, 0.0);
     if (live) {
-        const unsigned g = perm[s];
+        const unsigned g = perm[slot];
+        if (cell_keys) {
+            const int c = (int)cell_keys[g], a = cell_off[c], n = cell_off[c + 1] - a;
+            int smaller = 0;
+            for (int t = 0; t < n; ++t) smaller += perm[a + t] < g ? 1 : 0;
+            s = a + smaller;
+            if (perm_out) perm_out[s] = g;
+        }
         const unsigned idx = group ? group[g] : g;
         const double4 p = pos[idx];
         double fx, fy, fz;
         frac_coords(box, p.x, p.y, p.z, fx, fy, fz);
-        const double y = (fy - 0.5) * box.Ly;
-        double4 q;
-        q.x = (fx - 0.5) * box.Lx + box.xy * y;
-        q.y = y;
-        q.z = (fz - 0.5) * box.Lz;
-        q.w = 0.0;
+        const double4 q = wrapped_position(box, fx, fy, fz);
         pos_s[s] = q;
         posf_s[s] = make_float4((float)q.x, (float)q.y, (float)q.z, 0.0f);
         if (pv) {
@@ -156,7 +171,7 @@
         }
         tag_s[s] = idx;
         if (vec) {
-            double4 v = vec[idx];
+            v = vec[idx];
             v.w = 0.0;
             vec_s[s] = v;
             if (pv) {
@@ -176,20 +191,18 @@
             const double c = 1.7320508075688772;
             psi_s[s] = make_double4(uniform_pm(r[0], c), uniform_pm(r[1], c), uniform_pm(r[2], c), 0.0);
         }
-        if (far.on) {
-            double gx, gy, gz;
-            frac_coords(box, q.x, q.y, q.z, gx, gy, gz);
-            int4 o;
-            double4 d;
-            far_support(gx, gy, gz, far.G, o, d);
-            bin_need = true;
-            if (far.G.nxl < far.G.Nx) bin_need = wrapi(o.w - (far.G.x0 - far.G.P), far.G.Nx) < far.G.nxl + 2 * far.G.P;
-            bin = bin_index(o.x, o.y, o.z, far.fb);
-        }
+        if (far.on) site = far_site(box, far.G, far.fb, q);
     }
     if (far.on) {
-        const int rk = far_bin_rank(bin_need, bin, far.fb.cnt);
-        if (s < N) far.fb.rank_s[s] = rk;
+        if (far.rec) {
+            const int rk = far_bin_rank<true>(site.need, site.bin, far.fb.cnt);
+            const int k = site.need ? far.fb.off[site.bin] - far.fb.off[0] + rk : -1;
+            if ((unsigned)k < (unsigned)N)
+                far_record_store(far.rec + k, site, s, far.G, v.x, v.y, v.z);
+        } else {
+            const int rk = far_bin_rank(site.need, site.bin, far.fb.cnt);
+            if (slot < N) far.fb.rank_s[s] = rk;
+        }
     }
 }
 
@@ -205,9 +218,11 @@
 void launch_permute(const double4 *pos, const double4 *vec, const unsigned *group, const unsigned *perm, int N, DBox box,
                     double4 *pos_s, float4 *posf_s, double2 *pv, double4 *vec_s, unsigned *tag_s, hipStream_t s,
                     const double4 *pos_build, double half_skin2, int *flags, CellRanges need, const int *cell_off,
-                    const FarBinArgs *far, double4 *psi_s, uint32_t seed, uint32_t timestep, Gate gate, const uint32_t *ts_off) {
+                    const FarBinArgs *far, double4 *psi_s, uint32_t seed, uint32_t timestep, Gate gate, const uint32_t *ts_off,
+                    const unsigned *cell_keys, unsigned *perm_out) {
     hipLaunchKernelGGL(k_permute, dim3(nblocks(N, TPB)), dim3(TPB), 0, s, pos, vec, group, perm, N, box, pos_s, posf_s, pv, vec_s, tag_s,
-                       pos_build, half_skin2, flags, need, cell_off, far ? *far : FarBinArgs{}, psi_s, seed, timestep, gate, ts_off);
+                       pos_build, half_skin2, flags, need, cell_off, far ? *far : FarBinArgs{}, psi_s, seed, timestep, gate, ts_off,
+                       cell_keys, perm_out);
 }
 __global__ void k_gate_decide(int *__restrict__ flags, int *__restrict__ word) {
     const int f = flags[0] | flags[1];
diff --git a/pse_amd/engine.py b/pse_amd/engine.py
--- a/pse_amd/engine.py
+++ b/pse_amd/engine.py
@@ -244,6 +244,15 @@
         _lib.check(self._lib.pse_debug_matvec_ms(self._h, int(reps), ctypes.byref(ms)))
         return ms.value
 
+    def debug_prologue(self, n):
+        import numpy as np
+        tag = np.zeros(n, dtype=np.uint32); rec = np.zeros((n, 4), dtype=np.int32); b = np.zeros(n, dtype=np.int32)
+        k = ctypes.c_uint(0)
+        _lib.check(self._lib.pse_debug_prologue(self._h, int(n), tag.ctypes.data_as(ctypes.POINTER(ctypes.c_uint)),
+                                                rec.ctypes.data_as(ctypes.POINTER(ctypes.c_int)),
+                                                b.ctypes.data_as(ctypes.POINTER(ctypes.c_int)), ctypes.byref(k)))
+        return {"tag": tag, "rec": rec[:k.value], "bin": b[:k.value]}
+
     def grid_placement(self):
         n, a, b = ctypes.c_int(0), ctypes.c_float(0), ctypes.c_float(0)
         _lib.check(self._lib.pse_debug_grid_placement(self._h, ctypes.byref(n), ctypes.byref(a), ctypes.byref(b)))
```

New measurement: 324.9 million particle-steps/s. About the same (-0.7%).
